# hucsmn/suffix_array

Measured on AMD Instinct MI355X. Metric: input MB/s indexed (SA build), higher is better.
Workload: dtype u8; 1 GPU; c3_english_256m: 268435456 bytes per GPU, seed base + rank, one independent text per GPU; n_bytes=268435456, sigma=57, symbols_per_key=13, refinement_rounds=9, text_rounds=0, radix_passes=25, unresolved_after_initial_sort=199000237

## Files before the change

suffix_array_amd/csrc/host/pipeline.hpp:

```cpp
#pragma once
#include "support.hpp"
#include "tuning.hpp"
#include "pool.hpp"

#include <functional>

namespace sa {

constexpr int SORT_MAX_WG = 1024;
constexpr int BK_TOP_BITS_MAX = 18;
constexpr uint32_t BK_BUCKETS_MAX = 1u << BK_TOP_BITS_MAX;
static_assert(32 - 16 <= BK_MAX_LBITS, "two 8-bit passes inside a bucket");
constexpr size_t GRAM_MAX_ENTRIES = (size_t)1 << 24;
static_assert(GROUP_CAP_MAX == GS_CAP, "Tuning clamps SA_AMD_GROUP_CAP to the kernel's cap");

#ifdef SA_AMD_DIAG
typedef void (*DownsweepFn)(const uint64_t *, const uint32_t *, uint64_t *, uint32_t *, uint32_t *,
                            const uint32_t *, int64_t, int, uint32_t, int64_t, int);
struct SortVariant { int threads, items, wg_per_cu; DownsweepFn fn; const char *name; };
static const SortVariant sort_variants[] = {
    { 1024, 8, 2, k_radix_downsweep_wcl<1024, 8, 16, 1, false, uint64_t, 4>, "carry-completed lines 1024x8 + LDS prefetch of half of the next tile's keys (default)" },
    { 1024, 8, 2, k_radix_downsweep_wcl<1024, 8>, "carry-completed lines 1024x8" },
    { 512, 16, 1, k_radix_downsweep_wcl<512, 16>, "carry-completed lines 512x16" },
    { 1024, 8, 2, k_radix_downsweep_wcl<1024, 8, 8>, "carry 1024x8, granule 8" },
#ifdef SA_AMD_DIAG
    { 1024, 8, 2, k_radix_downsweep<1024, 8, 4>, "plain tile scatter 1024x8 (first generation)" },
    { 1024, 8, 2, k_radix_downsweep<1024, 8, 4, 1>, "plain 1024x8 ABLATION sequential stores (wrong results)" },
    { 1024, 8, 2, k_radix_downsweep<1024, 8, 4, 33>, "plain 1024x8 ABLATION no ranking + sequential stores (wrong results)" },
    { 1024, 8, 2, k_radix_downsweep<1024, 8, 4, 16>, "plain 1024x8 ABLATION no stores (wrong results)" },
    { 1024, 8, 2, k_radix_downsweep<1024, 8, 4, 49>, "plain 1024x8 ABLATION no ranking, no stores (wrong results)" },
    { 1024, 8, 2, k_radix_downsweep_wcl<1024, 8, 16, 1, true>, "carry 1024x8 DIAGNOSTIC phase stamps (tools/phase_stamps.py)" },
#endif
};
constexpr int N_SORT_VARIANTS = (int)(sizeof(sort_variants) / sizeof(sort_variants[0]));

struct SortGrid { int G; int64_t tiles_per_wg; int tile; };
static SortGrid sort_grid(int64_t count, const SortVariant &sv)
{
    SortGrid g;
    g.tile = sv.threads * sv.items;
    const int64_t tiles = ceil_div(count, g.tile);
    int max_wg = 256 * sv.wg_per_cu;
    if (max_wg > SORT_MAX_WG) max_wg = SORT_MAX_WG;
    g.tiles_per_wg = ceil_div(tiles, max_wg);
    if (g.tiles_per_wg < 1) g.tiles_per_wg = 1;
    g.G = (int)ceil_div(tiles, g.tiles_per_wg);
    if (g.G < 1) g.G = 1;
    return g;
}

#else
constexpr int N_SORT_VARIANTS = 1;
#endif

struct SortScratch {
    uint32_t *spine;
    uint32_t *digit_tot;
    unsigned long long *status;
    uint32_t *err;
};

struct Workspace {
    uint64_t *keysA, *keysB, *keysC;
    uint32_t *valsA, *valsB, *isa, *U0, *U1, *G0, *G1;
    uint32_t *spine, *digit_tot, *tcnt, *thead, *tnext, *hist, *total, *chg, *has_isa;
    uint8_t *packed;
    uint8_t *gram_flags;
    uint4 *gram_table;
    uint32_t *surv_bits, *surv_cnt, *todo_bits, *ft_cnt, *ft_head;
    unsigned long long *os_status;
    uint32_t *os_err;
    uint32_t *bk_start;
    uint32_t *early_bits, *early_cnt;
    SortScratch ss;
    size_t bytes, bytes2;
};

static Workspace carve(void *base, int64_t n, size_t cap = ~(size_t)0, void *base2 = nullptr)
{
    Workspace w;
    const size_t N = (size_t)(n > 0 ? n : 1);
    size_t off = 0, off2 = 0;
    auto take = [&](size_t b) {
        if (off + b <= cap) { size_t o = off; off = align_up(off + b, 256); return (char *)base + o; }
        size_t o = off2; off2 = align_up(off2 + b, 256); return (char *)base2 + o;
    };
    const size_t rr_tiles = (size_t)ceil_div((int64_t)N, RR_TILE);
    const size_t ft_tiles = (size_t)ceil_div((int64_t)N, FT_TILE) + 1;
    const size_t gram_entries = N < GRAM_MAX_ENTRIES ? N : GRAM_MAX_ENTRIES;
    w.spine = (uint32_t *)take((size_t)RADIX * SORT_MAX_WG * 4);
    w.digit_tot = (uint32_t *)take(RADIX * 4);
    w.os_status = (unsigned long long *)take(((size_t)ceil_div((int64_t)N, OS_MIN_TILE) + 1) * RADIX * 8);
    w.os_err = (uint32_t *)take(256);
    w.hist = (uint32_t *)take(256 * 4);
    w.total = (uint32_t *)take(256);
    w.chg = (uint32_t *)take((size_t)RR_CHG_COUNTERS * 32 * 4);
    w.tcnt = (uint32_t *)take(rr_tiles * 4);
    w.thead = (uint32_t *)take(rr_tiles * 4);
    w.tnext = (uint32_t *)take(rr_tiles * 4);
    w.surv_cnt = (uint32_t *)take(rr_tiles * 4);
    w.ft_cnt = (uint32_t *)take(ft_tiles * 4);
    w.ft_head = (uint32_t *)take(ft_tiles * 4);
    w.bk_start = (uint32_t *)take(((size_t)BK_BUCKETS_MAX + 1) * 4);
    w.early_cnt = (uint32_t *)take(((N + 1 + EARLY_TILE - 1) / EARLY_TILE + 8) * 4);
    w.gram_table = (uint4 *)take((gram_entries / 64 + 1) * 16);
    w.has_isa = (uint32_t *)take((N + 31) / 32 * 4);
    w.surv_bits = (uint32_t *)take((N + 31) / 32 * 4);
    w.todo_bits = (uint32_t *)take((N + 31) / 32 * 4);
    w.early_bits = (uint32_t *)take(((N + 1 + 31) / 32 + EARLY_THREADS) * 4);
    w.gram_flags = (uint8_t *)take(gram_entries + 64);
    w.packed = (uint8_t *)take(N / 2 + 64);
    w.keysA = (uint64_t *)take((N + 64) * 8);
    w.keysB = (uint64_t *)take((N + 64) * 8);
    w.valsA = (uint32_t *)take(N * 4);
    w.valsB = (uint32_t *)take(N * 4);
    w.isa = (uint32_t *)take(N * 4);
    w.U0 = (uint32_t *)take(N * 4);
    w.G0 = (uint32_t *)take(N * 4);
    w.U1 = (uint32_t *)take(N * 4);
    w.G1 = (uint32_t *)take(N * 4);
    w.keysC = (uint64_t *)take((N + 64) * 8);
    w.ss.spine = w.spine; w.ss.digit_tot = w.digit_tot; w.ss.status = w.os_status; w.ss.err = w.os_err;
    w.bytes = off;
    w.bytes2 = off2;
    return w;
}


struct OsShape { int threads, items; bool seq; int wg_per_cu; };
static const OsShape os_shapes64[] = { { 1024, 8, false, 1 }, { 512, 16, true, 2 }, { 512, 8, false, 2 } };
static const OsShape os_shapes32[] = { { 1024, 12, false, 1 }, { 512, 16, true, 2 }, { 512, 12, false, 2 }, { 1024, 8, false, 1 } };
constexpr int N_OS_SHAPES64 = (int)(sizeof(os_shapes64) / sizeof(os_shapes64[0]));
constexpr int N_OS_SHAPES32 = (int)(sizeof(os_shapes32) / sizeof(os_shapes32[0]));
constexpr int OS_TICKETS = 64;
constexpr int OS_MAX_RADIX = 512;
constexpr int OS_ZONE = OS_TICKETS + OS_MAX_RADIX * OS_NSEG;
static_assert(OS_NSEG <= OS_TICKETS, "one ticket word per segment");
constexpr int OS_MAX_ZONES = 2 * 8 + 2;
static_assert(OS_MAX_ZONES * OS_ZONE <= RADIX * SORT_MAX_WG, "the zones live in the spine slab");

#ifdef SA_AMD_DIAG
static bool onesweep_on(const SortScratch &ss, const Tuning &tn) { return ss.status != nullptr && !tn.no_onesweep; }
#else
static bool onesweep_on(const SortScratch &ss, const Tuning &) { return ss.status != nullptr; }
#endif

struct OnesweepGeom { int tiles, nseg, tiles_per_seg; int64_t seg_elems; };
static OnesweepGeom onesweep_geom(int64_t count, int tile)
{
    OnesweepGeom g;
    g.tiles = (int)ceil_div(count, tile);
    if (g.tiles < 1) g.tiles = 1;
    int nseg = g.tiles < OS_NSEG ? g.tiles : OS_NSEG;
    g.tiles_per_seg = (int)ceil_div(g.tiles, nseg);
    g.nseg = (int)ceil_div(g.tiles, g.tiles_per_seg);
    g.seg_elems = (int64_t)g.tiles_per_seg * tile;
    return g;
}

struct FirstCounts { uint32_t *counts; int64_t chunk_elems; int G; void *zero_ptr; size_t zero_bytes; };
static FirstCounts sort_first_counts(const SortScratch &ss, const Tuning &tn, int64_t count, bool keys32);

static int cu_count()
{
    static int cus = 0;
    if (cus > 0) return cus;
    int dev = 0;
    hipDeviceProp_t prop;
    if (hipGetDevice(&dev) == hipSuccess && hipGetDeviceProperties(&prop, dev) == hipSuccess && prop.multiProcessorCount > 0) cus = prop.multiProcessorCount;
    else { (void)hipGetLastError(); cus = 256; }
    return cus;
}

static int read_words(void *dst, const void *dsrc, size_t bytes, hipStream_t st);

__global__ __launch_bounds__(RADIX) void k_os_digit_totals(const uint32_t *__restrict__ hist, int nseg, uint32_t *__restrict__ digit_tot)
{
    uint32_t s = 0;
    for (int q = 0; q < nseg; ++q) s += hist[threadIdx.x * nseg + q];
    digit_tot[threadIdx.x] = s;
}

constexpr int HA_THREADS = 256;
template <typename KeyT>
__global__ __launch_bounds__(HA_THREADS) void k_radix_hist_all(const KeyT *__restrict__ keys, int64_t count, int begin_bit, int end_bit,
                                                               uint32_t *__restrict__ zone0, int zone_words, int ticket_words)
{
    __shared__ uint32_t h[8][RADIX];
    for (int i = threadIdx.x; i < 8 * RADIX; i += HA_THREADS) (&h[0][0])[i] = 0;
    __syncthreads();
    const int np = (end_bit - begin_bit + RADIX_BITS - 1) / RADIX_BITS;
    for (int64_t i = (int64_t)blockIdx.x * HA_THREADS + threadIdx.x; i < count; i += (int64_t)gridDim.x * HA_THREADS) {
        const uint64_t k = (uint64_t)keys[i];
        for (int p = 0; p < np; ++p) {
            const int sh = begin_bit + p * RADIX_BITS, nb = end_bit - sh < RADIX_BITS ? end_bit - sh : RADIX_BITS;
            atomicAdd(&h[p][(k >> sh) & ((1u << nb) - 1u)], 1u);
        }
    }
    __syncthreads();
    for (int i = threadIdx.x; i < np * RADIX; i += HA_THREADS) {
        const uint32_t c = (&h[0][0])[i];
        if (c) atomicAdd(&zone0[(size_t)(i / RADIX) * zone_words + ticket_words + (i % RADIX)], c);
    }
}

template <typename KeyT, int THREADS, int ITEMS, bool SEQ, int RBITS = RADIX_BITS>
static int sort_pairs_onesweep(KeyT *keys_in, uint32_t *vals_in, KeyT *keys_alt, uint32_t *vals_alt, int64_t count, int begin_bit, int end_bit,
                               const SortScratch &ss, uint32_t *final_vals, hipStream_t st, KeyT **keys_res, uint32_t **vals_res, int *passes,
                               int *skipped, const Tuning &tn, bool iota, bool may_skip, bool first_counted,
                               const uint8_t *text = nullptr, int64_t text_n = 0,
                               int text_bits = 8,
                               int val_extra = 0,
                               KeyT *keys_out2 = nullptr)
{
    constexpr int TILE = THREADS * ITEMS;
    constexpr int R = 1 << RBITS;
    static_assert(R <= OS_MAX_RADIX && (RBITS == RADIX_BITS || TILE >= 2 * OS_MIN_TILE), "zones and granule slab are sized for 8-bit digits of 4 Ki-element tiles");
    static_assert(TILE >= OS_MIN_TILE, "the granule slab is sized for tiles of at least OS_MIN_TILE elements");
    constexpr bool K64 = sizeof(KeyT) == 8;
    OnesweepGeom g = onesweep_geom(count, TILE);
    auto zone = [&](int i) { return ss.spine + (size_t)i * OS_ZONE; };
    int z = 0;
    bool have_counts = first_counted;
    const int npass = (int)ceil_div(end_bit - begin_bit, RBITS);
    const bool upfront = RBITS == RADIX_BITS && !tn.no_upfront_counts && count < tn.count_next_min_n && !may_skip && !text && npass <= 8 && npass >= 2;
    if (upfront) { g.nseg = 1; g.tiles_per_seg = g.tiles; g.seg_elems = (int64_t)g.tiles * TILE; }
    HIP_TRY(hipMemsetAsync(ss.status, 0, (size_t)g.tiles * R * 8, st));
    {
        int zones = (may_skip ? 2 * npass : npass) + 1;
        if (zones > OS_MAX_ZONES) return SA_AMD_EINTERNAL;
        const int z0 = (first_counted && !upfront) ? 1 : 0;
        HIP_TRY(hipMemsetAsync(zone(z0), 0, (size_t)(zones - z0) * OS_ZONE * 4, st));
    }
    if (upfront) {
        int blocks = (int)ceil_div(count, (int64_t)HA_THREADS * 16);
        if (blocks > 512) blocks = 512;
        if (blocks < 1) blocks = 1;
        PROF(K64 ? KC_UPSWEEP : KC_UPSWEEP32, count, st, hipLaunchKernelGGL((k_radix_hist_all<KeyT>), dim3((unsigned)blocks), dim3(HA_THREADS), 0, st, (const KeyT *)keys_in, count,
                                                                        begin_bit, end_bit, zone(0), (int)OS_ZONE, (int)OS_TICKETS));
        have_counts = true;
    }
    KeyT *kin = keys_in, *kout = keys_alt;
    uint32_t *vin = vals_in, *vout = vals_alt;
    constexpr int WG_PER_CU = THREADS <= 512 ? 2 : 1;
    int grid = cu_count() * WG_PER_CU;
    if (grid > g.tiles) grid = g.tiles;
    uint32_t epoch = 0;
    for (int shift = begin_bit; shift < end_bit; shift += RBITS) {
        const int nb = (end_bit - shift) < RBITS ? (end_bit - shift) : RBITS;
        const uint32_t dmask = (1u << nb) - 1u;
        const bool last = shift + RBITS >= end_bit;
        uint32_t *vdst = (last && final_vals) ? final_vals : vout;
        if (!have_counts) {
            if (RBITS != RADIX_BITS) return SA_AMD_EINTERNAL;
            int split = 2048 / g.nseg;
            while (split > 1 && g.seg_elems / split < 8192) split /= 2;
            const int64_t sub = K64 ? ((ceil_div(g.seg_elems, split) + 1) & ~(int64_t)1) : ((ceil_div(g.seg_elems, split) + 3) & ~(int64_t)3);
            if (K64)
                PROF(KC_UPSWEEP, count, st, hipLaunchKernelGGL((k_radix_upsweep), dim3(g.nseg * split), dim3(SORT_THREADS), 0, st, (const uint64_t *)kin,
                                                               zone(z) + OS_TICKETS, count, shift, dmask, g.seg_elems, g.nseg, split, sub));
            else
                PROF(KC_UPSWEEP32, count, st, hipLaunchKernelGGL((k_radix_upsweep32), dim3(g.nseg * split), dim3(SORT_THREADS), 0, st, (const uint32_t *)kin,
                                                                 zone(z) + OS_TICKETS, count, shift, dmask, g.seg_elems, g.nseg, split, sub));
        }
        if (RBITS == RADIX_BITS && may_skip && !tn.no_run_skip && count >= tn.run_skip_min && !(iota && *passes == 0) && !(last && final_vals)) {
            hipLaunchKernelGGL(k_os_digit_totals, dim3(1), dim3(RADIX), 0, st, (const uint32_t *)(zone(z) + OS_TICKETS), g.nseg, ss.digit_tot);
            LAUNCH_CHECK(st);
            uint32_t tot[RADIX];
            { const int rcw = read_words(tot, ss.digit_tot, sizeof(tot), st); if (rcw) return rcw; }
            bool constant = false;
            for (int d = 0; d < RADIX; ++d) constant |= (int64_t)tot[d] == count;
            if (constant) { ++*skipped; have_counts = false; ++z; continue; }
        }
        OnesweepPass P;
        P.hist_cur = zone(z) + OS_TICKETS;
        const bool count_next = !upfront && !last && (RBITS != RADIX_BITS || count >= tn.count_next_min_n || count < tn.count_next_below_n);
        P.hist_next = count_next ? zone(z + 1) + OS_TICKETS : nullptr;
        P.tickets = zone(z + 1);
        P.status = ss.status;
        P.err = ss.err;
        P.n = count;
        P.shift = shift; P.dmask = dmask;
        P.shift_next = shift + RBITS;
        { const int nbn = (end_bit - P.shift_next) < RBITS ? (end_bit - P.shift_next) : RBITS; P.dmask_next = last ? 0u : (1u << nbn) - 1u; }
        P.nseg = g.nseg; P.tiles_per_seg = g.tiles_per_seg; P.tiles = g.tiles;
        P.epoch = ++epoch;
        P.flags = (uint32_t)tn.onesweep_flags;
        P.text = text; P.text_n = text_n; P.text_bits = text_bits;
        P.val_extra = (text && *passes == 0 && iota) ? val_extra : 0;
        if (!K64 && !SEQ && text && *passes == 0)
            PROF(KC_ONESWEEP32, count, st,
                 hipLaunchKernelGGL((k_onesweep<THREADS, ITEMS, KeyT, SEQ, WG_PER_CU, RBITS, !K64 && !SEQ>), dim3(grid), dim3(THREADS), 0, st, (const KeyT *)kin,
                                    (const uint32_t *)((iota && *passes == 0) ? nullptr : vin), kout, vdst, P));
        else
        PROF(K64 ? KC_ONESWEEP : KC_ONESWEEP32, count, st,
             hipLaunchKernelGGL((k_onesweep<THREADS, ITEMS, KeyT, SEQ, WG_PER_CU, RBITS>), dim3(grid), dim3(THREADS), 0, st, (const KeyT *)kin,
                                (const uint32_t *)((iota && *passes == 0) ? nullptr : vin), kout, vdst, P));
        KeyT *tk = kin; kin = kout; kout = (keys_out2 && *passes == 0) ? keys_out2 : tk;
        uint32_t *free_v = vin;
        vin = vdst;
        vout = free_v;
        ++*passes;
        ++z;
        have_counts = count_next || upfront;
    }
    *keys_res = kin; *vals_res = vin;
    return SA_AMD_OK;
}

struct SortResult { uint64_t *keys; uint32_t *vals; int passes; int skipped; };

static int sort_pairs(uint64_t *keys_in, uint32_t *vals_in, uint64_t *keys_alt, uint32_t *vals_alt, int64_t count,
                      int begin_bit, int end_bit, const SortScratch &ss, uint32_t *final_vals,
                      hipStream_t st, SortResult *res, const Tuning &tn, bool iota = false,
                      bool may_skip = false,
                      bool first_counted = false)
{
    res->keys = keys_in; res->vals = vals_in; res->passes = 0; res->skipped = 0;
    if (count <= 1 || end_bit <= begin_bit) return SA_AMD_OK;
    if (onesweep_on(ss, tn)) {
#define OS_CALL64(T, I, S) sort_pairs_onesweep<uint64_t, T, I, S>(keys_in, vals_in, keys_alt, vals_alt, count, begin_bit, end_bit, ss, final_vals, st, \
                                                                 &res->keys, &res->vals, &res->passes, &res->skipped, tn, iota, may_skip, first_counted)
        switch (tn.onesweep64_shape) {
        case 1: return OS_CALL64(512, 16, true);
        case 2: return OS_CALL64(512, 8, false);
        default: return OS_CALL64(1024, 8, false);
        }
#undef OS_CALL64
    }
#ifdef SA_AMD_DIAG
    uint32_t *spine = ss.spine, *digit_tot = ss.digit_tot;
    const SortVariant &sv = sort_variants[tn.sort_variant];
    const SortGrid g = sort_grid(count, sv);
    uint64_t *kin = keys_in, *kout = keys_alt;
    uint32_t *vin = vals_in, *vout = vals_alt;
    for (int shift = begin_bit; shift < end_bit; shift += RADIX_BITS) {
        const int nb = (end_bit - shift) < RADIX_BITS ? (end_bit - shift) : RADIX_BITS;
        const uint32_t dmask = (1u << nb) - 1u;
        const bool last = shift + RADIX_BITS >= end_bit;
        uint32_t *vdst = (last && final_vals) ? final_vals : vout;
        {
            const int64_t chunk = g.tiles_per_wg * g.tile;
            int split = 2048 / g.G;
            if (split < 1) split = 1;
            while (split > 1 && chunk / split < 4096) split /= 2;
            const int64_t sub = (ceil_div(chunk, split) + 1) & ~(int64_t)1;
            if (first_counted && shift == begin_bit) {
            } else {
            if (split > 1 && res->passes == 0) HIP_TRY(hipMemsetAsync(spine, 0, (size_t)RADIX * g.G * 4, st));
            PROF(KC_UPSWEEP, count, st, hipLaunchKernelGGL((k_radix_upsweep), dim3(g.G * split), dim3(SORT_THREADS), 0, st, kin, spine,
                                                           count, shift, dmask, chunk, g.G, split, sub));
            }
        }
        PROF(KC_SPINE, (int64_t)RADIX * g.G, st, hipLaunchKernelGGL((k_spine_rows), dim3(RADIX), dim3(SPINE_THREADS), 0, st,
                                                                    spine, digit_tot, g.G));
        if (may_skip && !tn.no_run_skip && count >= tn.run_skip_min && !(iota && res->passes == 0) && !(last && final_vals)) {
            uint32_t tot[RADIX];
            { const int rcw = read_words(tot, digit_tot, sizeof(tot), st); if (rcw) return rcw; }
            bool constant = false;
            for (int d = 0; d < RADIX; ++d) constant |= (int64_t)tot[d] == count;
            if (constant) {
                HIP_TRY(hipMemsetAsync(spine, 0, (size_t)RADIX * g.G * 4, st));
                res->skipped++;
                continue;
            }
        }
        PROF(KC_DOWNSWEEP, count, st, hipLaunchKernelGGL((sv.fn), dim3(g.G), dim3(sv.threads), 0, st,
                                                         (const uint64_t *)kin, (const uint32_t *)((iota && res->passes == 0) ? nullptr : vin), kout, vdst,
                                                         spine, (const uint32_t *)digit_tot, count, shift,
                                                         dmask, g.tiles_per_wg, g.G));
        uint64_t *tk = kin; kin = kout; kout = tk;
        uint32_t *free_v = vin;
        vin = vdst;
        vout = free_v;
        res->passes++;
    }
    res->keys = kin; res->vals = vin;
    return SA_AMD_OK;
#else
    return SA_AMD_EINTERNAL;
#endif
}

struct SortResult32 { uint32_t *keys; uint32_t *vals; int passes; };
#ifdef SA_AMD_DIAG
constexpr int SORT32_THREADS = 1024;
typedef void (*Downsweep32Fn)(const uint32_t *, const uint32_t *, uint32_t *, uint32_t *, uint32_t *, const uint32_t *, int64_t, int,
                              uint32_t, int64_t, int);
struct Sort32Variant { int items; Downsweep32Fn fn; };
static const Sort32Variant sort32_variants[] = {
    { 12, k_radix_downsweep_wcl<SORT32_THREADS, 12, 16, 1, false, uint32_t, 12> },
    { 12, k_radix_downsweep_wcl<SORT32_THREADS, 12, 16, 1, false, uint32_t> },
    { 8, k_radix_downsweep_wcl<SORT32_THREADS, 8, 16, 1, false, uint32_t> },
    { 16, k_radix_downsweep_wcl<SORT32_THREADS, 16, 16, 1, false, uint32_t> },
    { 8, k_radix_downsweep_wcl<SORT32_THREADS, 8, 16, 1, false, uint32_t, 8> },
};
constexpr int N_SORT32_VARIANTS = (int)(sizeof(sort32_variants) / sizeof(sort32_variants[0]));

struct SortGrid32 { int G; int64_t tiles_per_wg, tile; };
static SortGrid32 sort_grid32(int64_t count, const Sort32Variant &sv)
{
    SortGrid32 g;
    g.tile = (int64_t)SORT32_THREADS * sv.items;
    const int64_t tiles = ceil_div(count, g.tile);
    g.tiles_per_wg = ceil_div(tiles, 512);
    if (g.tiles_per_wg < 1) g.tiles_per_wg = 1;
    g.G = (int)ceil_div(tiles, g.tiles_per_wg);
    return g;
}

#else
constexpr int N_SORT32_VARIANTS = 1;
#endif

static int sort_pairs32(uint32_t *keys_in, uint32_t *vals_in, uint32_t *keys_alt, uint32_t *vals_alt, int64_t count, int begin_bit,
                        int end_bit, const SortScratch &ss, uint32_t *final_vals, hipStream_t st, SortResult32 *res,
                        const Tuning &tn, bool iota = false, bool first_counted = false,
                        int rbits = RADIX_BITS,
                        const uint8_t *text = nullptr, int64_t text_n = 0, int text_bits = 8,
                        int val_extra = 0,
                        uint32_t *keys_out2 = nullptr)
{
    res->keys = keys_in; res->vals = vals_in; res->passes = 0;
    if (keys_out2 && (rbits != RADIX_BITS || text)) return SA_AMD_EINTERNAL;
    if (count <= 1 || end_bit <= begin_bit) return SA_AMD_OK;
    if (rbits != RADIX_BITS && (rbits != 9 || !onesweep_on(ss, tn) || !first_counted)) return SA_AMD_EINTERNAL;
    if (text && (!onesweep_on(ss, tn) || !first_counted || tn.onesweep32_shape != 0)) return SA_AMD_EINTERNAL;
    if (onesweep_on(ss, tn)) {
        int skipped = 0;
        if (rbits == 9)
            return sort_pairs_onesweep<uint32_t, 1024, 12, false, 9>(keys_in, vals_in, keys_alt, vals_alt, count, begin_bit, end_bit, ss, final_vals, st,
                                                                     &res->keys, &res->vals, &res->passes, &skipped, tn, iota, false, first_counted, text, text_n, text_bits, val_extra);
        if (text)
            return sort_pairs_onesweep<uint32_t, 1024, 12, false, RADIX_BITS>(keys_in, vals_in, keys_alt, vals_alt, count, begin_bit, end_bit, ss, final_vals, st,
                                                                              &res->keys, &res->vals, &res->passes, &skipped, tn, iota, false, first_counted, text, text_n, text_bits, val_extra);
#define OS_CALL32(T, I, S) sort_pairs_onesweep<uint32_t, T, I, S>(keys_in, vals_in, keys_alt, vals_alt, count, begin_bit, end_bit, ss, final_vals, st, \
                                                                 &res->keys, &res->vals, &res->passes, &skipped, tn, iota, false, first_counted, \
                                                                 nullptr, 0, 8, 0, keys_out2)
        switch (tn.onesweep32_shape) {
        case 1: return OS_CALL32(512, 16, true);
        case 2: return OS_CALL32(512, 12, false);
        case 3: return OS_CALL32(1024, 8, false);
        default: return OS_CALL32(1024, 12, false);
        }
#undef OS_CALL32
    }
#ifdef SA_AMD_DIAG
    uint32_t *spine = ss.spine, *digit_tot = ss.digit_tot;
    const Sort32Variant &sv = sort32_variants[tn.sort32_variant];
    const SortGrid32 g32 = sort_grid32(count, sv);
    const int64_t SORT32_TILE = g32.tile, tiles_per_wg = g32.tiles_per_wg;
    const int G = g32.G;
    uint32_t *kin = keys_in, *kout = keys_alt, *vin = vals_in, *vout = vals_alt;
    for (int shift = begin_bit; shift < end_bit; shift += RADIX_BITS) {
        const int nb = (end_bit - shift) < RADIX_BITS ? (end_bit - shift) : RADIX_BITS;
        const uint32_t dmask = (1u << nb) - 1u;
        const bool last = shift + RADIX_BITS >= end_bit;
        uint32_t *vdst = (last && final_vals) ? final_vals : vout;
        {
            const int64_t chunk = tiles_per_wg * SORT32_TILE;
            int split = 2048 / G;
            if (split < 1) split = 1;
            while (split > 1 && chunk / split < 8192) split /= 2;
            const int64_t sub = (ceil_div(chunk, split) + 3) & ~(int64_t)3;
            if (first_counted && shift == begin_bit) {
            } else {
            if (split > 1 && res->passes == 0) HIP_TRY(hipMemsetAsync(spine, 0, (size_t)RADIX * G * 4, st));
            PROF(KC_UPSWEEP32, count, st, hipLaunchKernelGGL((k_radix_upsweep32), dim3(G * split), dim3(SORT_THREADS), 0, st,
                                                           (const uint32_t *)kin, spine, count, shift, dmask, chunk, G, split, sub));
            }
        }
        PROF(KC_SPINE, (int64_t)RADIX * G, st, hipLaunchKernelGGL((k_spine_rows), dim3(RADIX), dim3(SPINE_THREADS), 0, st, spine, digit_tot, G));
        PROF(KC_DOWNSWEEP32, count, st, hipLaunchKernelGGL((sv.fn),
                                                         dim3(G), dim3(SORT32_THREADS), 0, st, (const uint32_t *)kin,
                                                         (const uint32_t *)((iota && res->passes == 0) ? nullptr : vin), kout,
                                                         vdst, spine, (const uint32_t *)digit_tot, count, shift, dmask,
                                                         tiles_per_wg, G));
        uint32_t *tk = kin; kin = kout; kout = (keys_out2 && res->passes == 0) ? keys_out2 : tk;
        uint32_t *free_v = vin;
        vin = vdst;
        vout = free_v;
        res->passes++;
    }
    res->keys = kin; res->vals = vin;
    return SA_AMD_OK;
#else
    return SA_AMD_EINTERNAL;
#endif
}

static FirstCounts sort_first_counts(const SortScratch &ss, const Tuning &tn, int64_t count, bool keys32)
{
    FirstCounts f;
    if (onesweep_on(ss, tn)) {
        const OsShape &sh = keys32 ? os_shapes32[tn.onesweep32_shape] : os_shapes64[tn.onesweep64_shape];
        const int tile = sh.threads * sh.items;
        const OnesweepGeom g = onesweep_geom(count, tile);
        f.counts = ss.spine + OS_TICKETS; f.chunk_elems = g.seg_elems; f.G = g.nseg;
        f.zero_ptr = ss.spine; f.zero_bytes = (size_t)OS_ZONE * 4;
        return f;
    }
#ifdef SA_AMD_DIAG
    f.counts = ss.spine; f.zero_ptr = ss.spine;
    if (keys32) {
        const SortGrid32 g32 = sort_grid32(count, sort32_variants[tn.sort32_variant]);
        f.chunk_elems = g32.tiles_per_wg * g32.tile; f.G = g32.G;
    } else {
        const SortGrid g64 = sort_grid(count, sort_variants[tn.sort_variant]);
        f.chunk_elems = g64.tiles_per_wg * g64.tile; f.G = g64.G;
    }
    f.zero_bytes = (size_t)RADIX * f.G * 4;
    return f;
#else
    f.counts = ss.spine; f.zero_ptr = ss.spine; f.chunk_elems = count; f.G = 1; f.zero_bytes = (size_t)RADIX * 4;
    return f;
#endif
}

struct BkShape { int threads, items, minw; };
static const BkShape bk_shapes[] = { { 256, 10, 6 }, { 512, 10, 8 }, { 1024, 10, 8 }, { 1024, 20, 1 }, { 256, 20, 1 } };
constexpr int N_BK_SHAPES = (int)(sizeof(bk_shapes) / sizeof(bk_shapes[0]));
constexpr int N_BK_DEFAULT = 4;
static int64_t bucket_cap(int shape) { return (int64_t)bk_shapes[shape].threads * bk_shapes[shape].items; }
static int64_t bucket_cap_max() { return bucket_cap(N_BK_DEFAULT - 1); }

static int bucket_sort32(const uint32_t *keys_in, const uint32_t *vals_in, uint32_t *keys_out, uint32_t *vals_out, int64_t count, int top_bits,
                         uint32_t *start, uint32_t *words, hipStream_t st, const Tuning &tn, bool *done, uint32_t *largest,
                         const BucketFinish *fin = nullptr, const KeyParams *P = nullptr, const KeySrc *K = nullptr, bool *fused = nullptr,
                         int val_extra = 0)
{
    *done = false; *largest = 0;
    if (fused) *fused = false;
    if (top_bits < 32 - BK_MAX_LBITS || top_bits > BK_TOP_BITS_MAX) return SA_AMD_EINTERNAL;
    const int lbits = 32 - top_bits;
    if (val_extra < 0 || lbits + val_extra > BK_MAX_LBITS) return SA_AMD_EINTERNAL;
    const uint32_t nb = 1u << top_bits;
    HIP_TRY(hipMemsetAsync(words, 0, 8, st));
    PROF(KC_MISC, nb, st, hipLaunchKernelGGL((k_bucket_starts), dim3((unsigned)ceil_div((int64_t)nb + 1, BK_STARTS_THREADS)), dim3(BK_STARTS_THREADS),
                                              0, st, keys_in, count, lbits, nb, start));
    PROF(KC_MISC, nb, st, hipLaunchKernelGGL((k_bucket_max), dim3((unsigned)ceil_div((int64_t)nb, BK_STARTS_THREADS)), dim3(BK_STARTS_THREADS), 0, st,
                                              (const uint32_t *)start, nb, words));
    uint32_t maxb = 0;
    { const int rcw = read_words(&maxb, words, 4, st); if (rcw) return rcw; }
    *largest = maxb;
    int shape = -1;
    if (tn.bucket_shape >= 0 && tn.bucket_shape < N_BK_SHAPES && bucket_cap(tn.bucket_shape) >= (int64_t)maxb) shape = tn.bucket_shape;
    for (int c = 0; shape < 0 && c < N_BK_DEFAULT; ++c)
        if (bucket_cap(c) >= (int64_t)maxb) shape = c;
    if (shape < 0) return SA_AMD_OK;
    const bool fuse = fin != nullptr && (bk_shapes[shape].items <= 10 || tn.bucket_finish_always);
    const BucketFinish F0 = BucketFinish();
    const KeyParams P0 = KeyParams();
    const KeySrc K0 = KeySrc();
#define BK_LAUNCH(T, I, W)                                                                                                               \
    do {                                                                                                                                 \
        if (fuse) PROF(KC_BUCKET, count, st, hipLaunchKernelGGL((k_bucket_sort<T, I, W, true>), dim3(nb), dim3(T), 0, st, keys_in, vals_in,         \
                                                                (const uint32_t *)start, lbits, keys_out, vals_out, words + 1, *fin, *P, *K, val_extra)); \
        else PROF(KC_BUCKET, count, st, hipLaunchKernelGGL((k_bucket_sort<T, I, W, false>), dim3(nb), dim3(T), 0, st, keys_in, vals_in,             \
                                                            (const uint32_t *)start, lbits, keys_out, vals_out, words + 1, F0, P0, K0, val_extra)); \
    } while (0)
    switch (shape) {
    case 0: BK_LAUNCH(256, 10, 6); break;
    case 1: BK_LAUNCH(512, 10, 8); break;
    case 2: BK_LAUNCH(1024, 10, 8); break;
    case 3: BK_LAUNCH(1024, 20, 1); break;
    default: BK_LAUNCH(256, 20, 1); break;
    }
#undef BK_LAUNCH
    *done = true;
    if (fused) *fused = fuse;
    return SA_AMD_OK;
}

#ifdef SA_AMD_DIAG
static int64_t sample_count(int64_t n, const Tuning &tn)
{
    int lg = tn.sample_log ? tn.sample_log : (n >= ((int64_t)1 << 28) ? 22 : (n >= ((int64_t)1 << 27) ? 21 : 20));
    while (lg > 16 && ((int64_t)1 << lg) * 4 > n) --lg;
    return (int64_t)1 << lg;
}

static int sample_sort64(uint64_t *keys_a, uint64_t *keys_b, uint64_t *keys_c, uint32_t *vals_a, uint32_t *vals_b, uint32_t *u0, uint32_t *u1,
                         uint32_t *big, uint32_t *small, uint32_t *words, uint32_t *final_vals, int64_t n, int key_bits, const SortScratch &ss,
                         hipStream_t st, sa_amd_stats *local, const Tuning &tn, bool *done, bool trace)
{
    *done = false;
    const int64_t S = sample_count(n, tn);
    if (S < 65536 || n < 4 * S || n >= ((int64_t)1 << 32)) return SA_AMD_OK;
    uint64_t *samp = keys_c, *samp_alt = keys_c + S;
    PROF(KC_MISC, S, st, hipLaunchKernelGGL((k_ss_sample), dim3((unsigned)ceil_div(S, 256)), dim3(256), 0, st, (const uint64_t *)keys_a, n, S, samp));
    SortResult sr;
// ... 11 lines not shown
    PROF(KC_SS_COUNT, n, st, hipLaunchKernelGGL((k_ss_count<1>), dim3((unsigned)tiles1), dim3(SS_THREADS), 0, st, (const uint64_t *)keys_a, n, sample, S,
                                                (const uint32_t *)nullptr, (const uint32_t *)nullptr, (const uint32_t *)nullptr, counts));
    PROF(KC_RR_SCAN, tiles1, st, hipLaunchKernelGGL((k_ss_scan_tiles<SS_WAYS>), dim3((unsigned)chunks), dim3(SS_WAYS), 0, st, counts, tiles1, per,
                                                    (const uint32_t *)nullptr, tot1));
    PROF(KC_RR_SCAN, chunks, st, hipLaunchKernelGGL((k_ss_bases1), dim3(1), dim3(SS_WAYS), 0, st, (const uint32_t *)tot1, chunks, base1, seg_start, seg_first));
    PROF(KC_RR_SCAN, max_tiles2, st, hipLaunchKernelGGL((k_ss_tiles), dim3(SS_WAYS + 1), dim3(256), 0, st, (const uint32_t *)seg_start, (const uint32_t *)seg_first,
                                                        max_tiles2, tile_seg, tile_base));
    PROF(KC_SS_SCATTER, n, st, hipLaunchKernelGGL((k_ss_scatter<1>), dim3((unsigned)tiles1), dim3(SS_THREADS), 0, st, (const uint64_t *)keys_a, (const uint32_t *)nullptr, n,
                                                  sample, S, (const uint32_t *)nullptr, (const uint32_t *)nullptr, (const uint32_t *)nullptr,
                                                  (const uint32_t *)counts, (const uint32_t *)base1, per, keys_b, vals_a));
    PROF(KC_SS_COUNT, n, st, hipLaunchKernelGGL((k_ss_count<2>), dim3((unsigned)max_tiles2), dim3(SS_THREADS), 0, st, (const uint64_t *)keys_b, n, sample, S,
                                                (const uint32_t *)tile_seg, (const uint32_t *)tile_base, (const uint32_t *)seg_start, counts));
    PROF(KC_RR_SCAN, max_tiles2, st, hipLaunchKernelGGL((k_ss_scan_tiles<SS_IDS2>), dim3(SS_WAYS), dim3(SS_IDS2), 0, st, counts, max_tiles2, (int64_t)0,
                                                        (const uint32_t *)seg_first, tot2));
    PROF(KC_RR_SCAN, SS_WAYS, st, hipLaunchKernelGGL((k_ss_bases2), dim3(SS_WAYS), dim3(SS_IDS2), 0, st, (const uint32_t *)tot2, (const uint32_t *)seg_start, bstart, (uint32_t)n));
    PROF(KC_SS_SCATTER, n, st, hipLaunchKernelGGL((k_ss_scatter<2>), dim3((unsigned)max_tiles2), dim3(SS_THREADS), 0, st, (const uint64_t *)keys_b, (const uint32_t *)vals_a, n,
                                                  sample, S, (const uint32_t *)tile_seg, (const uint32_t *)tile_base, (const uint32_t *)seg_start,
                                                  (const uint32_t *)counts, (const uint32_t *)bstart, (int64_t)1, keys_a, vals_b));
    HIP_TRY(hipMemsetAsync(words, 0, 16, st));
    if (!tn.sample_merge)
    PROF(KC_SS_BUCKET, n, st, hipLaunchKernelGGL((k_ss_bucket_sort<SB_SMALL_THREADS, SB_SMALL_ITEMS, 9, 0, false>), dim3((unsigned)SS_BUCKETS), dim3(SB_SMALL_THREADS), 0, st,
                                                 (const uint64_t *)keys_a, (const uint32_t *)vals_b, (const uint32_t *)bstart, keys_b, final_vals, words, words + 4));
    else
    PROF(KC_SS_BUCKET, n, st, hipLaunchKernelGGL((k_ss_bucket_merge<SB_SMALL_THREADS, SB_SMALL_ITEMS>), dim3((unsigned)SS_BUCKETS), dim3(SB_SMALL_THREADS), 0, st,
                                                 (const uint64_t *)keys_a, (const uint32_t *)vals_b, (const uint32_t *)bstart, keys_b, final_vals, words));
    PROF(KC_SS_BUCKET, 0, st, hipLaunchKernelGGL((k_ss_bucket_sort<SB_THREADS, SB_ITEMS, 10, SB_SMALL_CAP, true>), dim3((unsigned)SS_BUCKETS), dim3(SB_THREADS), 0, st,
                                                 (const uint64_t *)keys_a, (const uint32_t *)vals_b, (const uint32_t *)bstart, keys_b, final_vals, words, words + 4));
    uint32_t res[2] = { 0, 0 };
    { const int rcw = read_words(res, words, 8, st); if (rcw) return rcw; }
    local->sort_passes += 3; local->sorted_elements += 3 * n;
    if (trace) fprintf(stderr, "suffix_array_amd: sample sort: %lld samples, largest bucket %u (a workgroup holds %d), %u oversize buckets that are no equality buckets\n",
                       (long long)S, res[1], SB_CAP, res[0]);
    *done = res[0] == 0;
    return SA_AMD_OK;
}

#endif

static int make_key_params(const uint32_t *hist, KeyParams *P, int *sigma_out, int kb_max = 64)
{
    int sigma = 0;
    for (int c = 0; c < 256; ++c) {
        if (hist[c]) P->code[c] = (uint8_t)sigma++;
        else P->code[c] = 0;
    }
    *sigma_out = sigma;
    P->packed = nullptr;
    P->gram = 0; P->gram_m = 0; P->gram_tail = 0; P->gram_top = 0; P->gram_D = 0; P->gram_table = nullptr;
    const uint64_t se = sigma > 2 ? (uint64_t)sigma : 2u;
    P->sigma = se;
    if ((se & (se - 1)) == 0) {
        const int bits = bit_length(se - 1);
        P->bits = bits;
        P->k = kb_max / bits;
        const int used = P->k * bits;
        P->mask = used >= 64 ? ~0ull : ((1ull << used) - 1ull);
        P->top = 0;
        return used;
    }
    unsigned __int128 pw = 1;
    int k = 0;
    while (pw * se <= ((unsigned __int128)1 << kb_max)) { pw *= se; ++k; }
    P->bits = 0;
    P->k = k;
    P->mask = ~0ull;
    uint64_t top = 1;
    for (int i = 0; i + 1 < k; ++i) top *= se;
    P->top = top;
    const unsigned __int128 maxkey = pw - 1;
    return bit_length((uint64_t)maxkey);
}

struct PinnedWords {
    PinBlock b;
    bool failed = false;
    ~PinnedWords() { if (b.p) pool().release_pinned(b); }
};
static thread_local PinnedWords g_pinned;
static thread_local int g_readbacks = 0;
static thread_local bool g_posted_off = false;
static std::atomic<uint32_t> g_post_seq{0};

constexpr int POST_LINE = 16;
__global__ __launch_bounds__(256) void k_post_words(const uint32_t *__restrict__ src, uint32_t *__restrict__ dst, int words, uint32_t seq)
{
    const int lines = (words + POST_LINE - 2) / (POST_LINE - 1);
    for (int i = threadIdx.x; i < lines * POST_LINE; i += 256) {
        const int q = i / POST_LINE, j = i % POST_LINE;
        if (j) { const int k = q * (POST_LINE - 1) + j - 1; dst[i] = k < words ? src[k] : 0u; }
    }
    __threadfence_system();
    __syncthreads();
    for (int q = threadIdx.x; q < lines; q += 256) __hip_atomic_store(dst + q * POST_LINE, seq, __ATOMIC_RELEASE, __HIP_MEMORY_SCOPE_SYSTEM);
}

static int read_words(void *dst, const void *dsrc, size_t bytes, hipStream_t st)
{
    ++g_readbacks;
    if (!g_pinned.b.p && !g_pinned.failed) {
        if (pool().pinned(8192, -1, -1, &g_pinned.b) == SA_AMD_OK) memset(g_pinned.b.p, 0, 8192);
        else g_pinned.failed = true;
    }
    if (!g_pinned.b.p) {
        HIP_TRY(hipMemcpyAsync(dst, dsrc, bytes, hipMemcpyDeviceToHost, st));
        HIP_TRY(hipStreamSynchronize(st));
        return SA_AMD_OK;
    }
    const int words = (int)(bytes / 4);
    const int lines = (words + POST_LINE - 2) / (POST_LINE - 1);
    if (!g_posted_off && (bytes & 3) == 0 && words > 0 && (size_t)lines * POST_LINE * 4 <= 4096) {
        uint32_t *host = (uint32_t *)g_pinned.b.p;
        uint32_t seq = g_post_seq.fetch_add(1, std::memory_order_relaxed) + 1;
        if (seq == 0) seq = g_post_seq.fetch_add(1, std::memory_order_relaxed) + 1;
        hipLaunchKernelGGL(k_post_words, dim3(1), dim3(256), 0, st, (const uint32_t *)dsrc, host, words, seq);
        if (hipGetLastError() == hipSuccess) {
            const auto t0 = std::chrono::steady_clock::now();
            bool done = false, finished = false;
            for (unsigned spin = 0; !done; ++spin) {
                done = true;
                for (int q = lines - 1; q >= 0 && done; --q)
                    done = __atomic_load_n((volatile uint32_t *)(host + q * POST_LINE), __ATOMIC_ACQUIRE) == seq;
                if (done) break;
                if ((spin & 1023u) == 1023u) {
                    const double us = std::chrono::duration<double, std::micro>(std::chrono::steady_clock::now() - t0).count();
                    if (us > 200.0) {
                        if (finished) break;
                        const hipError_t q = hipStreamQuery(st);
                        if (q == hipSuccess) finished = true;
                        else if (q != hipErrorNotReady) { (void)hipGetLastError(); break; }
                    }
                }
            }
            if (done) {
                uint32_t *out = (uint32_t *)dst;
                for (int k = 0; k < words; ++k) out[k] = host[(k / (POST_LINE - 1)) * POST_LINE + 1 + k % (POST_LINE - 1)];
                return SA_AMD_OK;
            }
        }
    }
    char *copy = (char *)g_pinned.b.p + 4096;
    HIP_TRY(hipMemcpyAsync(copy, dsrc, bytes, hipMemcpyDeviceToHost, st));
    HIP_TRY(hipStreamSynchronize(st));
    memcpy(dst, copy, bytes);
    return SA_AMD_OK;
}

static bool binned(int64_t n, int64_t count, const Tuning &tn)
{
    if (tn.no_binned_isa) return false;
    if (tn.binned_isa_always) return count > 0;
    return n >= ((int64_t)1 << 25) && (count >= n || count >= tn.binned_min);
}

static int scatter_binned(uint32_t *pk, uint32_t *pv, uint32_t *altk, uint32_t *altv, int64_t count, int64_t n,
                          const Workspace &w, hipStream_t st, sa_amd_stats *local, const Tuning &tn, bool iota = false,
                          uint32_t *altk2 = nullptr, uint32_t *altv2 = nullptr)
{
    const int nb = bit_length((uint64_t)(n > 1 ? n : 1));
    int wlog = nb - 16;
    if (wlog < 10) wlog = 10;
    if (wlog > 15) wlog = 15;
    const bool two = nb > wlog && (tn.scatter_levels == 2 || (tn.scatter_levels == 0 && count >= ((int64_t)1 << 25)));
    SortResult32 pr;
    if (two) {
        int rc;
        if (iota) {
            const int mid = wlog + RADIX_BITS < nb ? wlog + RADIX_BITS : nb;
            rc = sort_pairs32(pk, nullptr, altk, altv, count, wlog, mid, w.ss, nullptr, st, &pr, tn, true);
            if (rc) return rc;
            if (pr.passes != 1) return SA_AMD_EINTERNAL;
            local->sort_passes += 1; local->sorted_elements += count;
            if (mid < nb) {
                rc = sort_pairs32(altk, altv, altk2, altv2, count, mid, nb, w.ss, nullptr, st, &pr, tn);
                if (rc) return rc;
                local->sort_passes += pr.passes; local->sorted_elements += (int64_t)pr.passes * count;
            }
        } else {
            rc = sort_pairs32(pk, pv, altk, altv, count, wlog, nb, w.ss, nullptr, st, &pr, tn, false, false, RADIX_BITS, nullptr, 0, 8, 0, altk2);
            if (rc) return rc;
            local->sort_passes += pr.passes; local->sorted_elements += (int64_t)pr.passes * count;
        }
        const unsigned grid = (unsigned)ceil_div(count, SW_CHUNK);
        if (wlog <= 13)
            PROF(KC_SCATTER, count, st, hipLaunchKernelGGL((k_scatter_windows<13>), dim3(grid), dim3(SW_THREADS), 0, st, (const uint32_t *)pr.keys,
                                                           (const uint32_t *)pr.vals, w.isa, count, (uint32_t)n, wlog));
        else
            PROF(KC_SCATTER, count, st, hipLaunchKernelGGL((k_scatter_windows<15>), dim3(grid), dim3(SW_THREADS), 0, st, (const uint32_t *)pr.keys,
                                                           (const uint32_t *)pr.vals, w.isa, count, (uint32_t)n, wlog));
        return SA_AMD_OK;
    }
    const int shift = nb > RADIX_BITS ? nb - RADIX_BITS : 0;
    int rc = sort_pairs32(pk, pv, altk, altv, count, shift, shift + RADIX_BITS, w.ss, nullptr, st, &pr, tn, iota);
    if (rc) return rc;
    local->sort_passes += pr.passes; local->sorted_elements += (int64_t)pr.passes * count;
    PROF(KC_SCATTER, count, st, hipLaunchKernelGGL((k_scatter_pairs<uint32_t>), dim3((unsigned)ceil_div(count, 1024)), dim3(256), 0, st,
                                                   (const uint32_t *)pr.keys, (const uint32_t *)pr.vals, w.isa, count, (uint32_t)n));
    return SA_AMD_OK;
}

struct Refined { const uint64_t *keys; const uint32_t *vals; uint32_t *vnext; int64_t m_global; };

constexpr int RC_FLAGGED = 16, RC_GROUPS = 8, RC_BIG_LISTED = 12, RC_BIG_ORDERED = 13, RC_WORDS = 17;
constexpr int RC_BIG_LISTED_SAVED = 14, RC_BIG_ORDERED_SAVED = 15;
struct RoundCtl {
    bool defer = false;
    const uint32_t *resume_tot = nullptr;
    bool skip_big = false;
    bool counters_clear = false;
    bool deferred = false;
    int64_t m_flagged = -1;
    int64_t big_listed = -1;
};

static int split_giant_groups(uint64_t *rkA, uint64_t *rkB, uint32_t *Vcur, uint32_t *Valt, const uint32_t *Ucur, const uint32_t *Gcur,
                              uint32_t *scratchU, uint32_t *scratchG, int64_t m, int64_t n, uint32_t groups, int kb, int sort_bits,
                              const Workspace &w, hipStream_t st, sa_amd_stats *local, Refined *out, const Tuning &tn, bool *taken,
                              bool starts_ready)
{
    *taken = false;
    const int64_t tiles = ceil_div(m, RR_TILE);
    auto up = [](size_t b) { return (b + 255) & ~(size_t)255; };
    char *sg = (char *)scratchG;
    uint32_t *starts = (uint32_t *)sg;            sg += up(((size_t)groups + 1) * 4);
    uint32_t *mps = (uint32_t *)sg;               sg += up(((size_t)groups + 1) * 4);
    uint32_t *Lless = (uint32_t *)sg;             sg += up((size_t)groups * 4);
    uint64_t *pivot = (uint64_t *)sg;             sg += up((size_t)groups * 8);
    const size_t cap = (size_t)m / 8 + 1;
    uint32_t *mv = (uint32_t *)sg, *mv_alt = mv + ((cap + 63) & ~(size_t)63);
    uint64_t *mk = (uint64_t *)scratchU, *mk_alt = mk + ((cap + 31) & ~(size_t)31);
    const size_t need_g = (size_t)(sg - (char *)scratchG) + 2 * ((cap + 63) & ~(size_t)63) * 4;
    const size_t need_u = 2 * ((cap + 31) & ~(size_t)31) * 8;
    if (need_g > (size_t)n * 4 || need_u > (size_t)n * 4) return SA_AMD_OK;
    if (!starts_ready)
        PROF(KC_RR_COUNT, m, st, hipLaunchKernelGGL((k_group_starts), dim3((unsigned)tiles), dim3(RR_THREADS), 0, st, Ucur, Gcur, m,
                                                    (const uint32_t *)w.ft_cnt, groups, starts));
    PROF(KC_MISC, groups, st, hipLaunchKernelGGL((k_split_pivots), dim3((unsigned)ceil_div((int64_t)groups, 256)), dim3(256), 0, st,
                                             (const uint64_t *)rkA, (const uint32_t *)starts, groups, kb, pivot));
    PROF(KC_RR_COUNT, m, st, hipLaunchKernelGGL((k_split_count), dim3((unsigned)tiles), dim3(RR_THREADS), 0, st, (const uint64_t *)rkA, m, kb,
                                                (const uint64_t *)pivot, w.tcnt));
    PROF(KC_RR_SCAN, tiles, st, hipLaunchKernelGGL((k_rr_scan), dim3(1), dim3(SPINE_THREADS), 0, st, w.tcnt, w.thead, tiles, w.total));
    uint32_t minor = 0;
    { const int rcw = read_words(&minor, w.total, 4, st); if (rcw) return rcw; }
    if ((int64_t)minor * 8 > m) return SA_AMD_OK;
    *taken = true;
    out->m_global = m;
    if (minor == 0) {
        out->keys = rkA; out->vals = Vcur; out->vnext = Valt;
        return SA_AMD_OK;
    }
    PROF(KC_RR_APPLY, m, st, hipLaunchKernelGGL((k_split_pass<false>), dim3((unsigned)tiles), dim3(RR_THREADS), 0, st,
                                                (const uint64_t *)rkA, (const uint32_t *)Vcur, m, kb, (const uint64_t *)pivot,
                                                (const uint32_t *)w.tcnt, (const uint32_t *)starts, groups, mps, (const uint32_t *)w.total,
                                                mk, mv, (const uint32_t *)nullptr, (uint64_t *)nullptr, (uint32_t *)nullptr));
    SortResult s2;
    const int rc = sort_pairs(mk, mv, mk_alt, mv_alt, minor, 0, sort_bits, w.ss, nullptr, st, &s2, tn);
    if (rc) return rc;
    local->sort_passes += s2.passes; local->sorted_elements += (int64_t)s2.passes * minor;
    PROF(KC_MISC, groups, st, hipLaunchKernelGGL((k_split_less), dim3((unsigned)ceil_div((int64_t)groups, 256)), dim3(256), 0, st,
                                             (const uint64_t *)s2.keys, (const uint32_t *)mps, (const uint64_t *)pivot, groups, kb, Lless));
    PROF(KC_RR_APPLY, m, st, hipLaunchKernelGGL((k_split_pass<true>), dim3((unsigned)tiles), dim3(RR_THREADS), 0, st,
                                                (const uint64_t *)rkA, (const uint32_t *)Vcur, m, kb, (const uint64_t *)pivot,
                                                (const uint32_t *)w.tcnt, (const uint32_t *)starts, groups, mps, (const uint32_t *)w.total,
                                                (uint64_t *)nullptr, (uint32_t *)nullptr, (const uint32_t *)Lless, rkB, Valt));
    PROF(KC_SCATTER, minor, st, hipLaunchKernelGGL((k_split_place_minor), dim3((unsigned)ceil_div((int64_t)minor, 256)), dim3(256), 0, st,
                                                   (const uint64_t *)s2.keys, (const uint32_t *)s2.vals, (int64_t)minor, kb,
                                                   (const uint32_t *)starts, (const uint32_t *)mps, (const uint32_t *)Lless, rkB, Valt));
    out->keys = rkB; out->vals = Valt; out->vnext = Vcur;
    return SA_AMD_OK;
}

static int refine_list(uint64_t *rkA, uint64_t *rkB, uint32_t *Vcur, uint32_t *Valt, const uint32_t *Ucur, const uint32_t *Gcur,
                       uint32_t *scratchU, uint32_t *scratchG, int64_t m, int64_t n, const uint8_t *dT, const KeyParams &P,
                       const KeySrc &K_in, int g_bits, bool *local_ok, const Workspace &w, hipStream_t st, sa_amd_stats *local,
                       Refined *out, const Tuning &tn, bool retry_local = false, int *split_rest = nullptr,
                       RoundCtl *ctl = nullptr)
{
    KeySrc K = K_in;
    K.net_min = tn.network_min;
    const bool resume = ctl && ctl->resume_tot;
    const int64_t tiles = ceil_div(m, RR_TILE);
    const int kb = K.kb;
    SortResult sr;
    int rc;
    bool counted = false;
    uint32_t groups = 0;
    if (!*local_ok && retry_local && !tn.no_local_sort && m < tn.dense_rekey_min) *local_ok = true;
    if (!*local_ok && retry_local && !tn.no_local_sort && m >= tn.dense_rekey_min) {
        PROF(KC_RR_COUNT, m, st, hipLaunchKernelGGL((k_flag_count), dim3((unsigned)tiles), dim3(RR_THREADS), 0, st,
                                                    (const uint8_t *)nullptr, Ucur, Gcur, m, w.tcnt, w.ft_cnt));
        PROF(KC_RR_SCAN, tiles, st, hipLaunchKernelGGL((k_rr_scan), dim3(1), dim3(SPINE_THREADS), 0, st, w.ft_cnt, w.thead, tiles, w.total + 8));
        { const int rcw = read_words(&groups, w.total + 8, 4, st); if (rcw) return rcw; }
        counted = true;
        if ((int64_t)groups * 2 * tn.group_cap >= m) *local_ok = true;
    }
    const bool had_local_pass = *local_ok;
    if (*local_ok) {
        uint8_t *flags = (uint8_t *)scratchG;
        const unsigned gs_blocks = (unsigned)ceil_div(m, GS_TILE);
        const int cap = tn.group_cap;
        const bool big_local = !tn.no_big_group_sort && kb <= 32 && m > GS_CAP && !(ctl && ctl->skip_big);
        uint32_t *bheads = big_local ? scratchU : (uint32_t *)nullptr, *bcount = big_local ? w.total + RC_BIG_LISTED : (uint32_t *)nullptr;
        if (!resume) {
        if (!(ctl && ctl->counters_clear))
            HIP_TRY(hipMemsetAsync(w.total + RC_BIG_LISTED, 0, 8, st));
        if (K.mode == KS_TEXT)
            PROF(KC_LOCAL, m, st, hipLaunchKernelGGL((k_group_sort<KS_TEXT>), dim3(gs_blocks), dim3(GS_THREADS), 0, st, (const uint32_t *)Vcur,
                                                     Gcur, Ucur, dT, P, m, n, K, rkA, Vcur, flags, cap, bheads, bcount));
        else if (K.mode == KS_LOWKEY)
            PROF(KC_LOCAL, m, st, hipLaunchKernelGGL((k_group_sort<KS_LOWKEY>), dim3(gs_blocks), dim3(GS_THREADS), 0, st, (const uint32_t *)Vcur,
                                                     Gcur, Ucur, dT, P, m, n, K, rkA, Vcur, flags, cap, bheads, bcount));
        else if (K.mode == KS_RANK)
            PROF(KC_LOCAL, m, st, hipLaunchKernelGGL((k_group_sort<KS_RANK>), dim3(gs_blocks), dim3(GS_THREADS), 0, st, (const uint32_t *)Vcur,
                                                     Gcur, Ucur, dT, P, m, n, K, rkA, Vcur, flags, cap, bheads, bcount));
        else if (K.mode == KS_CHASE)
            PROF(KC_LOCAL, m, st, hipLaunchKernelGGL((k_group_sort<KS_CHASE>), dim3(gs_blocks), dim3(GS_THREADS), 0, st, (const uint32_t *)Vcur,
                                                     Gcur, Ucur, dT, P, m, n, K, rkA, Vcur, flags, cap, bheads, bcount));
        else {
            int64_t gblocks = ceil_div(m, GK_THREADS);
            if (gblocks > 8192) gblocks = 8192;
            PROF(KC_GATHER, m, st, hipLaunchKernelGGL((k_gather_textkey<KS_SPARSE>), dim3((unsigned)gblocks), dim3(GK_THREADS), 0, st,
                                                      (const uint32_t *)Vcur, Gcur, dT, P, m, n, K, rkA));
            PROF(KC_LOCAL, m, st, hipLaunchKernelGGL((k_group_sort<KS_PRE>), dim3(gs_blocks), dim3(GS_THREADS), 0, st, (const uint32_t *)Vcur,
                                                     Gcur, Ucur, dT, P, m, n, K, rkA, Vcur, flags, cap, bheads, bcount));
        }
        if (gs_blocks > 1)
            PROF(KC_LOCAL, 0, st, hipLaunchKernelGGL((k_group_sort_straddle), dim3(gs_blocks - 1), dim3(GX_THREADS), 0, st, rkA, Vcur, Gcur,
                                                     Ucur, m, flags, cap, K, n));
        if (big_local) {
            const int lo = cap > GS_CAP ? cap : GS_CAP;
            PROF(KC_LOCAL, 0, st, hipLaunchKernelGGL((k_group_sort_big<256>), dim3((unsigned)(8 * cu_count())), dim3(256), 0, st, rkA, Vcur, Gcur, m, kb, lo,
                                                     (const uint32_t *)bheads, (const uint32_t *)bcount, flags, w.total + 13));
            PROF(KC_LOCAL, 0, st, hipLaunchKernelGGL((k_group_sort_big<512>), dim3((unsigned)(4 * cu_count())), dim3(512), 0, st, rkA, Vcur, Gcur, m, kb,
                                                     lo > GB_CAP_SMALL ? lo : GB_CAP_SMALL, (const uint32_t *)bheads, (const uint32_t *)bcount, flags, w.total + 13));
        }
        PROF(KC_RR_COUNT, m, st, hipLaunchKernelGGL((k_flag_count), dim3((unsigned)tiles), dim3(RR_THREADS), 0, st,
                                                    (const uint8_t *)flags, Ucur, Gcur, m, w.tcnt, w.ft_cnt));
        PROF(KC_RR_SCAN, tiles, st, hipLaunchKernelGGL((k_rr_scan_pair), dim3(2), dim3(SPINE_THREADS), 0, st, w.tcnt, w.thead, w.total + RC_FLAGGED,
                                                       w.ft_cnt, (uint32_t *)nullptr, w.total + RC_GROUPS, tiles));
        }
        if (ctl && ctl->defer && !resume) {
            ctl->deferred = true;
            out->keys = rkA; out->vals = Vcur; out->vnext = Valt; out->m_global = 0;
            return SA_AMD_OK;
        }
        uint32_t tot9[RC_WORDS] = { 0 };
// ... 27 lines not shown
    int sort_bits = kb + g_bits;
    bool rekeyed = false;
    if (m >= tn.dense_rekey_min) {
        if (!counted || had_local_pass) {
            PROF(KC_RR_COUNT, m, st, hipLaunchKernelGGL((k_flag_count), dim3((unsigned)tiles), dim3(RR_THREADS), 0, st,
                                                        (const uint8_t *)nullptr, Ucur, Gcur, m, w.tcnt, w.ft_cnt));
            PROF(KC_RR_SCAN, tiles, st, hipLaunchKernelGGL((k_rr_scan), dim3(1), dim3(SPINE_THREADS), 0, st, w.ft_cnt, w.thead, tiles, w.total + 8));
            { const int rcw = read_words(&groups, w.total + 8, 4, st); if (rcw) return rcw; }
            }
        const int idx_bits = bit_length((uint64_t)(groups > 0 ? groups - 1 : 0));
        if (ceil_div(kb + idx_bits, RADIX_BITS) < ceil_div(kb + g_bits, RADIX_BITS)) {
            sort_bits = kb + idx_bits;
            rekeyed = true;
        }
    }
    const bool split_wanted = rekeyed && !tn.no_split && m >= tn.split_min && groups > 0 && (int64_t)groups * tn.split_group_min <= m &&
                              !(split_rest && *split_rest > 0);
    bool starts_ready = false;
    if (had_local_pass) {
        if (rekeyed)
            PROF(KC_RR_APPLY, m, st, hipLaunchKernelGGL((k_rekey_dense), dim3((unsigned)tiles), dim3(RR_THREADS), 0, st, rkA, Ucur, Gcur, m,
                                                        (const uint32_t *)w.ft_cnt, kb));
    } else if (K.mode == KS_SPARSE) {
        int64_t gblocks = ceil_div(m, GK_THREADS);
        if (gblocks > 8192) gblocks = 8192;
        PROF(KC_GATHER, m, st, hipLaunchKernelGGL((k_gather_textkey<KS_SPARSE>), dim3((unsigned)gblocks), dim3(GK_THREADS), 0, st,
                                                  (const uint32_t *)Vcur, Gcur, dT, P, m, n, K, rkA));
        if (rekeyed)
            PROF(KC_RR_APPLY, m, st, hipLaunchKernelGGL((k_rekey_dense), dim3((unsigned)tiles), dim3(RR_THREADS), 0, st, rkA, Ucur, Gcur, m,
                                                        (const uint32_t *)w.ft_cnt, kb));
    } else {
        const uint32_t *th = rekeyed ? (const uint32_t *)w.ft_cnt : (const uint32_t *)nullptr;
        uint32_t *gs = split_wanted ? scratchG : (uint32_t *)nullptr;
        starts_ready = gs != nullptr;
        if (K.mode == KS_TEXT)
            PROF(KC_GATHER, m, st, hipLaunchKernelGGL((k_gather_keyed<KS_TEXT>), dim3((unsigned)tiles), dim3(RR_THREADS), 0, st,
                                                      (const uint32_t *)Vcur, Ucur, Gcur, dT, P, m, n, K, th, rkA, gs, groups));
        else if (K.mode == KS_LOWKEY)
            PROF(KC_GATHER, m, st, hipLaunchKernelGGL((k_gather_keyed<KS_LOWKEY>), dim3((unsigned)tiles), dim3(RR_THREADS), 0, st,
                                                      (const uint32_t *)Vcur, Ucur, Gcur, dT, P, m, n, K, th, rkA, gs, groups));
        else
            PROF(KC_GATHER, m, st, hipLaunchKernelGGL((k_gather_keyed<KS_RANK>), dim3((unsigned)tiles), dim3(RR_THREADS), 0, st,
                                                      (const uint32_t *)Vcur, Ucur, Gcur, dT, P, m, n, K, th, rkA, gs, groups));
    }
    if (split_rest && *split_rest > 0) --*split_rest;
    else if (split_wanted) {
        bool taken = false;
        rc = split_giant_groups(rkA, rkB, Vcur, Valt, Ucur, Gcur, scratchU, scratchG, m, n, groups, kb, sort_bits, w, st, local, out, tn, &taken,
                                starts_ready);
        if (rc || taken) return rc;
        if (split_rest) *split_rest = 3;
    }
    rc = sort_pairs(rkA, Vcur, rkB, Valt, m, 0, sort_bits, w.ss, nullptr, st, &sr, tn, false, true);
    if (rc) return rc;
    local->sort_passes += sr.passes; local->sorted_elements += (int64_t)sr.passes * m;
    out->keys = sr.keys; out->vals = sr.vals; out->m_global = m;
    out->vnext = (sr.vals == Vcur) ? Valt : Vcur;
    return SA_AMD_OK;
}

static int choose_gram_keys(const uint8_t *dT, int64_t n, KeyParams *Pp, int *key_bits, const Workspace &w, hipStream_t st,
                            const Tuning &tn, bool trace)
{
    KeyParams &P = *Pp;
    const uint64_t se = P.sigma;
    const uint64_t cap = (uint64_t)((size_t)n < GRAM_MAX_ENTRIES ? (size_t)n : GRAM_MAX_ENTRIES);
    int g = 0;
    uint64_t S = 1;
    for (int t = 1; t <= 8; ++t) {
        if (S * se > cap) break;
        S *= se; g = t;
        if (tn.gram_g >= 2 && g == tn.gram_g) break;
    }
    if (g < 2) return SA_AMD_OK;
    uint64_t top = 1;
    for (int t = 0; t + 1 < g; ++t) top *= se;
    const int64_t gtiles = ceil_div((int64_t)S, GT_TILE);
    HIP_TRY(hipMemsetAsync(w.gram_flags, 0, (size_t)S, st));
    PROF(KC_MISC, n, st, hipLaunchKernelGGL((k_gram_mark), dim3((unsigned)ceil_div(ceil_div(n, KB_TILE), GM_TPW)), dim3(KB_THREADS), 0, st, dT, n, P, g,
                                            (uint32_t)top, w.gram_flags));
    PROF(KC_MISC, (int64_t)S, st, hipLaunchKernelGGL((k_gram_count), dim3((unsigned)gtiles), dim3(GT_THREADS), 0, st,
                                            (const uint8_t *)w.gram_flags, (int64_t)S, w.tcnt));
    PROF(KC_RR_SCAN, gtiles, st, hipLaunchKernelGGL((k_rr_scan), dim3(1), dim3(SPINE_THREADS), 0, st, w.tcnt, w.thead, gtiles, w.total));
    uint32_t D = 0;
    { const int rcw = read_words(&D, w.total, 4, st); if (rcw) return rcw; }
    int m = 0;
    unsigned __int128 pw = 1;
    while (D >= 2 && (m + 1) * g <= 64 && pw * D <= ((unsigned __int128)1 << 64)) { pw *= D; ++m; }
    int tail = 0;
    while (m > 0 && tail < tn.gram_tail_max && m * g + tail + 1 <= 64 && pw * se <= ((unsigned __int128)1 << 64)) { pw *= se; ++tail; }
    const int gram_bits = m > 0 ? bit_length((uint64_t)(pw - 1)) : 0;
    const int plain_passes = (int)ceil_div(*key_bits, RADIX_BITS), gram_passes = (int)ceil_div(gram_bits, RADIX_BITS);
    const int syms = m * g + tail;
    const bool better = m > 0 && (syms > P.k || (syms == P.k && gram_passes < plain_passes));
    if (trace) fprintf(stderr, "suffix_array_amd: gram keys: %u of %llu %d-grams occur -> %d symbols (%d grams + %d plain) in %d bits (plain: %d in %d) -> %s\n",
                       D, (unsigned long long)S, g, syms, m, tail, gram_bits, P.k, *key_bits, better ? "gram keys" : "plain keys");
    if (!better) return SA_AMD_OK;
    PROF(KC_MISC, (int64_t)S, st, hipLaunchKernelGGL((k_gram_table), dim3((unsigned)gtiles), dim3(GT_THREADS), 0, st,
                                            (const uint8_t *)w.gram_flags, (int64_t)S, (const uint32_t *)w.tcnt, w.gram_table));
    P.gram = g; P.gram_m = m; P.gram_tail = tail; P.gram_top = (uint32_t)top; P.gram_D = D; P.gram_table = w.gram_table;
    P.bits = 0; P.k = syms; P.mask = ~0ull;
    *key_bits = gram_bits;
    return SA_AMD_OK;
}

struct EarlyDownload {
    int off = 0;
    int64_t threshold = 0;
    std::function<void(hipEvent_t)> start;
    std::function<int64_t()> stop;
    bool started = false;
    int64_t m_snap = 0;
    int64_t covered = 0;
    int64_t holes = 0;
    const uint32_t *d_bits = nullptr, *d_tile_off = nullptr, *d_holes = nullptr;
    hipEvent_t ev = nullptr;
};

struct DeviceBuild {
    const uint8_t *dT;
    uint32_t *dSA, *SA;
    int64_t n;
    hipStream_t st;
    Tuning tn;
    Workspace w;
    sa_amd_stats local;
    EarlyDownload *early = nullptr;
    bool trace = false;
    double trace_t = 0;
    double lap() { const double t = now_ms(), d = t - trace_t; trace_t = t; return d; }
    bool timing_only() const
    {
#ifdef SA_AMD_DIAG
        return tn.timing_only_initial_sort;
#else
        return false;
#endif
    }
    KeyParams P, Ptext;
    int sigma = 0, key_bits = 0, g_bits = 0, top_shift = 0;
    bool force_dense = false, text_ok = false, local_ok = false, probe_dense = false;
    SortResult sr;
    const uint32_t *sorted32 = nullptr;
    int bucket_top_bits = 0;
    bool flat_text = false;
    bool bucket_finished = false;
    uint64_t *sorted0 = nullptr;
    uint32_t *Ucur = nullptr, *Unext = nullptr, *Gcur = nullptr, *Gnext = nullptr, *Vcur = nullptr;
    uint64_t *rkA = nullptr, *rkB = nullptr;
    int64_t tiles = 0, m = 0, depth = 0;
    uint32_t m32 = 0;
    bool lists_ready = false, finished32 = false, fused64 = false, sparse = false;
    bool isa_tail_ranks = false;
    int s_sym = 0, tkb = 0, key2_bits = 0;
    bool unary_done = false;
    bool prev_clean = true;
    int deferred_misses = 0;


    int early_maybe_start()
    {
        if (!early || early->started || m <= 0 || m > early->threshold || !early->start) return SA_AMD_OK;
        if (!early->ev && hipEventCreateWithFlags(&early->ev, hipEventDisableTiming) != hipSuccess) { (void)hipGetLastError(); return SA_AMD_OK; }
        hipLaunchKernelGGL(k_set_u32, dim3(1), dim3(1), 0, st, dSA, (uint32_t)n);
        LAUNCH_CHECK(st);
        HIP_TRY(hipMemsetAsync(w.early_bits, 0, (((size_t)n + 1 + 31) / 32 + EARLY_THREADS) * 4, st));
        int64_t blocks = ceil_div(m, 256 * 8);
        if (blocks > 65536) blocks = 65536;
        if ((((uintptr_t)Ucur) & 15) != 0) return SA_AMD_OK;
        PROF(KC_MISC, m, st, hipLaunchKernelGGL((k_early_mark), dim3((unsigned)blocks), dim3(256), 0, st, (const uint32_t *)Ucur, m, (uint32_t)early->off, w.early_bits));
        HIP_TRY(hipEventRecord(early->ev, st));
        early->started = true;
        early->m_snap = m;
        if (trace) fprintf(stderr, "suffix_array_amd: early download starts with %lld suffixes still tied\n", (long long)m);
        early->start(early->ev);
        return SA_AMD_OK;
    }
    int early_finish()
    {
        if (!early || !early->started) return SA_AMD_OK;
        early->covered = early->stop ? early->stop() : 0;
        if (early->covered > n + early->off) early->covered = n + early->off;
        early->holes = 0;
        if (early->covered <= 0) return SA_AMD_OK;
        const int64_t tiles_e = ceil_div(early->covered, EARLY_TILE);
        const int64_t words = ceil_div(early->covered, 32);
        PROF(KC_MISC, early->covered, st, hipLaunchKernelGGL((k_early_count), dim3((unsigned)tiles_e), dim3(EARLY_THREADS), 0, st,
                                                             (const uint32_t *)w.early_bits, words, w.early_cnt));
        PROF(KC_RR_SCAN, tiles_e, st, hipLaunchKernelGGL((k_rr_scan), dim3(1), dim3(SPINE_THREADS), 0, st, w.early_cnt, (uint32_t *)nullptr, tiles_e, w.early_cnt + tiles_e));
        uint32_t *holes = (uint32_t *)w.keysC;
        PROF(KC_MISC, early->covered, st, hipLaunchKernelGGL((k_early_gather), dim3((unsigned)tiles_e), dim3(EARLY_THREADS), 0, st,
                                                             (const uint32_t *)w.early_bits, words, (const uint32_t *)w.early_cnt,
                                                             (const uint32_t *)(dSA + 1 - early->off), holes));
        uint32_t total = 0;
        { const int rcw = read_words(&total, w.early_cnt + tiles_e, 4, st); if (rcw) return rcw; }
        early->holes = total;
        early->d_bits = w.early_bits; early->d_tile_off = w.early_cnt; early->d_holes = holes;
        return SA_AMD_OK;
    }

    int choose_bucket_bits() const
    {
        if (tn.no_bucket_sort || n < tn.bucket_min_n || n <= 1) return 0;
        const bool wide_ok = onesweep_on(w.ss, tn) && tn.onesweep32_shape == 0;
        if (tn.bucket_bits == 18 && wide_ok) return 18;
        if (tn.bucket_bits == 16) return 16;
        const bool value_bits = wide_ok && !tn.no_value_bits && !tn.no_text_keys && g_bits <= 30 &&
                                ((sigma == 256 && P.bits == 8) || (sigma == 4 && P.bits == 2 && !tn.no_packed_text));
        if (value_bits && (n >> 16) > 7500 && (n >> 18) * 10 <= bucket_cap_max() * 9) return 18;
        if ((n >> 16) * 10 <= bucket_cap(2) * 9) return 16;
        if (wide_ok && (n >> 18) * 10 <= bucket_cap_max() * 9) return 18;
        if ((n >> 16) * 10 <= bucket_cap_max() * 9) return 16;
        return 0;
    }

    bool flat_rule_applies() const { return n >= 2 && n < tn.top32_probe_min_n && n < ((int64_t)1 << 24) && !tn.no_flat_rule; }

    int geometry_and_probes()
    {
        int rc = SA_AMD_OK; (void)rc;
        HIP_TRY(hipMemsetAsync(w.hist, 0, 256 * 4, st));
        {
            int64_t blocks = ceil_div(ceil_div(n, 16), BH_THREADS);
            if (blocks > 2048) blocks = 2048;
            if (blocks < 1) blocks = 1;
            const bool counts = flat_rule_applies();
            if (counts) PROF(KC_BYTE_HIST, n, st, hipLaunchKernelGGL((k_byte_hist_counts), dim3((unsigned)(blocks > 256 ? 256 : blocks)), dim3(BH_THREADS), 0, st, dT, n, w.hist));
            else PROF(KC_BYTE_HIST, n, st, hipLaunchKernelGGL((k_byte_hist), dim3((unsigned)blocks), dim3(BH_THREADS), 0, st, dT, n, w.hist));
        }
        uint32_t hist[256];
        { const int rcw = read_words(hist, w.hist, sizeof(hist), st); if (rcw) return rcw; }
        int kb_max = tn.key_bits_max;
        if (flat_rule_applies()) {
            double h0 = 0.0; int used = 0;
            for (int c = 0; c < 256; ++c)
                if (hist[c]) { const double pc = (double)hist[c] / (double)n; h0 -= pc * std::log2(pc); ++used; }
            if (used >= 2 && h0 > std::log2((double)used) - 0.01) {
                int kb = (bit_length((uint64_t)(n - 1)) + 20 + 7) / 8 * 8;
                if (kb < 32) kb = 32;
                if (kb < kb_max) kb_max = kb;
                flat_text = true;
            }
        }
        key_bits = make_key_params(hist, &P, &sigma, kb_max);
        local.sigma = sigma; local.bits_per_symbol = P.bits; local.symbols_per_key = P.k;
        if (sigma == 1 && !tn.no_unary_shortcut) {
            int64_t blocks = ceil_div(n, 256 * 16);
            if (blocks > 16384) blocks = 16384;
            PROF(KC_MISC, n, st, hipLaunchKernelGGL((k_fill_descending), dim3((unsigned)blocks), dim3(256), 0, st, SA, n));
            unary_done = true;
            return SA_AMD_OK;
        }

        g_bits = bit_length((uint64_t)(n - 1 > 0 ? n - 1 : 1));
        bucket_top_bits = choose_bucket_bits();
        force_dense = tn.force_dense;
        text_ok = !force_dense && !tn.no_text_rounds;
        local_ok = !tn.no_local_sort;

        top_shift = 0;
        if (text_ok && local_ok && key_bits > 32 && !tn.no_top32) {
            bool use = tn.force_top32;
            if (!use && n >= tn.top32_probe_min_n) {
                int64_t S = (int64_t)1 << 20;
                while (S > 1024 && S * 8 > n) S >>= 1;
                PROF(KC_MISC, S, st, hipLaunchKernelGGL((k_sample_keys), dim3((unsigned)ceil_div(S, GK_THREADS)), dim3(GK_THREADS), 0, st, dT, P, n, S,
                                                        key_bits - 32, w.keysA));
                const uint32_t H = (uint32_t)S * 4u;
                HIP_TRY(hipMemsetAsync(w.keysB, 0xff, (size_t)H * 8, st));
                HIP_TRY(hipMemsetAsync(w.total, 0, 8, st));
                PROF(KC_MISC, S, st, hipLaunchKernelGGL((k_count_sample_dups), dim3((unsigned)(ceil_div(S, 256) < 4096 ? ceil_div(S, 256) : 4096)), dim3(256), 0, st, (const uint64_t *)w.keysA, S,
                                                        (unsigned long long *)w.keysB, H - 1u, w.total));
                const int tb = choose_bucket_bits();
                if (tb) {
                    HIP_TRY(hipMemsetAsync(w.keysC, 0, ((size_t)1 << tb) * 4, st));
                    PROF(KC_MISC, S / 4, st, hipLaunchKernelGGL((k_sample_bucket_hist), dim3((unsigned)ceil_div(S / 4, BK_STARTS_THREADS)), dim3(BK_STARTS_THREADS), 0, st,
                                                            (const uint64_t *)w.keysA, S / 4, tb, (uint32_t *)w.keysC));
                    PROF(KC_MISC, S, st, hipLaunchKernelGGL((k_u32_max), dim3((unsigned)(((size_t)1 << tb) / BK_STARTS_THREADS)), dim3(BK_STARTS_THREADS), 0, st,
                                                            (const uint32_t *)w.keysC, 1u << tb, w.total + 1));
                }
                uint32_t dups = 0;
                {
                    uint32_t two[2] = { 0, 0 };
                    const int rcw = read_words(two, w.total, 8, st); if (rcw) return rcw;
                    dups = two[0];
                    const double est = (double)two[1] * (double)n / (double)(S / 4);
                    if (tb && est > 3.0 * (double)bucket_cap_max()) {
                        bucket_top_bits = 0;
                        if (trace) fprintf(stderr, "suffix_array_amd: bucket sort of the 32-bit first stage: largest bucket estimated at %.0f suffixes -> four global passes\n", est);
                    }
                }
                const double p32 = (double)n * 2.0 * (double)dups / ((double)S * (double)S);
                use = p32 < (double)tn.top32_partners_x100 / 100.0;
                double p64 = -1.0;
                if (!use && p32 < 4.0 * (double)tn.top32_collisions_x100 / 100.0) {
                    PROF(KC_MISC, S, st, hipLaunchKernelGGL((k_sample_keys), dim3((unsigned)ceil_div(S, GK_THREADS)), dim3(GK_THREADS), 0, st, dT, P, n, S,
                                                            -1, w.keysA));
                    HIP_TRY(hipMemsetAsync(w.keysB, 0xff, (size_t)H * 8, st));
                    HIP_TRY(hipMemsetAsync(w.total, 0, 4, st));
                    PROF(KC_MISC, S, st, hipLaunchKernelGGL((k_count_sample_dups), dim3((unsigned)(ceil_div(S, 256) < 4096 ? ceil_div(S, 256) : 4096)), dim3(256), 0, st, (const uint64_t *)w.keysA, S,
                                                            (unsigned long long *)w.keysB, H - 1u, w.total));
                    uint32_t dups64 = 0;
                    { const int rcw = read_words(&dups64, w.total, 4, st); if (rcw) return rcw; }
                    const double chance = (double)S * (double)S / 8589934592.0;
                    const double d64 = (double)dups64 > chance ? (double)dups64 - chance : 0.0;
                    p64 = (double)n * 2.0 * d64 / ((double)S * (double)S);
// ... 172 lines not shown
            if (!ss_done) {
            rc = sort_pairs(w.keysA, w.valsA, w.keysB, w.valsB, n, 0, key_bits, w.ss, SA, st, &sr, tn, iota, sigma == 1, counted);
            if (rc) return rc;
            local.sort_passes += sr.passes; local.sorted_elements += (int64_t)sr.passes * n;
            }
        }
        P.packed = packed_out;
        if (sr.vals != SA) {
            PROF(KC_MISC, n, st, hipLaunchKernelGGL((k_copy_u32), dim3(1), dim3(256), 0, st, sr.vals, SA, n));
        }

        return SA_AMD_OK;
    }

    int first_round_from_sorted_keys()
    {
        int rc = SA_AMD_OK; (void)rc;
        Ucur = w.U0; Unext = w.U1; Gcur = w.G0; Gnext = w.G1;
        Vcur = w.valsA;
        tiles = ceil_div(n, RR_TILE);
        m32 = 0;
        m = 0;
        rkA = w.keysA; rkB = w.keysB;
        sorted0 = sr.keys;
        lists_ready = false;
        depth = P.k;
        Ptext = P;
        if (P.bits == 0) Ptext.bits = bit_length(P.sigma - 1);
        Ptext.gram = 0;
        s_sym = 0; tkb = 0;
        {
            const int room = 64 - g_bits;
            s_sym = room / Ptext.bits;
            if (s_sym > 64) s_sym = 64;
            tkb = s_sym * Ptext.bits;
        }
        finished32 = false; fused64 = false;
        if (top_shift && local_ok && !tn.no_fused_finish && !timing_only()) {
            const int cap = tn.group_cap;
            uint32_t *surv_bits = w.surv_bits, *surv_head = w.isa;
            if (!bucket_finished) {
            HIP_TRY(hipMemsetAsync(surv_bits, 0, ((size_t)n + 31) / 32 * 4, st));
            HIP_TRY(hipMemsetAsync(w.tcnt, 0, (size_t)tiles * 4, st));
            HIP_TRY(hipMemsetAsync(w.thead, 0, (size_t)tiles * 4, st));
            HIP_TRY(hipMemsetAsync(w.total, 0, 16, st));
            HIP_TRY(hipMemsetAsync(w.chg, 0, (size_t)RR_CHG_COUNTERS * 32 * 4, st));
            KeySrc K = KeySrc(); K.mode = KS_LOWKEY; K.kb = top_shift;
            PROF(KC_FINISH, n, st, hipLaunchKernelGGL((k_finish_sorted<uint32_t, KS_LOWKEY, false>), dim3((unsigned)ceil_div(n, FT_TILE)), dim3(FT_THREADS),
                                                     0, st, sorted32, SA, dT, P, n, K, cap, surv_bits, surv_head, w.tcnt, w.total, (uint32_t *)nullptr,
                                                     (uint32_t *)nullptr, (uint32_t *)nullptr));
            }
            if (!bucket_finished) PROF(KC_RR_SCAN, tiles, st, hipLaunchKernelGGL((k_rr_scan), dim3(1), dim3(SPINE_THREADS), 0, st, w.tcnt, w.thead, tiles, w.total));
            uint32_t cnt3[3] = { 0, 0, 0 };
            {
                uint32_t words[64 + RR_CHG_COUNTERS * 32];
                const int rcw = read_words(words, w.total, sizeof(words), st); if (rcw) return rcw;
                cnt3[0] = words[0]; cnt3[1] = words[1];
                for (int c = 0; c < RR_CHG_COUNTERS; ++c) cnt3[2] += words[64 + c * 32];
                if (bucket_finished) {
                    cnt3[0] = 0;
                    for (int c = 0; c < RR_CHG_COUNTERS; ++c) cnt3[0] += words[64 + c * 32 + 1];
                    if (cnt3[0] != 0 && cnt3[1] == 0)
                        PROF(KC_RR_SCAN, tiles, st, hipLaunchKernelGGL((k_rr_scan), dim3(1), dim3(SPINE_THREADS), 0, st, w.tcnt, w.thead, tiles, w.total));
                }
            }
            if (cnt3[1] == 0) {
                finished32 = true;
                m = cnt3[0];
                local.locally_sorted += cnt3[2];
                local.unresolved_after_initial = m;
                if (m > 0) {
                    PROF(KC_RR_APPLY, n, st, hipLaunchKernelGGL((k_surv_compact), dim3((unsigned)tiles), dim3(256), 0, st, (const uint32_t *)surv_bits,
                                                                (const uint32_t *)surv_head, (const uint32_t *)SA, n, (const uint32_t *)w.tcnt,
                                                                (const uint32_t *)w.total, Ucur, Gcur, Vcur));
                    rkA = (sr.keys == w.keysA) ? w.keysB : w.keysA;
                    rkB = w.keysC;
                    lists_ready = true;
                }
            }
        }
        if (!top_shift && text_ok && local_ok && s_sym > 0 && tn.fused64 && !tn.no_fused_finish && !tn.sparse_div_set && !timing_only()) {
            const int cap = tn.group_cap;
            const int64_t ft_tiles = ceil_div(n, FT_TILE);
            uint32_t *surv_head = w.isa;
            HIP_TRY(hipMemsetAsync(w.surv_bits, 0, ((size_t)n + 31) / 32 * 4, st));
            HIP_TRY(hipMemsetAsync(w.todo_bits, 0, ((size_t)n + 31) / 32 * 4, st));
            HIP_TRY(hipMemsetAsync(w.ft_cnt, 0, (size_t)(ft_tiles + 1) * 4, st));
            HIP_TRY(hipMemsetAsync(w.ft_head, 0, (size_t)(ft_tiles + 1) * 4, st));
            HIP_TRY(hipMemsetAsync(w.surv_cnt, 0, (size_t)tiles * 4, st));
            HIP_TRY(hipMemsetAsync(w.thead, 0, (size_t)tiles * 4, st));
            HIP_TRY(hipMemsetAsync(w.total, 0, 32, st));
            HIP_TRY(hipMemsetAsync(w.chg, 0, (size_t)RR_CHG_COUNTERS * 32 * 4, st));
            KeySrc K = KeySrc(); K.mode = KS_TEXT; K.h = depth; K.s = s_sym; K.kb = tkb;
            PROF(KC_FINISH, n, st, hipLaunchKernelGGL((k_finish_sorted<uint64_t, KS_TEXT, true>), dim3((unsigned)ft_tiles), dim3(FT_THREADS), 0, st,
                                                     (const uint64_t *)sorted0, SA, dT, Ptext, n, K, cap, w.surv_bits, surv_head, w.surv_cnt, w.total,
                                                     w.todo_bits, w.ft_cnt, w.ft_head));
            PROF(KC_RR_SCAN, ft_tiles, st, hipLaunchKernelGGL((k_rr_scan), dim3(1), dim3(SPINE_THREADS), 0, st, w.ft_cnt, w.ft_head, ft_tiles, w.total + 3));
            uint32_t cnt4[4] = { 0, 0, 0, 0 };
            {
                uint32_t words[64 + RR_CHG_COUNTERS * 32];
                const int rcw = read_words(words, w.total, sizeof(words), st); if (rcw) return rcw;
                cnt4[0] = words[0]; cnt4[1] = words[1]; cnt4[3] = words[3];
                for (int c = 0; c < RR_CHG_COUNTERS; ++c) cnt4[2] += words[64 + c * 32];
            }
            local.unresolved_after_initial = cnt4[2];
            const int64_t m_todo = cnt4[3];
            local.locally_sorted += (int64_t)cnt4[2] - m_todo;
            rkA = (sr.keys == w.keysA) ? w.keysB : w.keysA;
            rkB = w.keysC;
            if (m_todo > 0) {
                PROF(KC_RR_APPLY, n, st, hipLaunchKernelGGL((k_todo_compact<uint64_t>), dim3((unsigned)ft_tiles), dim3(FT_THREADS), 0, st,
                                                            (const uint64_t *)sorted0, (const uint32_t *)SA, n, (const uint32_t *)w.todo_bits,
                                                            (const uint32_t *)w.ft_cnt, (const uint32_t *)w.ft_head, (const uint32_t *)(w.total + 3),
                                                            Ucur, Gcur, Vcur));
                uint32_t *Valt = (Vcur == w.valsA) ? w.valsB : w.valsA;
                Refined rf;
                bool big_local = true;
                rc = refine_list(rkA, rkB, Vcur, Valt, Ucur, Gcur, Unext, Gnext, m_todo, n, dT, Ptext, K, g_bits, &big_local, w, st, &local, &rf, tn);
                if (rc) return rc;
                const int64_t tt = ceil_div(m_todo, RR_TILE);
                PROF(KC_RR_COUNT, m_todo, st, hipLaunchKernelGGL((k_rr_count<false>), dim3((unsigned)tt), dim3(RR_THREADS), 0, st, rf.keys,
                                                            (const uint32_t *)Ucur, m_todo, w.ft_cnt, w.ft_head, 0, (uint32_t *)nullptr, 0));
                PROF(KC_RR_SCAN, tt, st, hipLaunchKernelGGL((k_rr_scan), dim3(1), dim3(SPINE_THREADS), 0, st, w.ft_cnt, w.ft_head, tt, w.total + 4));
                PROF(KC_RR_APPLY, m_todo, st, hipLaunchKernelGGL((k_rr_apply<false, true, 4>), dim3((unsigned)tt), dim3(RR_THREADS), 0, st,
                                                            rf.keys, rf.vals, (const uint32_t *)Ucur, m_todo, (const uint32_t *)w.ft_cnt,
                                                            (const uint32_t *)w.ft_head, SA, surv_head, Unext, Gnext, rf.vnext, (uint32_t)n,
                                                            w.surv_bits, 0, (uint64_t *)nullptr, w.surv_cnt, (const uint32_t *)(w.total + 4), 0, (const uint32_t *)nullptr, 0, (uint32_t *)nullptr));
            }
            PROF(KC_RR_SCAN, tiles, st, hipLaunchKernelGGL((k_rr_scan), dim3(1), dim3(SPINE_THREADS), 0, st, w.surv_cnt, w.thead, tiles, w.total));
            { const int rcw = read_words(&m32, w.total, 4, st); if (rcw) return rcw; }
            m = m32;
            Ucur = w.U0; Gcur = w.G0; Vcur = w.valsA; Unext = w.U1; Gnext = w.G1;
            if (m > 0)
                PROF(KC_RR_APPLY, n, st, hipLaunchKernelGGL((k_surv_compact), dim3((unsigned)tiles), dim3(256), 0, st, (const uint32_t *)w.surv_bits,
                                                            (const uint32_t *)surv_head, (const uint32_t *)SA, n, (const uint32_t *)w.surv_cnt,
                                                            (const uint32_t *)w.total, Ucur, Gcur, Vcur));
            fused64 = true;
            lists_ready = true;
            depth += s_sym;
            local.text_rounds++;
            local.rounds++;
        }
        return SA_AMD_OK;
    }

    int group_heads()
    {
        int rc = SA_AMD_OK; (void)rc;
        if (!finished32 && !fused64) {
        if (top_shift)
            PROF(KC_RR_COUNT, n, st, hipLaunchKernelGGL((k_rr_count<true, uint32_t>), dim3((unsigned)tiles), dim3(RR_THREADS), 0, st, sorted32,
                                                        (const uint32_t *)nullptr, n, w.tcnt, w.thead, 0, (uint32_t *)nullptr, 0));
        else
            PROF(KC_RR_COUNT, n, st, hipLaunchKernelGGL((k_rr_count<true, uint64_t, true>), dim3((unsigned)tiles), dim3(RR_THREADS), 0, st, (const uint64_t *)sr.keys,
                                                        (const uint32_t *)nullptr, n, w.tcnt, w.thead, 0, w.tnext, 0));
        PROF(KC_RR_SCAN, tiles, st, hipLaunchKernelGGL((k_rr_scan), dim3(1), dim3(SPINE_THREADS), 0, st, w.tcnt, w.thead, tiles, w.total));
        { const int rcw = read_words(&m32, w.total, 4, st); if (rcw) return rcw; }
        m = m32;
        local.unresolved_after_initial = m;
        if (timing_only()) m = 0;
        }
        return SA_AMD_OK;
    }

    int finish_top32_ties()
    {
        int rc = SA_AMD_OK; (void)rc;
        if (!finished32 && top_shift && m > 0) {
            rkA = (sr.keys == w.keysA) ? w.keysB : w.keysA;
            rkB = w.keysC;
            PROF(KC_RR_APPLY, n, st, hipLaunchKernelGGL((k_rr_apply<true, false, 1, uint32_t>), dim3((unsigned)tiles), dim3(RR_THREADS), 0, st,
                                                        sorted32, (const uint32_t *)SA, (const uint32_t *)nullptr, n,
                                                        (const uint32_t *)w.tcnt, (const uint32_t *)w.thead, SA, w.isa, Ucur, Gcur, Vcur, 0u,
                                                        w.has_isa, 0, (uint64_t *)nullptr, (uint32_t *)nullptr, (const uint32_t *)w.total, 0, (const uint32_t *)nullptr, 0, (uint32_t *)nullptr));
            uint32_t *Valt = (Vcur == w.valsA) ? w.valsB : w.valsA;
            Refined rf;
            KeySrc K = KeySrc(); K.mode = KS_LOWKEY; K.kb = top_shift;
            rc = refine_list(rkA, rkB, Vcur, Valt, Ucur, Gcur, Unext, Gnext, m, n, dT, P, K, g_bits, &local_ok, w, st, &local, &rf, tn);
            if (rc) return rc;
            tiles = ceil_div(m, RR_TILE);
            PROF(KC_RR_COUNT, m, st, hipLaunchKernelGGL((k_rr_count<false>), dim3((unsigned)tiles), dim3(RR_THREADS), 0, st, rf.keys,
                                                        (const uint32_t *)Ucur, m, w.tcnt, w.thead, 0, (uint32_t *)nullptr, 0));
            PROF(KC_RR_SCAN, tiles, st, hipLaunchKernelGGL((k_rr_scan), dim3(1), dim3(SPINE_THREADS), 0, st, w.tcnt, w.thead, tiles, w.total));
            PROF(KC_RR_APPLY, m, st, hipLaunchKernelGGL((k_rr_apply<false, true, 3>), dim3((unsigned)tiles), dim3(RR_THREADS), 0, st,
                                                        rf.keys, rf.vals, (const uint32_t *)Ucur, m, (const uint32_t *)w.tcnt,
                                                        (const uint32_t *)w.thead, SA, w.isa, Unext, Gnext, rf.vnext, (uint32_t)n,
                                                        (uint32_t *)nullptr, 0, (uint64_t *)nullptr, (uint32_t *)nullptr,
                                                        (const uint32_t *)w.total, 0, (const uint32_t *)nullptr, 0, (uint32_t *)nullptr));
            { const int rcw = read_words(&m32, w.total, 4, st); if (rcw) return rcw; }
            m = m32;
            uint32_t *t;
            t = Ucur; Ucur = Unext; Unext = t;
            t = Gcur; Gcur = Gnext; Gnext = t;
            Vcur = rf.vnext;
            lists_ready = true;
            local.unresolved_after_initial = m;
        }
        return SA_AMD_OK;
    }

    int rank_setup_and_text_rounds()
    {
        int rc = SA_AMD_OK; (void)rc;
        key2_bits = bit_length((uint64_t)(2 * n));
        const int64_t sparse_div = tn.sparse_div;
        const int64_t sparse_limit = n / sparse_div;
        sparse = false;
        const bool dense_first = m > 0 && !lists_ready && (force_dense || (!text_ok && m > sparse_limit) || (probe_dense && m > sparse_limit));
        if (m > 0 && dense_first) {
            isa_tail_ranks = !tn.no_first_tail;
            if (isa_tail_ranks)
                PROF(KC_RR_SCAN, tiles, st, hipLaunchKernelGGL((k_rr_scan_next), dim3(1), dim3(SPINE_THREADS), 0, st, w.tnext, tiles, (uint32_t *)nullptr));
            if (binned(n, n, tn)) {
                uint64_t *pk = (sr.keys == w.keysA) ? w.keysB : w.keysA;
                const bool from_sa = !tn.setup_key_copy && (((uintptr_t)dSA) & 15) == 0;
                const size_t H = ((size_t)n + 1 + 3) & ~(size_t)3;
                uint32_t *pk32 = (uint32_t *)pk, *sk32 = (uint32_t *)sr.keys;
                uint64_t *pk_out = from_sa ? (uint64_t *)nullptr : pk;
                uint32_t *pv_out = from_sa ? pk32 + H + 1 : w.U1;
                if (isa_tail_ranks)
                    PROF(KC_RR_APPLY, n, st, hipLaunchKernelGGL((k_rr_apply<true, false, 2, uint64_t, true>), dim3((unsigned)tiles), dim3(RR_THREADS), 0, st,
                                                                sr.keys, (const uint32_t *)SA, (const uint32_t *)nullptr, n, w.tcnt, w.thead,
                                                                SA, w.isa, Ucur, Gcur, Vcur, (uint32_t)n, (uint32_t *)nullptr, 0, pk_out, pv_out, (const uint32_t *)w.total, 0, (const uint32_t *)w.tnext, 0, (uint32_t *)nullptr));
                else
                PROF(KC_RR_APPLY, n, st, hipLaunchKernelGGL((k_rr_apply<true, false, 2>), dim3((unsigned)tiles), dim3(RR_THREADS), 0, st,
                                                            sr.keys, (const uint32_t *)SA, (const uint32_t *)nullptr, n, w.tcnt, w.thead,
                                                            SA, w.isa, Ucur, Gcur, Vcur, (uint32_t)n, (uint32_t *)nullptr, 0, pk_out, pv_out, (const uint32_t *)w.total, 0, (const uint32_t *)nullptr, 0, (uint32_t *)nullptr));
                if (from_sa) {
                    hipLaunchKernelGGL(k_set_u32, dim3(1), dim3(1), 0, st, dSA, (uint32_t)n);
                    LAUNCH_CHECK(st);
                    rc = scatter_binned(dSA, pk32 + H, sk32, sk32 + H, n + 1, n, w, st, &local, tn, false, pk32);
                } else
                    rc = scatter_binned((uint32_t *)pk, w.U1, (uint32_t *)sr.keys, w.G1, n, n, w, st, &local, tn);
                if (rc) return rc;
            } else if (isa_tail_ranks) {
                PROF(KC_RR_APPLY, n, st, hipLaunchKernelGGL((k_rr_apply<true, false, 0, uint64_t, true>), dim3((unsigned)tiles), dim3(RR_THREADS), 0, st,
                                                            sr.keys, (const uint32_t *)SA, (const uint32_t *)nullptr, n, w.tcnt, w.thead,
                                                            SA, w.isa, Ucur, Gcur, Vcur, (uint32_t)n, (uint32_t *)nullptr, 0,
                                                            (uint64_t *)nullptr, (uint32_t *)nullptr, (const uint32_t *)w.total, 0, (const uint32_t *)w.tnext, 0, (uint32_t *)nullptr));
            } else {
                PROF(KC_RR_APPLY, n, st, hipLaunchKernelGGL((k_rr_apply<true, false, 0>), dim3((unsigned)tiles), dim3(RR_THREADS), 0, st,
                                                            sr.keys, (const uint32_t *)SA, (const uint32_t *)nullptr, n, w.tcnt, w.thead,
                                                            SA, w.isa, Ucur, Gcur, Vcur, (uint32_t)n, (uint32_t *)nullptr, 0,
                                                            (uint64_t *)nullptr, (uint32_t *)nullptr, (const uint32_t *)w.total, 0, (const uint32_t *)nullptr, 0, (uint32_t *)nullptr));
            }
        } else if (m > 0) {
            HIP_TRY(hipMemsetAsync(w.has_isa, 0, ((size_t)n + 31) / 32 * 4, st));
            if (!lists_ready) {
                rkA = (sr.keys == w.keysA) ? w.keysB : w.keysA;
                rkB = w.keysC;
                PROF(KC_RR_APPLY, n, st, hipLaunchKernelGGL((k_rr_apply<true, false, 1>), dim3((unsigned)tiles), dim3(RR_THREADS), 0, st,
                                                            (const uint64_t *)sorted0, (const uint32_t *)SA, (const uint32_t *)nullptr, n,
                                                            (const uint32_t *)w.tcnt, (const uint32_t *)w.thead, SA, w.isa, Ucur, Gcur, Vcur, 0u,
                                                            w.has_isa, 0, (uint64_t *)nullptr, (uint32_t *)nullptr, (const uint32_t *)w.total, 0, (const uint32_t *)nullptr, 0, (uint32_t *)nullptr));
            }
            bool progressing = true;

            bool counters_clear = false;
            while (text_ok && s_sym > 0 && m > sparse_limit && local.text_rounds < tn.max_text_rounds && progressing) {
                if ((rc = early_maybe_start())) return rc;
                const int64_t m_before = m;
                uint32_t *Valt = (Vcur == w.valsA) ? w.valsB : w.valsA;
                Refined rf;
                KeySrc K = KeySrc(); K.mode = KS_TEXT; K.h = depth; K.s = s_sym; K.kb = tkb;
                RoundCtl ctl;
                ctl.defer = prev_clean && local_ok && !tn.no_defer;
                ctl.counters_clear = counters_clear;
                rc = refine_list(rkA, rkB, Vcur, Valt, Ucur, Gcur, Unext, Gnext, m, n, dT, Ptext, K, g_bits, &local_ok, w, st, &local, &rf, tn, false, nullptr, &ctl);
                if (rc) return rc;
                uint32_t words[RC_WORDS];
                for (int attempt = 0; ; ++attempt) {
                    const uint32_t *gate = ctl.deferred ? (const uint32_t *)(w.total + RC_FLAGGED) : (const uint32_t *)nullptr;
                    tiles = ceil_div(m, RR_TILE);
                    PROF(KC_RR_COUNT, m, st, hipLaunchKernelGGL((k_rr_count<false>), dim3((unsigned)tiles), dim3(RR_THREADS), 0, st, rf.keys,
                                                                (const uint32_t *)Ucur, m, w.tcnt, w.thead, 0, (uint32_t *)nullptr, 0, gate));
                    PROF(KC_RR_SCAN, tiles, st, hipLaunchKernelGGL((k_rr_scan_round), dim3(2), dim3(SPINE_THREADS), 0, st, w.tcnt, w.thead, tiles, w.total,
                                                                   (uint32_t *)nullptr, (uint32_t *)nullptr, w.total + RC_BIG_LISTED, gate));
                    PROF(KC_RR_APPLY, m, st, hipLaunchKernelGGL((k_rr_apply<false, true, 3>), dim3((unsigned)tiles), dim3(RR_THREADS), 0, st,
                                                                rf.keys, rf.vals, (const uint32_t *)Ucur, m, (const uint32_t *)w.tcnt,
                                                                (const uint32_t *)w.thead, SA, w.isa, Unext, Gnext, rf.vnext,
                                                                (uint32_t)n, (uint32_t *)nullptr, 0, (uint64_t *)nullptr, (uint32_t *)nullptr,
                                                                (const uint32_t *)w.total, 0, (const uint32_t *)nullptr, 0, (uint32_t *)nullptr, gate));
                    { const int rcw = read_words(words, w.total, sizeof(words), st); if (rcw) return rcw; }
                    if (!ctl.deferred) break;
                    if (words[RC_FLAGGED] == 0) { ctl.m_flagged = 0; local.locally_sorted += m; break; }
                    if (attempt > 0) return SA_AMD_EINTERNAL;
                    uint32_t tot[RC_WORDS];
                    memcpy(tot, words, sizeof(tot));
                    ctl.resume_tot = tot; ctl.defer = false; ctl.deferred = false;
                    rc = refine_list(rkA, rkB, Vcur, Valt, Ucur, Gcur, Unext, Gnext, m, n, dT, Ptext, K, g_bits, &local_ok, w, st, &local, &rf, tn, false, nullptr, &ctl);
                    if (rc) return rc;
                    ctl.resume_tot = nullptr;
                }
                prev_clean = ctl.m_flagged == 0;
                counters_clear = true;
                uint32_t *Vnext = rf.vnext;
                m32 = words[0];
                m = m32;
                uint32_t *t;
                t = Ucur; Ucur = Unext; Unext = t;
                t = Gcur; Gcur = Gnext; Gnext = t;
                Vcur = Vnext;
                depth += s_sym;
                local.text_rounds++;
                local.rounds++;
                progressing = m * 4 <= m_before * 3;
                if (trace) fprintf(stderr, "suffix_array_amd: text round %d depth %lld: tied %lld -> %lld  (%.2f ms)\n", local.text_rounds, (long long)depth, (long long)m_before, (long long)m, lap());
            }
            if (m > sparse_limit) {
                int64_t blocks = ceil_div(n, 256);
                if (blocks > 16384) blocks = 16384;
                if (binned(n, n, tn) && (((uintptr_t)dSA) & 15) == 0) {
                    hipLaunchKernelGGL(k_set_u32, dim3(1), dim3(1), 0, st, dSA, (uint32_t)n);
                    LAUNCH_CHECK(st);
                    const size_t H = ((size_t)n + 1 + 3) & ~(size_t)3;
                    rc = scatter_binned(dSA, nullptr, (uint32_t *)rkB, (uint32_t *)rkB + H, n + 1, n, w, st, &local, tn, true,
                                        (uint32_t *)rkA, (uint32_t *)rkA + H);
                    if (rc) return rc;
                } else
                    PROF(KC_SCATTER, n, st, hipLaunchKernelGGL((k_isa_from_sa), dim3((unsigned)blocks), dim3(256), 0, st, (const uint32_t *)SA, w.isa, n));
                blocks = ceil_div(m, 256);
                if (blocks > 16384) blocks = 16384;
                PROF(KC_SCATTER, m, st, hipLaunchKernelGGL((k_isa_tied), dim3((unsigned)blocks), dim3(256), 0, st, (const uint32_t *)Vcur,
                                                           (const uint32_t *)Gcur, w.isa, m, n));
            } else {
                sparse = m > 0;
            }
        }
        local.sparse_mode = sparse ? 1 : 0;
        if (trace) fprintf(stderr, "suffix_array_amd: initial sort + text rounds + rank set-up done, %lld tied (%.2f ms since the last line)\n", (long long)m, lap());

        return SA_AMD_OK;
    }

    int doubling_rounds()
    {
        int rc = SA_AMD_OK; (void)rc;
        const int64_t depth_text = depth;
        int64_t h = depth;
        bool chase_ok = false;
        int split_rest = 0;
        bool parent_tail = isa_tail_ranks;
        int64_t changed_prev = isa_tail_ranks ? m : 0;
        int64_t m_local_off = m;
        int rounds_local_off = 0;
        bool all_small = false;
        bool counters_clear = false;
        const int sa_final = (!sparse && !tn.sa_every_round) ? 1 : 0;
        while (m > 0) {
            if (local.rounds >= 48) return SA_AMD_EINTERNAL;
            if ((rc = early_maybe_start())) return rc;
            uint32_t *Valt = (Vcur == w.valsA) ? w.valsB : w.valsA;
            KeySrc K = KeySrc();
            K.mode = sparse ? KS_SPARSE : KS_RANK; K.h = h; K.kb = key2_bits; K.isa = w.isa;
            if (!local_ok && !tn.no_local_sort && m * 2 < m_local_off) local_ok = true;
            const bool retry_local = !local_ok && ++rounds_local_off >= 3;
            K.iters = (!sparse && local_ok && chase_ok) ? (m >= tn.chase_big_min ? tn.chase_big : tn.chase) : 1;
            if (K.iters > 1) K.mode = KS_CHASE;
            K.has_isa = w.has_isa; K.sorted_keys = sorted0; K.sorted_top32 = sorted32; K.sa = SA; K.depth = depth_text; K.top_shift = top_shift;
            Refined rf;
            if (local_ok) { m_local_off = m; rounds_local_off = 0; }
            const int64_t expect = (!parent_tail || m < changed_prev) ? m : changed_prev;
            const bool bin = !sparse && binned(n, expect, tn);
            RoundCtl ctl;
            ctl.defer = prev_clean && !bin && local_ok && !tn.no_defer;
            ctl.skip_big = all_small;
            ctl.counters_clear = counters_clear;
            rc = refine_list(rkA, rkB, Vcur, Valt, Ucur, Gcur, Unext, Gnext, m, n, dT, P, K, g_bits, &local_ok, w, st, &local, &rf, tn, retry_local, &split_rest, &ctl);
            if (rc) return rc;
            uint32_t words[64 + RR_CHG_COUNTERS * 32];
            for (int attempt = 0; ; ++attempt) {
                if (retry_local && rf.m_global < m) { m_local_off = m; rounds_local_off = 0; }
                const uint64_t *keysS = rf.keys; const uint32_t *valsS = rf.vals; uint32_t *Vnext = rf.vnext;
                const uint32_t *gate = ctl.deferred ? (const uint32_t *)(w.total + RC_FLAGGED) : (const uint32_t *)nullptr;
                tiles = ceil_div(m, RR_TILE);
                if (sparse)
                    PROF(KC_RR_COUNT, m, st, hipLaunchKernelGGL((k_rr_count<false>), dim3((unsigned)tiles), dim3(RR_THREADS), 0, st, keysS, Ucur, m, w.tcnt,
                                       w.thead, 0, (uint32_t *)nullptr, 0, gate));
                else
                    PROF(KC_RR_COUNT, m, st, hipLaunchKernelGGL((k_rr_count<false, uint64_t, true>), dim3((unsigned)tiles), dim3(RR_THREADS), 0, st, keysS, Ucur, m,
                                       w.tcnt, w.thead, 0, w.tnext, key2_bits, gate));
                PROF(KC_RR_SCAN, tiles, st, hipLaunchKernelGGL((k_rr_scan_round), dim3(2), dim3(SPINE_THREADS), 0, st, w.tcnt, w.thead, tiles, w.total,
                                                               sparse ? (uint32_t *)nullptr : w.tnext, sparse ? (uint32_t *)nullptr : w.chg, w.total + RC_BIG_LISTED, gate));
                if (sparse) {
// ... 137 lines not shown
```

suffix_array_amd/csrc/host/tuning.hpp:

```cpp
#pragma once
#include <cstdlib>
#include <cstdint>
#include <atomic>

namespace sa {

constexpr int64_t SPARSE_DIV_DEFAULT = 64;
constexpr int GROUP_CAP_MAX = 1024;

inline bool env_flag(const char *name)
{
    const char *e = getenv(name);
    return e && *e && !(e[0] == '0' && e[1] == 0);
}

inline int64_t env_int(const char *name, int64_t def, int64_t lo, int64_t hi)
{
    const char *e = getenv(name);
    if (!e || !*e) return def;
    char *end = nullptr;
    const long long v = strtoll(e, &end, 10);
    if (end == e) return def;
    return v < lo ? lo : (v > hi ? hi : (int64_t)v);
}

inline int env_small_max() { return (int)env_int("SA_AMD_SMALL_MAX", 8192, 0, 8192); }

#ifdef SA_AMD_DIAG
inline std::atomic<int> g_rerank_routes{0};
#endif

struct Tuning {
    int sort_variant = 0;
    int sort32_variant = 0;
    int key_bits_max = 64;
    int group_cap = GROUP_CAP_MAX;
    int64_t sparse_div = SPARSE_DIV_DEFAULT;
    bool sparse_div_set = false;
    bool force_dense = false;
    bool no_text_rounds = false;
    bool no_local_sort = false;
    bool no_top32 = false;
    bool force_top32 = false;
    bool no_fused_finish = false;
    bool fused64 = false;
    bool no_packed_text = false;
    bool no_binned_isa = false;
    bool binned_isa_always = false;
    bool no_run_skip = false;
    int64_t run_skip_min = (int64_t)1 << 25;
    int64_t dense_rekey_min = (int64_t)1 << 22;
    bool no_first_tail = false;
    bool sa_every_round = false;
    bool setup_key_copy = false;
    bool no_repeat_probe = false;
    int64_t binned_min = (int64_t)1 << 26;
    int chase = 7;
    int chase_big = 3;
    int64_t chase_big_min = (int64_t)1 << 23;
    int scatter_levels = 0;
    int max_text_rounds = 4;
    bool no_split = false;
    int64_t split_min = (int64_t)1 << 22;
    int64_t split_group_min = (int64_t)1 << 15;
    bool no_gram_keys = false;
    int64_t gram_min_n = (int64_t)1 << 22;
    int gram_g = 0;
    int gram_tail_max = 8;
    int top32_partners_x100 = 50;
    int top32_collisions_x100 = 400;
    int64_t top32_probe_min_n = (int64_t)1 << 21;
    int small_max = 8192;
    bool no_onesweep = false;
    int onesweep_flags = 0;
    int onesweep64_shape = 0;
    int onesweep32_shape = 0;
    bool no_unary_shortcut = false;
    int64_t count_next_min_n = 20000000;
    int64_t count_next_below_n = 393216;
    int network_min = 256;
    bool no_upfront_counts = false;
    bool no_flat_rule = false;
    bool no_posted_readback = false;
    bool no_defer = false;
    bool no_big_group_sort = false;
    bool no_text_keys = false;
    bool no_value_bits = false;
    bool no_bucket_sort = false;
    int64_t bucket_min_n = (int64_t)1 << 25;
    bool no_bucket_finish = false;
    bool bucket_finish_always = false;
    int bucket_bits = 0;
    int bucket_shape = -1;
#ifdef SA_AMD_DIAG
    bool sample_sort = false;
    int64_t sample_sort_min_n = (int64_t)1 << 26;
    bool sample_merge = false;
    int sample_log = 0;
    bool timing_only_initial_sort = false;
#endif

    static Tuning from_env(int n_sort_variants, int n_sort32_variants, int n_os64 = 1, int n_os32 = 1)
    {
        Tuning t;
        t.sort_variant = (int)env_int("SA_AMD_SORT_VARIANT", 0, 0, 1 << 20);
        if (t.sort_variant >= n_sort_variants) t.sort_variant = 0;
        t.sort32_variant = (int)env_int("SA_AMD_SORT32_VARIANT", 0, 0, 1 << 20);
        if (t.sort32_variant >= n_sort32_variants) t.sort32_variant = 0;
        t.key_bits_max = (int)env_int("SA_AMD_KEY_BITS", 64, 16, 64);
        t.group_cap = (int)env_int("SA_AMD_GROUP_CAP", GROUP_CAP_MAX, 2, GROUP_CAP_MAX);
        t.sparse_div_set = getenv("SA_AMD_SPARSE_DIV") != nullptr;
        t.sparse_div = env_int("SA_AMD_SPARSE_DIV", SPARSE_DIV_DEFAULT, 1, (int64_t)1 << 40);
        t.force_dense = env_flag("SA_AMD_FORCE_DENSE");
        t.no_text_rounds = env_flag("SA_AMD_NO_TEXT_ROUNDS");
        t.no_local_sort = env_flag("SA_AMD_NO_LOCAL_SORT");
        t.no_top32 = env_flag("SA_AMD_NO_TOP32");
        t.force_top32 = env_flag("SA_AMD_FORCE_TOP32");
        t.no_fused_finish = env_flag("SA_AMD_NO_FUSED_FINISH");
        t.fused64 = env_flag("SA_AMD_FUSED64");
        t.no_packed_text = env_flag("SA_AMD_NO_PACKED_TEXT");
        t.no_binned_isa = env_flag("SA_AMD_NO_BINNED_ISA");
        t.binned_isa_always = env_flag("SA_AMD_BINNED_ISA_ALWAYS");
        t.no_run_skip = env_flag("SA_AMD_NO_RUN_SKIP");
        t.run_skip_min = env_int("SA_AMD_RUN_SKIP_MIN", (int64_t)1 << 25, 1, (int64_t)1 << 40);
        t.no_first_tail = env_flag("SA_AMD_NO_FIRST_TAIL");
        t.no_repeat_probe = env_flag("SA_AMD_NO_REPEAT_PROBE");
        t.dense_rekey_min = env_int("SA_AMD_DENSE_REKEY_MIN", (int64_t)1 << 22, 1, (int64_t)1 << 40);
        t.max_text_rounds = (int)env_int("SA_AMD_MAX_TEXT_ROUNDS", 4, 0, 8);
        t.chase = (int)env_int("SA_AMD_CHASE", 7, 1, 15);
        t.chase_big = (int)env_int("SA_AMD_CHASE_BIG", 3, 1, 15);
        t.chase_big_min = env_int("SA_AMD_CHASE_BIG_MIN", (int64_t)1 << 23, 1, (int64_t)1 << 40);
        t.scatter_levels = (int)env_int("SA_AMD_SCATTER_LEVELS", 0, 0, 2);
        t.binned_min = env_int("SA_AMD_BINNED_MIN", (int64_t)1 << 26, 1, (int64_t)1 << 40);
        t.no_split = env_flag("SA_AMD_NO_SPLIT");
        t.split_min = env_int("SA_AMD_SPLIT_MIN", (int64_t)1 << 22, 1, (int64_t)1 << 40);
        t.split_group_min = env_int("SA_AMD_SPLIT_GROUP_MIN", (int64_t)1 << 15, 1, (int64_t)1 << 40);
        t.no_gram_keys = env_flag("SA_AMD_NO_GRAM_KEYS");
        t.gram_min_n = env_int("SA_AMD_GRAM_MIN_N", (int64_t)1 << 22, 1, (int64_t)1 << 40);
        t.gram_g = (int)env_int("SA_AMD_GRAM_G", 0, 0, 8);
        t.gram_tail_max = (int)env_int("SA_AMD_GRAM_TAIL", 8, 0, 8);
        t.top32_partners_x100 = (int)env_int("SA_AMD_TOP32_PARTNERS_X100", 50, 0, 1000000);
        t.top32_collisions_x100 = (int)env_int("SA_AMD_TOP32_COLLISIONS_X100", 400, 0, 1000000);
        t.top32_probe_min_n = env_int("SA_AMD_TOP32_PROBE_MIN_N", (int64_t)1 << 21, 8192, (int64_t)1 << 40);
        t.small_max = env_small_max();
        t.no_onesweep = env_flag("SA_AMD_NO_ONESWEEP");
        t.onesweep_flags = (int)env_int("SA_AMD_ONESWEEP_FLAGS", 0, 0, 255);
        t.onesweep64_shape = (int)env_int("SA_AMD_ONESWEEP64_SHAPE", 0, 0, 1 << 20);
        if (t.onesweep64_shape >= n_os64) t.onesweep64_shape = 0;
        t.onesweep32_shape = (int)env_int("SA_AMD_ONESWEEP32_SHAPE", 0, 0, 1 << 20);
        if (t.onesweep32_shape >= n_os32) t.onesweep32_shape = 0;
        t.no_big_group_sort = env_flag("SA_AMD_NO_BIG_GROUP_SORT");
        t.no_defer = env_flag("SA_AMD_NO_DEFER");
        t.no_posted_readback = env_flag("SA_AMD_NO_POSTED_READBACK");
        t.no_flat_rule = env_flag("SA_AMD_NO_FLAT_RULE");
        t.no_upfront_counts = env_flag("SA_AMD_NO_UPFRONT_COUNTS");
        t.network_min = (int)env_int("SA_AMD_NETWORK_MIN", 256, 0, 1 << 20);
        t.count_next_min_n = env_int("SA_AMD_COUNT_NEXT_MIN_N", 20000000, 0, (int64_t)1 << 40);
        t.count_next_below_n = env_int("SA_AMD_COUNT_NEXT_BELOW_N", 393216, 0, (int64_t)1 << 40);
        t.no_unary_shortcut = env_flag("SA_AMD_NO_UNARY_SHORTCUT");

        t.no_text_keys = env_flag("SA_AMD_NO_TEXT_KEYS");
        t.no_value_bits = env_flag("SA_AMD_NO_VALUE_BITS");
        t.no_bucket_sort = env_flag("SA_AMD_NO_BUCKET_SORT");
        t.bucket_min_n = env_int("SA_AMD_BUCKET_MIN_N", (int64_t)1 << 25, 1, (int64_t)1 << 40);
        t.no_bucket_finish = env_flag("SA_AMD_NO_BUCKET_FINISH");
        t.bucket_finish_always = env_flag("SA_AMD_BUCKET_FINISH_ALWAYS");
        t.bucket_bits = (int)env_int("SA_AMD_BUCKET_BITS", 0, 0, 18);
        if (t.bucket_bits != 16 && t.bucket_bits != 18) t.bucket_bits = 0;
        t.bucket_shape = (int)env_int("SA_AMD_BUCKET_SHAPE", -1, -1, 64);
#ifdef SA_AMD_DIAG
        t.sample_sort = env_flag("SA_AMD_SAMPLE_SORT");
        t.sample_merge = env_flag("SA_AMD_SAMPLE_MERGE");
        t.sample_sort_min_n = env_int("SA_AMD_SAMPLE_SORT_MIN_N", (int64_t)1 << 26, (int64_t)1 << 17, (int64_t)1 << 40);
        t.sample_log = (int)env_int("SA_AMD_SAMPLE_LOG", 0, 0, 24);
        if (t.sample_log != 0 && t.sample_log < 16) t.sample_log = 16;
        t.timing_only_initial_sort = env_flag("SA_AMD_TIMING_ONLY_INITIAL_SORT");
        {
            const int r = g_rerank_routes.load(std::memory_order_relaxed);
            t.sa_every_round = (r & 1) != 0;
            t.setup_key_copy = (r & 2) != 0;
        }
#endif
        return t;
    }
};

constexpr size_t STAGE_BYTES = (size_t)16 << 20;

struct HostTuning {
    int small_max;
    int copy_threads;
    size_t staged_min;
    bool prefault;
    int prefault_keep;
    bool prefault_wait;
    int64_t early_div;
    size_t early_min;
    size_t early_chunk;
    int64_t early_wait;
    bool reduced;
    bool lanes;
    int64_t lanes_min_n;
    bool kernel_d2h;
    bool kernel_d2h_always;
    int verbose;

    static HostTuning from_env()
    {
        HostTuning h;
        h.small_max = env_small_max();
        h.copy_threads = (int)env_int("SA_AMD_COPY_THREADS", 12, 0, 32);
        h.staged_min = (size_t)env_int("SA_AMD_STAGED_MIN_BYTES", (int64_t)64 << 20, 0, (int64_t)1 << 40);
        h.prefault = env_int("SA_AMD_NO_PREFAULT", 0, 0, 1) == 0;
        h.prefault_keep = (int)env_int("SA_AMD_PREFAULT_KEEP", 3, 0, 32);
        h.prefault_wait = env_int("SA_AMD_PREFAULT_WAIT", 0, 0, 1) != 0;
        h.early_div = env_int("SA_AMD_EARLY_DIV", 4, 0, 1 << 20);
        h.early_min = (size_t)env_int("SA_AMD_EARLY_MIN_BYTES", (int64_t)128 << 20, 0, (int64_t)1 << 40);
        h.early_chunk = (size_t)env_int("SA_AMD_EARLY_CHUNK_BYTES", (int64_t)STAGE_BYTES, 65536, (int64_t)STAGE_BYTES) & ~(size_t)4095;
        h.early_wait = env_int("SA_AMD_EARLY_WAIT_CHUNKS", 0, 0, 1 << 20);
        h.reduced = env_int("SA_AMD_NO_REDUCED", 0, 0, 1) == 0;
        h.lanes = env_int("SA_AMD_NO_LANES", 0, 0, 1) == 0;
        h.lanes_min_n = env_int("SA_AMD_LANES_MIN_N", (int64_t)32 << 20, 0, (int64_t)1 << 40);
        h.kernel_d2h = env_int("SA_AMD_NO_KERNEL_D2H", 0, 0, 1) == 0;
        h.kernel_d2h_always = env_int("SA_AMD_KERNEL_D2H_ALWAYS", 0, 0, 1) != 0;
        h.verbose = (int)env_int("SA_AMD_VERBOSE", 0, 0, 9);
        return h;
    }
};

}
```

suffix_array_amd/csrc/kernels/onesweep.hpp:

```cpp
#pragma once
#include "common.hpp"
#include "radix_sort.hpp"

namespace sa {

constexpr int OS_NSEG = 8;
constexpr int OS_LB = 3;
struct __attribute__((packed, aligned(4))) Words4 { uint32_t x, y, z, w; };
constexpr int OS_MIN_TILE = 4096;

__device__ __forceinline__ unsigned os_xcc_id()
{
    return (unsigned)__builtin_amdgcn_s_getreg((3 << 11) | 20) & 7u;
}

typedef __attribute__((address_space(1))) unsigned long long os_gu64;

__device__ __forceinline__ uint32_t text_key32(const uint8_t *__restrict__ T, int64_t n, int64_t i)
{
    if (i + 8 <= n) {
        const uintptr_t a = (uintptr_t)(T + i);
        const uint32_t *W = (const uint32_t *)(a & ~(uintptr_t)3);
        const uint32_t lo = W[0], hi = W[1];
        const uint32_t le = __builtin_amdgcn_alignbyte(hi, lo, (uint32_t)(a & 3u));
        return __builtin_bswap32(le);
    }
    uint32_t k = 0;
#pragma unroll
    for (int b = 0; b < 4; ++b) k = (k << 8) | (i + b < n ? (uint32_t)T[i + b] : 0u);
    return k;
}

__global__ __launch_bounds__(SORT_THREADS) void k_text_upsweep32(const uint8_t *__restrict__ T, int64_t n, uint32_t *__restrict__ counts,
                                                                 int shift, uint32_t dmask, int64_t chunk_elems, int G, int split, int64_t sub_elems)
{
    __shared__ uint32_t h[SORT_WAVES][512];
    for (int i = threadIdx.x; i < SORT_WAVES * 512; i += SORT_THREADS) (&h[0][0])[i] = 0;
    __syncthreads();
    uint32_t *mine = h[wave_id()];
    const int g = (int)(blockIdx.x / split), part = (int)(blockIdx.x % split);
    const int64_t cbegin = (int64_t)g * chunk_elems;
    int64_t cend = cbegin + chunk_elems;
    if (cend > n) cend = n;
    int64_t begin = cbegin + (int64_t)part * sub_elems;
    int64_t end = begin + sub_elems;
    if (begin > cend) begin = cend;
    if (end > cend || part == split - 1) end = cend;
    int64_t i = begin + (int64_t)threadIdx.x * 16;
    for (; i + 16 <= end && i + 32 <= n; i += (int64_t)SORT_THREADS * 16) {
        const uintptr_t a = (uintptr_t)(T + i);
        const uint32_t *W = (const uint32_t *)(a & ~(uintptr_t)3);
        const uint32_t sh = (uint32_t)(a & 3u);
        const Words4 q = *(const Words4 *)W;
        const uint32_t w4 = W[4], w5 = W[5];
        const uint32_t v[6] = { __builtin_amdgcn_alignbyte(q.y, q.x, sh), __builtin_amdgcn_alignbyte(q.z, q.y, sh), __builtin_amdgcn_alignbyte(q.w, q.z, sh),
                                __builtin_amdgcn_alignbyte(w4, q.w, sh), __builtin_amdgcn_alignbyte(w5, w4, sh), 0u };
#pragma unroll
        for (int j = 0; j < 16; ++j) {
            const uint32_t key = __builtin_bswap32(__builtin_amdgcn_alignbyte(v[(j >> 2) + 1], v[j >> 2], (uint32_t)(j & 3)));
            atomicAdd(&mine[(key >> shift) & dmask], 1u);
        }
    }
    for (; i < end; i += (int64_t)SORT_THREADS * 16)
        for (int64_t p = i; p < i + 16 && p < end; ++p) atomicAdd(&mine[(text_key32(T, n, p) >> shift) & dmask], 1u);
    __syncthreads();
    for (int d = threadIdx.x; d <= (int)dmask; d += SORT_THREADS) {
        uint32_t sum = 0;
#pragma unroll
        for (int w = 0; w < SORT_WAVES; ++w) sum += h[w][d];
        if (sum) atomicAdd(&counts[(int64_t)d * G + g], sum);
    }
}

__global__ __launch_bounds__(256) void k_pack_text2(const uint8_t *__restrict__ T, int64_t n, KeyParams P, uint8_t *__restrict__ packed)
{
    __shared__ uint8_t lcode[256];
    lcode[threadIdx.x] = P.code[threadIdx.x];
    __syncthreads();
    const int64_t words = (n + 15) / 16;
    for (int64_t wi = (int64_t)blockIdx.x * 256 + threadIdx.x; wi < words; wi += (int64_t)gridDim.x * 256) {
        const int64_t p = wi * 16;
        uint32_t v = 0;
        if (p + 16 <= n && (((uintptr_t)(T + p)) & 15) == 0) {
            const uint4 q = *(const uint4 *)(T + p);
            const uint32_t w4[4] = { q.x, q.y, q.z, q.w };
#pragma unroll
            for (int j = 0; j < 16; ++j) v = (v << 2) | (uint32_t)lcode[(w4[j >> 2] >> (8 * (j & 3))) & 255u];
        } else {
#pragma unroll
            for (int j = 0; j < 16; ++j) v = (v << 2) | (p + j < n ? (uint32_t)lcode[T[p + j]] : 0u);
        }
        ((uint32_t *)packed)[wi] = __builtin_bswap32(v);
    }
}

__device__ __forceinline__ uint64_t packed_window64(const uint8_t *B)
{
    const uintptr_t a = (uintptr_t)B;
    const uint32_t *W = (const uint32_t *)(a & ~(uintptr_t)3);
    const uint32_t sh = (uint32_t)(a & 3u);
    const uint32_t w0 = W[0], w1 = W[1], w2 = W[2];
    const uint32_t v0 = __builtin_amdgcn_alignbyte(w1, w0, sh), v1 = __builtin_amdgcn_alignbyte(w2, w1, sh);
    return ((uint64_t)__builtin_bswap32(v0) << 32) | (uint64_t)__builtin_bswap32(v1);
}

__global__ __launch_bounds__(SORT_THREADS) void k_packed2_upsweep32(const uint8_t *__restrict__ packed, int64_t n, uint32_t *__restrict__ counts,
                                                                    int shift, uint32_t dmask, int64_t chunk_elems, int G, int split, int64_t sub_elems)
{
    __shared__ uint32_t h[SORT_WAVES][512];
    for (int i = threadIdx.x; i < SORT_WAVES * 512; i += SORT_THREADS) (&h[0][0])[i] = 0;
    __syncthreads();
    uint32_t *mine = h[wave_id()];
    const int g = (int)(blockIdx.x / split), part = (int)(blockIdx.x % split);
    const int64_t cbegin = (int64_t)g * chunk_elems;
    int64_t cend = cbegin + chunk_elems;
    if (cend > n) cend = n;
    int64_t begin = cbegin + (int64_t)part * sub_elems;
    int64_t end = begin + sub_elems;
    if (begin > cend) begin = cend;
    if (end > cend || part == split - 1) end = cend;
    for (int64_t i = begin + (int64_t)threadIdx.x * 16; i < end; i += (int64_t)SORT_THREADS * 16) {
        const uint64_t win = packed_window64(packed + (i >> 2));
#pragma unroll
        for (int j = 0; j < 16; ++j)
            if (i + j < end) atomicAdd(&mine[((uint32_t)(win >> (32 - 2 * j)) >> shift) & dmask], 1u);
    }
    __syncthreads();
    for (int d = threadIdx.x; d <= (int)dmask; d += SORT_THREADS) {
        uint32_t sum = 0;
#pragma unroll
        for (int w = 0; w < SORT_WAVES; ++w) sum += h[w][d];
        if (sum) atomicAdd(&counts[(int64_t)d * G + g], sum);
    }
}

struct OnesweepPass {
    const uint32_t *hist_cur;
    uint32_t *hist_next;
    uint32_t *tickets;
    unsigned long long *status;
    uint32_t *err;
    int64_t n;
    int shift, shift_next;
    uint32_t dmask, dmask_next;
    int nseg, tiles_per_seg, tiles;
    uint32_t epoch;
    const uint8_t *text;
    int64_t text_n;
    int text_bits;
    int val_extra;
    uint32_t flags;
};

template <int THREADS, int ITEMS, typename KeyT, bool SEQ, int WG_PER_CU, int RBITS = RADIX_BITS, bool TEXT_KEYS = false>
__global__ __launch_bounds__(THREADS, WG_PER_CU * THREADS / 256) void k_onesweep(
    const KeyT *__restrict__ keys_in, const uint32_t *__restrict__ vals_in, KeyT *__restrict__ keys_out, uint32_t *__restrict__ vals_out,
    OnesweepPass P)
{
    constexpr int RADIX = 1 << RBITS;
    constexpr int RADIX_BITS = RBITS;
    static_assert(RBITS == 8 || !SEQ, "the digits of the sequential shapes travel as bytes");
    static_assert(!TEXT_KEYS || sizeof(KeyT) == 4, "text keys are the top 32 key bits");
    constexpr int TILE = THREADS * ITEMS;
    constexpr int NWAVES = THREADS / WAVE;
    constexpr int WAVE_ELEMS = WAVE * ITEMS;
    static_assert(THREADS >= RADIX, "thread d owns digit d");
    static_assert(TILE < 65536, "16-bit tile-local counters");
    static_assert(ITEMS % 4 == 0, "digits are packed four to a register, tile positions two");
    __shared__ __attribute__((aligned(16))) KeyT lds_k[TILE];
    __shared__ __attribute__((aligned(16))) uint32_t lds_v_sep[SEQ ? 1 : TILE];
    __shared__ uint16_t wave_hist[NWAVES][RADIX];
    __shared__ uint32_t digit_base[RADIX];
    __shared__ uint32_t goff[RADIX];
    __shared__ uint32_t bnd[RADIX];
    __shared__ uint8_t seg0[RADIX];
    __shared__ uint32_t hist2[RADIX * OS_NSEG];
    __shared__ uint32_t scan_lds[NWAVES + 1];
    __shared__ int s_tile, s_seg;
    uint32_t *lds_v = SEQ ? (uint32_t *)lds_k : lds_v_sep;

    const int tid = threadIdx.x, l = lane_id(), w = wave_id();
    const unsigned xcc = os_xcc_id();
    const int nseg = P.nseg;
    const bool count_next = P.hist_next != nullptr;
    for (int i = tid; i < RADIX * OS_NSEG; i += THREADS) hist2[i] = 0;
    int cand = 0;
    int cur_seg = -1;
    uint32_t my_segbase = 0;
    uint16_t *my_hist = wave_hist[w];
    const int e0 = w * WAVE_ELEMS + l;
    const uint32_t seg_elems = (uint32_t)P.tiles_per_seg * (uint32_t)TILE;
    const unsigned long long tagA = ((unsigned long long)(P.epoch * 4u + 1u)) << 32, tagI = ((unsigned long long)(P.epoch * 4u + 2u)) << 32;
    os_gu64 *status = (os_gu64 *)P.status;
#ifdef SA_AMD_DIAG
    const bool stamping = (P.flags & 128u) != 0 && tid == 0;
    unsigned long long t_prev = stamping ? __builtin_amdgcn_s_memtime() : 0ull;
    auto stamp = [&](int phase) {
        if (stamping) {
            const unsigned long long now = __builtin_amdgcn_s_memtime();
            atomicAdd(&g_phase_cycles[phase], now - t_prev);
            t_prev = now;
        }
    };
#else
    auto stamp = [](int) {};
#endif

    const int own = ((int)xcc < nseg) ? (nseg - 1 - (int)xcc) / 8 + 1 : 0;
    auto cand_seg = [&](int c) { return c < own ? (int)xcc + 8 * c : c - own; };
    auto seg_tiles = [&](int s) { int cnt = P.tiles - s * P.tiles_per_seg; return cnt > P.tiles_per_seg ? P.tiles_per_seg : cnt; };
    auto take_ticket = [&](int *sg) -> int {
        while (cand < own + nseg) {
            const int s = cand_seg(cand), cnt = seg_tiles(s);
            if (cnt > 0) {
                const int k = (int)atomicAdd(&P.tickets[s], 1u);
                if (k < cnt) { *sg = s; return s * P.tiles_per_seg + k; }
            }
            ++cand;
        }
        *sg = -1;
        return -1;
    };
    int next_t = -1, next_seg = -1, pend_s = -1, pend_k = 0x7fffffff;
    if (tid == 0) next_t = take_ticket(&next_seg);
    for (;;) {
        if (tid == 0) { s_tile = next_t; s_seg = next_seg; }
        __syncthreads();
        const int t = s_tile, seg = s_seg;
        if (t < 0) break;
        if (tid == 0) {
            pend_s = cand < own + nseg ? cand_seg(cand) : -1;
            pend_k = (pend_s >= 0 && seg_tiles(pend_s) > 0) ? (int)atomicAdd(&P.tickets[pend_s], 1u) : 0x7fffffff;
        }
        const int seg_first = seg * P.tiles_per_seg;
        int e0v = e0, tidv = tid;
        asm volatile("" : "+v"(e0v), "+v"(tidv));
        int ebv = w * WAVE_ELEMS + l * ITEMS;
        asm volatile("" : "+v"(ebv));
#define OS_ELEM(j) (TEXT_KEYS ? ebv + (j) : e0v + (j) * WAVE)
        const int64_t base = (int64_t)t * TILE;
        const int valid = (P.n - base) >= TILE ? TILE : (int)(P.n - base);
        const bool full = valid == TILE;
        KeyT key[ITEMS];
        uint32_t val[ITEMS], pp[ITEMS / 2];
        uint32_t xpack = 0;
#define OS_POS(j) ((pp[(j) >> 1] >> (16 * ((j) & 1))) & 0xffffu)
        if (TEXT_KEYS && P.text_bits == 2) {
            const uint64_t win = packed_window64(P.text + ((base + ebv) >> 2));
#pragma unroll
            for (int j = 0; j < ITEMS; ++j) key[j] = (full || ebv + j < valid) ? (KeyT)(uint32_t)(win >> (32 - 2 * j)) : (KeyT)~(KeyT)0;
            if (P.val_extra) {
#pragma unroll
                for (int j = 0; j < ITEMS; ++j) xpack |= (((uint32_t)win >> (30 - 2 * j)) & 3u) << (2 * j);
            }
        } else if (TEXT_KEYS && base + TILE + 24 <= P.text_n) {
            static_assert(!TEXT_KEYS || (ITEMS <= 13 && ITEMS % 4 == 0), "ITEMS + 3 bytes out of five aligned words (2 ITEMS + 30 bits out of 64 for the packed text); a lane's first position is word-aligned relative to the tile");
            const uintptr_t a = (uintptr_t)(P.text + base + ebv);
            const uint32_t *W = (const uint32_t *)(a & ~(uintptr_t)3);
            const uint32_t sh = (uint32_t)(a & 3u);
            const Words4 q = *(const Words4 *)W;
            const uint32_t w4 = W[4];
            const uint32_t v0 = __builtin_amdgcn_alignbyte(q.y, q.x, sh), v1 = __builtin_amdgcn_alignbyte(q.z, q.y, sh),
                           v2 = __builtin_amdgcn_alignbyte(q.w, q.z, sh), v3 = __builtin_amdgcn_alignbyte(w4, q.w, sh);
            const uint32_t v[5] = { v0, v1, v2, v3, 0u };
#pragma unroll
            for (int j = 0; j < ITEMS; ++j)
                key[j] = (KeyT)__builtin_bswap32(__builtin_amdgcn_alignbyte(v[(j >> 2) + 1], v[j >> 2], (uint32_t)(j & 3)));
            if (P.val_extra) {
#pragma unroll
                for (int j = 0; j < ITEMS; ++j) xpack |= ((v[(j + 4) >> 2] >> (8 * ((j + 4) & 3) + 6)) & 3u) << (2 * j);
            }
        } else {
#pragma unroll
        for (int j = 0; j < ITEMS; ++j) {
            const int e = OS_ELEM(j);
            if (TEXT_KEYS) {
                key[j] = (full || e < valid) ? (KeyT)text_key32(P.text, P.text_n, base + e) : (KeyT)~(KeyT)0;
                if (P.val_extra && base + e + 4 < P.text_n) xpack |= ((uint32_t)P.text[base + e + 4] >> 6) << (2 * j);
            } else key[j] = (full || e < valid) ? keys_in[base + e] : (KeyT)~(KeyT)0;
        }
        }
        if (seg != cur_seg) {
            uint32_t tot = 0, below = 0;
            if (tid < RADIX) {
                for (int s = 0; s < nseg; ++s) {
                    const uint32_t c = P.hist_cur[tid * nseg + s];
                    if (s < seg) below += c;
                    tot += c;
                }
            }
            uint32_t all;
            const uint32_t dstart = block_excl_sum<THREADS>(tot, scan_lds, &all);
            my_segbase = dstart + below;
            cur_seg = seg;
        }
        for (int i = tid; i < NWAVES * RADIX / 2; i += THREADS) ((uint32_t *)&wave_hist[0][0])[i] = 0;
        __syncthreads();
        stamp(0);
#pragma unroll
        for (int j = 0; j < ITEMS; ++j) {
            const bool ok = full || OS_ELEM(j) < valid;
            const uint32_t d = digit_of(key[j], P.shift, P.dmask);
            const uint64_t okm = __ballot(ok);
            uint32_t xlo = ~(uint32_t)okm, xhi = ~(uint32_t)(okm >> 32);
#pragma unroll
            for (int b = 0; b < RADIX_BITS; ++b) {
                const uint32_t sel = (uint32_t)((int32_t)(d << (31 - b)) >> 31);
                const uint64_t bal = __ballot(sel != 0);
                xlo |= (uint32_t)bal ^ sel;
                xhi |= (uint32_t)(bal >> 32) ^ sel;
            }
            const uint32_t mlo = ~xlo, mhi = ~xhi;
            const uint32_t below = __builtin_amdgcn_mbcnt_hi(mhi, __builtin_amdgcn_mbcnt_lo(mlo, 0u));
            const uint32_t prior = my_hist[d];
            if (ok && below == 0) my_hist[d] = (uint16_t)(prior + (uint32_t)(__popc(mlo) + __popc(mhi)));
            if ((j & 1) == 0) pp[j >> 1] = prior + below; else pp[j >> 1] |= (prior + below) << 16;
            __builtin_amdgcn_sched_barrier(0);
        }
        stamp(1);
        auto load_vals = [&]() {
        if (vals_in) {
#pragma unroll
            for (int j = 0; j < ITEMS; ++j) {
                const int e = OS_ELEM(j);
                val[j] = (full || e < valid) ? vals_in[base + e] : 0u;
            }
        } else {
#pragma unroll
            for (int j = 0; j < ITEMS; ++j) val[j] = (uint32_t)(base + OS_ELEM(j));
            if (TEXT_KEYS && P.val_extra) {
                const int e = P.val_extra;
#pragma unroll
                for (int j = 0; j < ITEMS; ++j) val[j] |= (((xpack >> (2 * j)) & 3u) >> (2 - e)) << (32 - e);
            }
        }
        };
        if (!SEQ) load_vals();
        lds_barrier();
        stamp(2);
        uint32_t tot = 0;
        if (tid < RADIX) {
#pragma unroll
            for (int ww = 0; ww < NWAVES; ++ww) {
                const uint32_t cnt = wave_hist[ww][tid];
                wave_hist[ww][tid] = (uint16_t)tot;
                tot += cnt;
            }
        }
        unsigned long long lb[OS_LB];
        const bool walk = tid < RADIX && t > seg_first;
        const bool late_look = (P.flags & 1u) == 0;
        if (walk) {
            __hip_atomic_store(status + (int64_t)t * RADIX + tid, tagA | (unsigned long long)tot, __ATOMIC_RELAXED, __HIP_MEMORY_SCOPE_AGENT);
            if (!late_look) {
#pragma unroll
                for (int q = 0; q < OS_LB; ++q) {
                    const int k = t - 1 - q;
                    lb[q] = k >= seg_first ? __hip_atomic_load(status + (int64_t)k * RADIX + tid, __ATOMIC_RELAXED, __HIP_MEMORY_SCOPE_AGENT) : 0ull;
                }
            }
        }
        uint32_t tile_total;
        const uint32_t dbase = block_excl_sum_b<THREADS, true>(tot, scan_lds, &tile_total);
        if (tid < RADIX) digit_base[tid] = dbase;
        lds_barrier();
        stamp(3);
        uint32_t dpack[SEQ ? ITEMS / 4 : 1];
#pragma unroll
        for (int j = 0; j < ITEMS; ++j) {
            const uint32_t d = digit_of(key[j], P.shift, P.dmask);
            const uint32_t ps = OS_POS(j) + digit_base[d] + my_hist[d];
            if ((j & 1) == 0) pp[j >> 1] = (pp[j >> 1] & 0xffff0000u) | ps; else pp[j >> 1] = (pp[j >> 1] & 0xffffu) | (ps << 16);
            if (full || OS_ELEM(j) < valid) lds_k[ps] = key[j];
        }
        if (!SEQ) {
#pragma unroll
            for (int j = 0; j < ITEMS; ++j)
                if (full || OS_ELEM(j) < valid) lds_v[OS_POS(j)] = val[j];
        } else load_vals();
        if (walk && late_look) {
#pragma unroll
            for (int q = 0; q < OS_LB; ++q) {
                const int k = t - 1 - q;
                lb[q] = k >= seg_first ? __hip_atomic_load(status + (int64_t)k * RADIX + tid, __ATOMIC_RELAXED, __HIP_MEMORY_SCOPE_AGENT) : 0ull;
            }
        }
        stamp(4);
        if (tid < RADIX) {
            uint32_t g = my_segbase;
            if (walk) {
                uint32_t acc = 0;
                int k = t - 1;
                bool done = false;
                unsigned spins = 0;
                while (!done) {
#pragma unroll
                    for (int q = 0; q < OS_LB; ++q) {
                        if (done || k - q < seg_first) break;
                        unsigned long long x = lb[q];
                        for (;;) {
                            const unsigned long long tg = x & 0xffffffff00000000ull;
                            if (tg == tagI) { acc += (uint32_t)x; done = true; break; }
                            if (tg == tagA) { acc += (uint32_t)x; break; }
                            if (++spins > (1u << 22)) { atomicAdd(P.err, 1u); done = true; break; }
                            __builtin_amdgcn_s_sleep(2);
                            x = __hip_atomic_load(status + (int64_t)(k - q) * RADIX + tid, __ATOMIC_RELAXED, __HIP_MEMORY_SCOPE_AGENT);
                        }
                    }
                    k -= OS_LB;
                    if (!done) {
                        if (k < seg_first) { atomicAdd(P.err, 1u); break; }
#pragma unroll
                        for (int q = 0; q < OS_LB; ++q)
                            lb[q] = k - q >= seg_first ? __hip_atomic_load(status + (int64_t)(k - q) * RADIX + tid, __ATOMIC_RELAXED, __HIP_MEMORY_SCOPE_AGENT) : 0ull;
                    }
                }
                g = acc;
#ifdef SA_AMD_DIAG
                if ((P.flags & 128u) != 0 && tid == 7) {
                    atomicAdd(&g_phase_cycles[8], 1ull);
                    atomicAdd(&g_phase_cycles[9], (unsigned long long)(t - 1 - k));
                    atomicAdd(&g_phase_cycles[10], (unsigned long long)spins);
                }
#endif
            }
            __hip_atomic_store(status + (int64_t)t * RADIX + tid, tagI | (unsigned long long)(g + tot), __ATOMIC_RELAXED, __HIP_MEMORY_SCOPE_AGENT);
            goff[tid] = g - dbase;
            if (count_next) {
                const uint32_t s0 = g / seg_elems;
                seg0[tid] = (uint8_t)s0;
                bnd[tid] = (s0 + 1u) * seg_elems;
            }
        }
        __syncthreads();
        stamp(5);
#pragma unroll
        for (int j = 0; j < ITEMS; ++j) {
            const int idx = tidv + j * THREADS;
            const bool ok = full || idx < valid;
            KeyT kx = 0;
            uint32_t d = 0, gp = 0;
            if (SEQ && (j & 3) == 0) dpack[j >> 2] = 0;
            if (ok) {
                kx = lds_k[idx];
                d = digit_of(kx, P.shift, P.dmask);
                gp = goff[d] + (uint32_t)idx;
                keys_out[gp] = kx;
                if (!SEQ) vals_out[gp] = lds_v[idx];
                else dpack[j >> 2] |= d << (8 * (j & 3));
            }
            if (count_next) {
                const uint32_t slot = ok ? ((uint32_t)seg0[d] + (gp >= bnd[d] ? 1u : 0u)) * RADIX + digit_of(kx, P.shift_next, P.dmask_next) : 0u;
                const uint64_t act = __ballot(ok);
                const uint32_t f = (uint32_t)__builtin_amdgcn_readfirstlane((int)slot);
                if (__all(!ok || slot == f)) {
                    if (act && l == 0) atomicAdd(&hist2[f], (uint32_t)__popcll(act));
                } else if (ok) atomicAdd(&hist2[slot], 1u);
            }
        }
        stamp(6);
        if (SEQ) {
            lds_barrier();
#pragma unroll
            for (int j = 0; j < ITEMS; ++j)
                if (full || OS_ELEM(j) < valid) lds_v[OS_POS(j)] = val[j];
            lds_barrier();
#pragma unroll
            for (int j = 0; j < ITEMS; ++j) {
                const int idx = tidv + j * THREADS;
                if (full || idx < valid) {
                    const uint32_t d = (dpack[j >> 2] >> (8 * (j & 3))) & 255u;
                    vals_out[goff[d] + (uint32_t)idx] = lds_v[idx];
                }
            }
        }
        stamp(7);
#undef OS_POS
#undef OS_ELEM
        if (tid == 0) {
            if (pend_s >= 0 && pend_k < seg_tiles(pend_s)) { next_t = pend_s * P.tiles_per_seg + pend_k; next_seg = pend_s; }
            else { if (pend_s >= 0) ++cand; next_t = take_ticket(&next_seg); }
        }
    }
    if (count_next) {
        __syncthreads();
        for (int i = tid; i < RADIX * OS_NSEG; i += THREADS) {
            const uint32_t c = hist2[i];
            const int s = i / RADIX, d = i % RADIX;
            if (c && s < nseg) atomicAdd(&P.hist_next[d * nseg + s], c);
        }
    }
}

}
```

suffix_array_amd/csrc/kernels/rerank.hpp:

```cpp
#pragma once
#include "common.hpp"

namespace sa {

constexpr int RR_THREADS = 1024;
constexpr int RR_ITEMS = 8;
constexpr int RR_TILE = RR_THREADS * RR_ITEMS;

constexpr int RR_WAVE_ELEMS = WAVE * RR_ITEMS;

struct WaveGroups { uint64_t head[RR_ITEMS], tied[RR_ITEMS], valid[RR_ITEMS], phead[RR_ITEMS]; };

__device__ __forceinline__ uint64_t shfl64(uint64_t v, int src)
{
    return ((uint64_t)(uint32_t)__shfl((int)(uint32_t)(v >> 32), src, WAVE) << 32) | (uint32_t)__shfl((int)(uint32_t)v, src, WAVE);
}

template <typename KeyT, bool PARENTS = false>
__device__ __forceinline__ WaveGroups rr_wave_classify(const KeyT *__restrict__ keys, int64_t m, int64_t wbase, int key_shift, int g_shift = 0,
                                                       uint64_t *kout = nullptr)
{
    const int l = lane_id();
    uint64_t k[RR_ITEMS];
    WaveGroups g;
#pragma unroll
    for (int r = 0; r < RR_ITEMS; ++r) {
        const int64_t i = wbase + 64 * r + l;
        k[r] = i < m ? ((uint64_t)keys[i] >> key_shift) : 0ull;
        g.valid[r] = __ballot(i < m);
    }
    const uint64_t before = (wbase > 0 && wbase - 1 < m) ? ((uint64_t)keys[wbase - 1] >> key_shift) : 0ull;
    const uint64_t after = (wbase + RR_WAVE_ELEMS < m) ? ((uint64_t)keys[wbase + RR_WAVE_ELEMS] >> key_shift) : 0ull;
#pragma unroll
    for (int r = 0; r < RR_ITEMS; ++r) {
        uint64_t up = shfl64(k[r], l ? l - 1 : 0);
        const uint64_t prev_last = r ? shfl64(k[r ? r - 1 : 0], 63) : before;
        if (l == 0) up = prev_last;
        const int64_t i = wbase + 64 * r + l;
        g.head[r] = __ballot(i < m && (i == 0 || k[r] != up));
        g.phead[r] = PARENTS ? __ballot(i < m && (i == 0 || ((k[r] ^ up) >> g_shift) != 0ull)) : 0ull;
    }
    if (kout) {
#pragma unroll
        for (int r = 0; r < RR_ITEMS; ++r) kout[r] = k[r];
        kout[RR_ITEMS] = before;
    }
    const uint64_t last_key = shfl64(k[RR_ITEMS - 1], 63);
    const bool boundary_after = (wbase + RR_WAVE_ELEMS >= m) || after != last_key;
#pragma unroll
    for (int r = 0; r < RR_ITEMS; ++r) {
        const uint64_t bnd = g.head[r] | ~g.valid[r];
        const uint64_t bnd_next0 = (r + 1 < RR_ITEMS) ? ((g.head[(r + 1) % RR_ITEMS] | ~g.valid[(r + 1) % RR_ITEMS]) & 1ull)
                                                      : (boundary_after ? 1ull : 0ull);
        const uint64_t next = (bnd >> 1) | (bnd_next0 << 63);
        g.tied[r] = g.valid[r] & ~(g.head[r] & next);
    }
    return g;
}

constexpr uint32_t RR_NO_HEAD = 0xffffffffu;
constexpr int RR_CHG_COUNTERS = 16;
__device__ __forceinline__ uint32_t rr_first_head_code(const WaveGroups &g, int64_t wbase, int r_from)
{
    uint32_t code = RR_NO_HEAD;
#pragma unroll
    for (int r = RR_ITEMS - 1; r >= 0; --r) {
        if (r >= r_from && g.head[r]) {
            const int b = __builtin_ctzll(g.head[r]);
            code = ((uint32_t)(wbase + 64 * r + b) << 1) | (uint32_t)((g.phead[r] >> b) & 1ull);
        }
    }
    return code;
}

template <bool FIRST, typename KeyT = uint64_t, bool PARENTS = false>
__global__ __launch_bounds__(RR_THREADS) void k_rr_count(const KeyT *__restrict__ keys,
                                                          const uint32_t *__restrict__ U, int64_t m,
                                                          uint32_t *__restrict__ tile_cnt,
                                                          uint32_t *__restrict__ tile_head, int key_shift,
                                                          uint32_t *__restrict__ tile_first, int g_shift,
                                                          const uint32_t *__restrict__ gate = nullptr)
{
    __shared__ uint32_t wcnt[RR_THREADS / WAVE], whead[RR_THREADS / WAVE], wfirst[RR_THREADS / WAVE];
    if (gate && *gate) return;
    const int64_t wbase = (int64_t)blockIdx.x * RR_TILE + (int64_t)wave_id() * RR_WAVE_ELEMS;
    uint64_t kk[RR_ITEMS + 1];
    const WaveGroups g = rr_wave_classify<KeyT, false>(keys, m, wbase, key_shift, 0, PARENTS ? kk : nullptr);
    uint32_t cnt = 0, lasthead = 0;
#pragma unroll
    for (int r = 0; r < RR_ITEMS; ++r) {
        cnt += (uint32_t)__popcll(g.tied[r]);
        if (g.head[r]) {
            const int64_t i = wbase + 64 * r + (63 - __builtin_clzll(g.head[r]));
            lasthead = (FIRST ? (uint32_t)i : U[i]) + 1u;
        }
    }
    uint32_t first_code = RR_NO_HEAD;
    if (PARENTS) {
        bool found = false;
#pragma unroll
        for (int r = 0; r < RR_ITEMS; ++r) {
            if (!found && g.head[r]) {
                found = true;
                const int b = __builtin_ctzll(g.head[r]);
                const uint64_t mine = shfl64(kk[r], b);
                const uint64_t left = b ? shfl64(kk[r], b - 1) : (r ? shfl64(kk[r ? r - 1 : 0], 63) : kk[RR_ITEMS]);
                const int64_t i = wbase + 64 * r + b;
                const uint32_t ph = (i == 0 || ((mine ^ left) >> g_shift) != 0ull) ? 1u : 0u;
                first_code = ((uint32_t)i << 1) | ph;
            }
        }
    }
    if (lane_id() == 0) { wcnt[wave_id()] = cnt; whead[wave_id()] = lasthead; wfirst[wave_id()] = first_code; }
    __syncthreads();
    if (threadIdx.x == 0) {
        uint32_t tot = 0, mx = 0, fc = RR_NO_HEAD;
        for (int w = 0; w < RR_THREADS / WAVE; ++w) { tot += wcnt[w]; mx = mx > whead[w] ? mx : whead[w]; fc = fc < wfirst[w] ? fc : wfirst[w]; }
        tile_cnt[blockIdx.x] = tot;
        tile_head[blockIdx.x] = mx;
        if (PARENTS) tile_first[blockIdx.x] = fc;
    }
}

__device__ __forceinline__ void rr_scan_next_body(uint32_t *__restrict__ tile_first, int64_t tiles, uint32_t *__restrict__ changed_cnt)
{
    __shared__ uint32_t s_min[SPINE_THREADS];
    const int t = threadIdx.x;
    const int64_t per = (tiles + SPINE_THREADS - 1) / SPINE_THREADS;
    int64_t b = (int64_t)t * per, e = b + per;
    if (b > tiles) b = tiles;
    if (e > tiles) e = tiles;
    uint32_t mn = RR_NO_HEAD;
    for (int64_t i = b; i < e; ++i) { const uint32_t c = tile_first[i]; mn = mn < c ? mn : c; }
    s_min[t] = mn;
    __syncthreads();
    for (int o = 1; o < SPINE_THREADS; o <<= 1) {
        const uint32_t other = t + o < SPINE_THREADS ? s_min[t + o] : RR_NO_HEAD;
        __syncthreads();
        if (other < s_min[t]) s_min[t] = other;
        __syncthreads();
    }
    uint32_t run = t + 1 < SPINE_THREADS ? s_min[t + 1] : RR_NO_HEAD;
    for (int64_t i = e - 1; i >= b; --i) {
        const uint32_t c = tile_first[i];
        tile_first[i] = run;
        run = run < c ? run : c;
    }
    if (t < RR_CHG_COUNTERS && changed_cnt) changed_cnt[t * 32] = 0u;
}

__global__ __launch_bounds__(SPINE_THREADS) void k_rr_scan_next(uint32_t *__restrict__ tile_first, int64_t tiles, uint32_t *__restrict__ changed_cnt)
{
    rr_scan_next_body(tile_first, tiles, changed_cnt);
}

__device__ __forceinline__ void rr_scan_body(uint32_t *__restrict__ tile_cnt, uint32_t *__restrict__ tile_head, int64_t tiles,
                                             uint32_t *__restrict__ out_total)
{
    __shared__ uint32_t lds[SPINE_THREADS / WAVE + 1];
    const int64_t per = ((tiles + SPINE_THREADS - 1) / SPINE_THREADS + 3) & ~(int64_t)3;
    int64_t b = (int64_t)threadIdx.x * per, e = b + per;
    if (b > tiles) b = tiles;
    if (e > tiles) e = tiles;
    const int64_t ev = b + ((e - b) & ~(int64_t)3);
    const bool heads = tile_head != nullptr;
    uint32_t s = 0, mx = 0;
    for (int64_t i = b; i < ev; i += 4) {
        const uint4 c = *(const uint4 *)(tile_cnt + i);
        s += c.x + c.y + c.z + c.w;
        if (heads) { const uint4 h = *(const uint4 *)(tile_head + i); mx = max(max(mx, max(h.x, h.y)), max(h.z, h.w)); }
    }
    for (int64_t i = ev; i < e; ++i) { s += tile_cnt[i]; if (heads) mx = max(mx, tile_head[i]); }
    uint32_t tot, mtot;
    uint32_t off = block_excl_sum<SPINE_THREADS>(s, lds, &tot);
    uint32_t incm = block_incl_max<SPINE_THREADS>(mx, lds, &mtot);
    uint32_t prevm = __shfl_up(incm, 1, WAVE);
    __shared__ uint32_t wlast[SPINE_THREADS / WAVE];
    if (lane_id() == WAVE - 1) wlast[wave_id()] = incm;
    __syncthreads();
    if (lane_id() == 0) prevm = wave_id() ? wlast[wave_id() - 1] : 0u;
    uint32_t run = prevm;
    for (int64_t i = b; i < ev; i += 4) {
        const uint4 c = *(const uint4 *)(tile_cnt + i);
        uint4 oc;
        oc.x = off; off += c.x; oc.y = off; off += c.y; oc.z = off; off += c.z; oc.w = off; off += c.w;
        *(uint4 *)(tile_cnt + i) = oc;
        if (heads) {
            const uint4 h = *(const uint4 *)(tile_head + i);
            uint4 oh;
            oh.x = run; run = max(run, h.x); oh.y = run; run = max(run, h.y); oh.z = run; run = max(run, h.z); oh.w = run; run = max(run, h.w);
            *(uint4 *)(tile_head + i) = oh;
        }
    }
    for (int64_t i = ev; i < e; ++i) {
        const uint32_t c = tile_cnt[i];
        tile_cnt[i] = off; off += c;
        if (heads) { const uint32_t h = tile_head[i]; tile_head[i] = run; run = run > h ? run : h; }
    }
    if (threadIdx.x == 0) *out_total = tot;
}

__global__ __launch_bounds__(SPINE_THREADS) void k_rr_scan(uint32_t *__restrict__ tile_cnt,
                                                            uint32_t *__restrict__ tile_head, int64_t tiles,
                                                            uint32_t *__restrict__ out_total)
{
    rr_scan_body(tile_cnt, tile_head, tiles, out_total);
}

__global__ __launch_bounds__(SPINE_THREADS) void k_rr_scan_pair(uint32_t *__restrict__ cntA, uint32_t *__restrict__ headA, uint32_t *__restrict__ outA,
                                                                 uint32_t *__restrict__ cntB, uint32_t *__restrict__ headB, uint32_t *__restrict__ outB,
                                                                 int64_t tiles)
{
    if (blockIdx.x == 0) rr_scan_body(cntA, headA, tiles, outA);
    else rr_scan_body(cntB, headB, tiles, outB);
}

__global__ __launch_bounds__(SPINE_THREADS) void k_rr_scan_round(uint32_t *__restrict__ tile_cnt, uint32_t *__restrict__ tile_head, int64_t tiles,
                                                                  uint32_t *__restrict__ out_total, uint32_t *__restrict__ tile_first,
                                                                  uint32_t *__restrict__ changed_cnt, uint32_t *__restrict__ clear2,
                                                                  const uint32_t *__restrict__ gate)
{
    if (gate && *gate) return;
    if (blockIdx.x == 0) { rr_scan_body(tile_cnt, tile_head, tiles, out_total); return; }
    if (tile_first) rr_scan_next_body(tile_first, tiles, changed_cnt);
    if (threadIdx.x == 0 && clear2) { clear2[2] = clear2[0]; clear2[3] = clear2[1]; clear2[0] = 0u; clear2[1] = 0u; }
}

template <bool FIRST, bool WRITE_SA, int ISA_MODE, typename KeyT = uint64_t, bool FTAIL = false>
__global__ __launch_bounds__(RR_THREADS) void k_rr_apply(
    const KeyT *__restrict__ keys, const uint32_t *__restrict__ V, const uint32_t *__restrict__ U, int64_t m,
    const uint32_t *__restrict__ tile_cnt, const uint32_t *__restrict__ tile_head, uint32_t *__restrict__ SA,
    uint32_t *__restrict__ ISA, uint32_t *__restrict__ Uo, uint32_t *__restrict__ Go, uint32_t *__restrict__ Vo,
    uint32_t n_text, uint32_t *__restrict__ has_isa, int g_shift, uint64_t *__restrict__ pair_k,
    uint32_t *__restrict__ pair_v, const uint32_t *__restrict__ tile_total, int key_shift,
    const uint32_t *__restrict__ tile_next, int parent_tail, uint32_t *__restrict__ changed_cnt,
    const uint32_t *__restrict__ gate = nullptr,
    int sa_final = 0)
{
    constexpr bool SPARSE = ISA_MODE == 1;
    if (gate && *gate) return;
    constexpr bool TAIL = (FIRST ? FTAIL : true) && (ISA_MODE == 0 || ISA_MODE == 2);
    constexpr bool COUNT_CHANGED = TAIL && !FIRST;
    constexpr int NW = RR_THREADS / WAVE;
    __shared__ uint32_t wcnt[NW], whead[NW], wfirst[NW];
    __shared__ uint32_t s_chg;
    if (COUNT_CHANGED && threadIdx.x == 0) s_chg = 0;
    if (FIRST && !WRITE_SA && SPARSE) {
        const uint32_t here = tile_cnt[blockIdx.x];
        const uint32_t next = (blockIdx.x + 1 < gridDim.x) ? tile_cnt[blockIdx.x + 1] : *tile_total;
        if (next == here) return;
    }
    const int l = lane_id(), w = wave_id();
    const int64_t wbase = (int64_t)blockIdx.x * RR_TILE + (int64_t)w * RR_WAVE_ELEMS;
    const WaveGroups g = rr_wave_classify<KeyT, TAIL>(keys, m, wbase, key_shift, g_shift);
    uint32_t slot[RR_ITEMS], v[RR_ITEMS];
#pragma unroll
    for (int r = 0; r < RR_ITEMS; ++r) {
        const int64_t i = wbase + 64 * r + l;
        const bool in = i < m;
        slot[r] = FIRST ? (uint32_t)i : (in ? U[i] : 0u);
        v[r] = in ? V[i] : 0u;
    }
    {
        uint32_t cnt = 0, lasthead = 0;
#pragma unroll
        for (int r = 0; r < RR_ITEMS; ++r) {
            cnt += (uint32_t)__popcll(g.tied[r]);
            if (g.head[r]) lasthead = (uint32_t)__shfl((int)slot[r], 63 - __builtin_clzll(g.head[r]), WAVE) + 1u;
        }
        if (l == 0) { wcnt[w] = cnt; whead[w] = lasthead; wfirst[w] = TAIL ? rr_first_head_code(g, wbase, 0) : RR_NO_HEAD; }
    }
    __syncthreads();
    uint32_t run_cnt = tile_cnt[blockIdx.x], run_head = tile_head[blockIdx.x];
    for (int ww = 0; ww < w; ++ww) { run_cnt += wcnt[ww]; run_head = run_head > whead[ww] ? run_head : whead[ww]; }
    uint32_t next_code[RR_ITEMS];
    uint32_t n_changed = 0;
    if (TAIL) {
        uint32_t behind = tile_next[blockIdx.x];
        for (int ww = NW - 1; ww > w; --ww) behind = wfirst[ww] != RR_NO_HEAD ? wfirst[ww] : behind;
        if (behind == RR_NO_HEAD) behind = ((uint32_t)m << 1) | 1u;
#pragma unroll
        for (int r = RR_ITEMS - 1; r >= 0; --r) {
            next_code[r] = behind;
            if (g.head[r]) {
                const int b = __builtin_ctzll(g.head[r]);
                behind = ((uint32_t)(wbase + 64 * r + b) << 1) | (uint32_t)((g.phead[r] >> b) & 1ull);
            }
        }
    }
    const uint64_t le_mask = (l == 63) ? ~0ull : ((2ull << l) - 1ull);
    const uint64_t lt_mask = le_mask >> 1;
    auto code_behind = [&](int r) -> uint32_t {
        const uint64_t hgt = (l == 63) ? 0ull : (g.head[r] & (~0ull << (l + 1)));
        if (!hgt) return next_code[r];
        const int b = __builtin_ctzll(hgt);
        return ((uint32_t)(wbase + 64 * r + b) << 1) | (uint32_t)((g.phead[r] >> b) & 1ull);
    };
    constexpr bool PAIRS = COUNT_CHANGED && ISA_MODE == 2;
    uint64_t cmask[PAIRS ? RR_ITEMS : 1];
    uint32_t pair_off = 0;
    if (PAIRS) {
        __shared__ uint32_t wpairs[NW];
        __shared__ uint32_t s_base;
        uint32_t mine = 0;
#pragma unroll
        for (int r = 0; r < RR_ITEMS; ++r) {
            const int64_t i = wbase + 64 * r + l;
            cmask[r] = __ballot(i < m && !(parent_tail && (code_behind(r) & 1u)));
            mine += (uint32_t)__popcll(cmask[r]);
        }
        if (l == 0) wpairs[w] = mine;
        __syncthreads();
        if (threadIdx.x == 0) {
            uint32_t tot = 0;
            for (int ww = 0; ww < NW; ++ww) tot += wpairs[ww];
            s_base = tot ? atomicAdd(&changed_cnt[0], tot) : 0u;
        }
        __syncthreads();
        pair_off = s_base;
        for (int ww = 0; ww < w; ++ww) pair_off += wpairs[ww];
    }
#pragma unroll
    for (int r = 0; r < RR_ITEMS; ++r) {
        const int64_t i = wbase + 64 * r + l;
        const uint64_t hle = g.head[r] & le_mask;
        const int src = hle ? 63 - __builtin_clzll(hle) : 0;
        const uint32_t hslot = (uint32_t)__shfl((int)slot[r], src, WAVE);
        const uint32_t run = hle ? hslot + 1u : run_head;
        const uint32_t off = run_cnt + (uint32_t)__popcll(g.tied[r] & lt_mask);
        uint32_t rank = run;
        bool changed = true;
        if (TAIL) {
            const uint32_t code = code_behind(r);
            rank = slot[r] + ((code >> 1) - 1u - (uint32_t)i) + 1u;
            changed = !(parent_tail && (code & 1u));
            if (COUNT_CHANGED && !PAIRS) n_changed += (uint32_t)__popcll(__ballot(i < m && changed));
        }
        if (i < m) {
            if (WRITE_SA && slot[r] < n_text && !(sa_final && ((g.tied[r] >> l) & 1ull))) SA[slot[r]] = v[r];
            if (PAIRS) {
                if (changed) {
                    const uint32_t o = pair_off + (uint32_t)__popcll(cmask[r] & lt_mask);
                    ((uint32_t *)pair_k)[o] = v[r];
                    pair_v[o] = rank;
                }
            } else if (ISA_MODE == 2) {
                if (pair_k) ((uint32_t *)pair_k)[i] = v[r];
                pair_v[i] = rank;
            } else if (ISA_MODE != 3 && ISA_MODE != 4 && v[r] < n_text) {
                if (changed) {
                    ISA[v[r]] = rank;
                    if (SPARSE) atomicOr(&has_isa[v[r] >> 5], 1u << (v[r] & 31u));
                }
            }
            if ((g.tied[r] >> l) & 1ull) {
                if (ISA_MODE == 4) {
                    ISA[slot[r]] = run - 1u;
                    atomicOr(&has_isa[slot[r] >> 5], 1u << (slot[r] & 31u));
                    atomicAdd(&pair_v[slot[r] / RR_TILE], 1u);
                } else {
                    Uo[off] = slot[r]; Go[off] = run - 1u; Vo[off] = v[r];
                }
            }
        }
        run_cnt += (uint32_t)__popcll(g.tied[r]);
        if (g.head[r]) run_head = (uint32_t)__shfl((int)slot[r], 63 - __builtin_clzll(g.head[r]), WAVE) + 1u;
        if (PAIRS) pair_off += (uint32_t)__popcll(cmask[r]);
    }
    if (COUNT_CHANGED && !PAIRS) {
        if (l == 0 && n_changed) atomicAdd(&s_chg, n_changed);
        __syncthreads();
        if (threadIdx.x == 0 && s_chg) atomicAdd(&changed_cnt[(blockIdx.x % RR_CHG_COUNTERS) * 32], s_chg);
    }
}

}
```

suffix_array_amd/csrc/sa_diag.h:

```cpp
#ifndef SUFFIX_ARRAY_AMD_DIAG_H
#define SUFFIX_ARRAY_AMD_DIAG_H
#include "../../include/suffix_array_amd.h"
#ifdef __cplusplus
extern "C" {
#endif
int32_t sa_amd_debug_phase_cycles(uint64_t *out, int32_t count);
int32_t sa_amd_debug_group_sort_stamps(int32_t on);
int32_t sa_amd_debug_rerank_routes(int32_t flags);
int32_t sa_amd_debug_sort_variant_count(void);
const char *sa_amd_debug_sort_variant_name(int32_t index);
int32_t sa_amd_test_sort_pairs(uint64_t *keys, uint32_t *vals, int64_t count, int32_t begin_bit, int32_t end_bit);
int32_t sa_amd_test_sample_sort64(uint64_t *keys, uint32_t *vals, int64_t count, int32_t key_bits, int32_t *done);
int32_t sa_amd_test_sort_pairs32(uint32_t *keys, uint32_t *vals, int64_t count, int32_t begin_bit, int32_t end_bit);
int32_t sa_amd_test_bucket_sort32(uint32_t *keys, uint32_t *vals, int64_t count, int32_t top_bits, uint32_t *largest);
int32_t sa_amd_test_build_keys(const uint8_t *T, int32_t n, uint64_t *keys, int32_t *bits, int32_t *k);
int32_t sa_amd_proto_induce_l(const uint8_t *T, const uint8_t *typeL, uint32_t *SA, int32_t n, const uint32_t *head,
                              double *ms, uint64_t *counters);
#ifdef __cplusplus
}
#endif
#endif
```

suffix_array_amd/csrc/sa_diag.inc:

```

SA_EXPORT int32_t sa_amd_debug_phase_cycles(uint64_t *out, int32_t count)
{
    unsigned long long h[16] = { 0 };
    if (hipMemcpyFromSymbol(h, HIP_SYMBOL(sa::g_phase_cycles), sizeof(h)) != hipSuccess) return SA_AMD_EHIP;
    for (int i = 0; i < count && i < 16; ++i) out[i] = h[i];
    unsigned long long z[16] = { 0 };
    (void)hipMemcpyToSymbol(HIP_SYMBOL(sa::g_phase_cycles), z, sizeof(z));
    return 16;
}

SA_EXPORT int32_t sa_amd_debug_group_sort_stamps(int32_t on)
{
    const int v = on ? 1 : 0;
    return hipMemcpyToSymbol(HIP_SYMBOL(sa::g_gs_stamp_on), &v, sizeof(v)) == hipSuccess ? SA_AMD_OK : SA_AMD_EHIP;
}

SA_EXPORT int32_t sa_amd_debug_rerank_routes(int32_t flags)
{
    return sa::g_rerank_routes.exchange(flags & 3);
}

SA_EXPORT int32_t sa_amd_debug_sort_variant_count(void) { return sa::N_SORT_VARIANTS; }
SA_EXPORT const char *sa_amd_debug_sort_variant_name(int32_t i)
{
    return (i >= 0 && i < sa::N_SORT_VARIANTS) ? sa::sort_variants[i].name : "";
}

SA_EXPORT int32_t sa_amd_test_sort_pairs(uint64_t *keys, uint32_t *vals, int64_t count, int32_t begin_bit, int32_t end_bit)
{
    using namespace sa;
    if (count < 0 || (count > 0 && (!keys || !vals)) || begin_bit < 0 || end_bit > 64) return SA_AMD_EINVAL;
    if (sa_amd_device_count() <= 0) return SA_AMD_ENODEVICE;
    if (count == 0) return SA_AMD_OK;
    const Tuning tn = Tuning::from_env(N_SORT_VARIANTS, N_SORT32_VARIANTS, N_OS_SHAPES64, N_OS_SHAPES32);
    const size_t N = (size_t)count;
    DevBuf dk, dv, dsp;
    int32_t rc;
    if ((rc = dk.alloc(N * 8 * 2))) return rc;
    if ((rc = dv.alloc(N * 4 * 2))) return rc;
    if ((rc = dsp.alloc(((size_t)RADIX * SORT_MAX_WG + RADIX) * 4))) return rc;
    uint64_t *k = dk.as<uint64_t>(); uint32_t *v = dv.as<uint32_t>(), *spine = dsp.as<uint32_t>();
    HIP_TRY(hipMemcpy(k, keys, N * 8, hipMemcpyHostToDevice));
    HIP_TRY(hipMemcpy(v, vals, N * 4, hipMemcpyHostToDevice));
    SortResult sr;
    DevBuf dst;
    if ((rc = dst.alloc(((size_t)ceil_div(count, OS_MIN_TILE) + 1) * RADIX * 8 + 256))) return rc;
    HIP_TRY(hipMemset(dst.p, 0, 256));
    SortScratch ss; ss.spine = spine; ss.digit_tot = spine + (size_t)RADIX * SORT_MAX_WG;
    ss.err = dst.as<uint32_t>(); ss.status = (unsigned long long *)(dst.as<char>() + 256);
    rc = sort_pairs(k, v, k + N, v + N, count, begin_bit, end_bit, ss, nullptr, nullptr, &sr, tn);
    if (rc != SA_AMD_OK) return rc;
    HIP_TRY(hipDeviceSynchronize());
    HIP_TRY(hipMemcpy(keys, sr.keys, N * 8, hipMemcpyDeviceToHost));
    HIP_TRY(hipMemcpy(vals, sr.vals, N * 4, hipMemcpyDeviceToHost));
    { uint32_t e = 0; HIP_TRY(hipMemcpy(&e, ss.err, 4, hipMemcpyDeviceToHost)); if (e) return SA_AMD_EINTERNAL; }
    return SA_AMD_OK;
}

SA_EXPORT int32_t sa_amd_test_sample_sort64(uint64_t *keys, uint32_t *vals, int64_t count, int32_t key_bits, int32_t *done)
{
    using namespace sa;
    if (count <= 0 || !keys || !vals || !done || key_bits < 1 || key_bits > 64) return SA_AMD_EINVAL;
    if (sa_amd_device_count() <= 0) return SA_AMD_ENODEVICE;
    const Tuning tn = Tuning::from_env(N_SORT_VARIANTS, N_SORT32_VARIANTS, N_OS_SHAPES64, N_OS_SHAPES32);
    const size_t N = (size_t)count;
    DevBuf dk, dv, dsp, dst, dbig, dsmall;
    int32_t rc;
    if ((rc = dk.alloc((N + 64) * 8 * 3))) return rc;
    if ((rc = dv.alloc(N * 4 * 5))) return rc;
    if ((rc = dsp.alloc(((size_t)RADIX * SORT_MAX_WG + RADIX) * 4))) return rc;
    if ((rc = dst.alloc(((size_t)ceil_div(count, OS_MIN_TILE) + 1) * RADIX * 8 + 256))) return rc;
    if ((rc = dbig.alloc(((size_t)ceil_div(count, SS_TILE) + SS_WAYS) * SS_IDS2 * 4))) return rc;
    if ((rc = dsmall.alloc((size_t)8 << 20))) return rc;
    HIP_TRY(hipMemset(dst.p, 0, 256));
    uint64_t *k = dk.as<uint64_t>();
    uint32_t *v = dv.as<uint32_t>(), *spine = dsp.as<uint32_t>();
    HIP_TRY(hipMemcpy(k, keys, N * 8, hipMemcpyHostToDevice));
    SortScratch ss; ss.spine = spine; ss.digit_tot = spine + (size_t)RADIX * SORT_MAX_WG;
    ss.err = dst.as<uint32_t>(); ss.status = (unsigned long long *)(dst.as<char>() + 256);
    sa_amd_stats local;
    memset(&local, 0, sizeof(local));
    bool ok = false;
    uint32_t *words = dsmall.as<uint32_t>() + ((size_t)6 << 18);
    rc = sample_sort64(k, k + (N + 64), k + 2 * (N + 64), v, v + N, v + 2 * N, v + 3 * N, dbig.as<uint32_t>(), dsmall.as<uint32_t>(), words,
                       v + 4 * N, count, key_bits, ss, nullptr, &local, tn, &ok, false);
    if (rc != SA_AMD_OK) return rc;
    HIP_TRY(hipDeviceSynchronize());
    *done = ok ? 1 : 0;
    if (ok) {
        HIP_TRY(hipMemcpy(keys, k + (N + 64), N * 8, hipMemcpyDeviceToHost));
        HIP_TRY(hipMemcpy(vals, v + 4 * N, N * 4, hipMemcpyDeviceToHost));
    }
    { uint32_t e = 0; HIP_TRY(hipMemcpy(&e, ss.err, 4, hipMemcpyDeviceToHost)); if (e) return SA_AMD_EINTERNAL; }
    return SA_AMD_OK;
}

SA_EXPORT int32_t sa_amd_test_sort_pairs32(uint32_t *keys, uint32_t *vals, int64_t count, int32_t begin_bit, int32_t end_bit)
{
    using namespace sa;
    if (count < 0 || (count > 0 && (!keys || !vals)) || begin_bit < 0 || end_bit > 32) return SA_AMD_EINVAL;
    if (sa_amd_device_count() <= 0) return SA_AMD_ENODEVICE;
    if (count == 0) return SA_AMD_OK;
    const Tuning tn = Tuning::from_env(N_SORT_VARIANTS, N_SORT32_VARIANTS, N_OS_SHAPES64, N_OS_SHAPES32);
    const size_t N = ((size_t)count + 3) & ~(size_t)3;
    DevBuf dk, dv, dsp;
    int32_t rc;
    if ((rc = dk.alloc(N * 4 * 2))) return rc;
    if ((rc = dv.alloc(N * 4 * 2))) return rc;
    if ((rc = dsp.alloc(((size_t)RADIX * SORT_MAX_WG + RADIX) * 4))) return rc;
    uint32_t *k = dk.as<uint32_t>(), *v = dv.as<uint32_t>(), *spine = dsp.as<uint32_t>();
    HIP_TRY(hipMemcpy(k, keys, (size_t)count * 4, hipMemcpyHostToDevice));
    HIP_TRY(hipMemcpy(v, vals, (size_t)count * 4, hipMemcpyHostToDevice));
    SortResult32 sr;
    DevBuf dst;
    if ((rc = dst.alloc(((size_t)ceil_div(count, OS_MIN_TILE) + 1) * RADIX * 8 + 256))) return rc;
    HIP_TRY(hipMemset(dst.p, 0, 256));
    SortScratch ss; ss.spine = spine; ss.digit_tot = spine + (size_t)RADIX * SORT_MAX_WG;
    ss.err = dst.as<uint32_t>(); ss.status = (unsigned long long *)(dst.as<char>() + 256);
    rc = sort_pairs32(k, v, k + N, v + N, count, begin_bit, end_bit, ss, nullptr, nullptr, &sr, tn);
    if (rc != SA_AMD_OK) return rc;
    HIP_TRY(hipDeviceSynchronize());
    HIP_TRY(hipMemcpy(keys, sr.keys, (size_t)count * 4, hipMemcpyDeviceToHost));
    HIP_TRY(hipMemcpy(vals, sr.vals, (size_t)count * 4, hipMemcpyDeviceToHost));
    { uint32_t e = 0; HIP_TRY(hipMemcpy(&e, ss.err, 4, hipMemcpyDeviceToHost)); if (e) return SA_AMD_EINTERNAL; }
    return SA_AMD_OK;
}

__global__ void k_test_count_digit(const uint32_t *keys, int64_t n, int shift, uint32_t dmask, uint32_t *counts, int64_t chunk_elems, int G)
{
    for (int64_t i = (int64_t)blockIdx.x * blockDim.x + threadIdx.x; i < n; i += (int64_t)gridDim.x * blockDim.x)
        atomicAdd(&counts[(int64_t)((keys[i] >> shift) & dmask) * G + i / chunk_elems], 1u);
}

SA_EXPORT int32_t sa_amd_test_bucket_sort32(uint32_t *keys, uint32_t *vals, int64_t count, int32_t top_bits, uint32_t *largest)
{
    using namespace sa;
    if (count < 0 || (count > 0 && (!keys || !vals)) || !largest || (top_bits != 16 && top_bits != 18)) return SA_AMD_EINVAL;
    if (sa_amd_device_count() <= 0) return SA_AMD_ENODEVICE;
    *largest = 0;
    if (count == 0) return SA_AMD_OK;
    const Tuning tn = Tuning::from_env(N_SORT_VARIANTS, N_SORT32_VARIANTS, N_OS_SHAPES64, N_OS_SHAPES32);
    const size_t N = ((size_t)count + 3) & ~(size_t)3;
    DevBuf dk, dv, dsp, dst, dbs;
    int32_t rc;
    if ((rc = dk.alloc(N * 4 * 2))) return rc;
    if ((rc = dv.alloc(N * 4 * 3))) return rc;
    if ((rc = dsp.alloc(((size_t)RADIX * SORT_MAX_WG + RADIX) * 4))) return rc;
    if ((rc = dst.alloc(((size_t)ceil_div(count, OS_MIN_TILE) + 1) * RADIX * 8 + 256))) return rc;
    if ((rc = dbs.alloc(((size_t)BK_BUCKETS_MAX + 1) * 4))) return rc;
    uint32_t *k = dk.as<uint32_t>(), *v = dv.as<uint32_t>(), *spine = dsp.as<uint32_t>();
    HIP_TRY(hipMemcpy(k, keys, (size_t)count * 4, hipMemcpyHostToDevice));
    HIP_TRY(hipMemcpy(v, vals, (size_t)count * 4, hipMemcpyHostToDevice));
    HIP_TRY(hipMemset(dst.p, 0, 256));
    SortScratch ss; ss.spine = spine; ss.digit_tot = spine + (size_t)RADIX * SORT_MAX_WG;
    ss.err = dst.as<uint32_t>(); ss.status = (unsigned long long *)(dst.as<char>() + 256);
    SortResult32 sr;
    const int rbits = top_bits == 18 ? 9 : RADIX_BITS;
    bool counted = false;
    if (rbits == 9) {
        const FirstCounts fc = sort_first_counts(ss, tn, count, true);
        HIP_TRY(hipMemset(fc.zero_ptr, 0, fc.zero_bytes));
        hipLaunchKernelGGL(k_test_count_digit, dim3(256), dim3(256), 0, nullptr, (const uint32_t *)k, count, 32 - top_bits, 511u, fc.counts, fc.chunk_elems, fc.G);
        HIP_TRY(hipGetLastError());
        counted = true;
    }
    rc = sort_pairs32(k, v, k + N, v + N, count, 32 - top_bits, 32, ss, nullptr, nullptr, &sr, tn, false, counted, rbits);
    if (rc != SA_AMD_OK) return rc;
    uint32_t *kout = sr.keys == k ? k + N : k, *vout = v + 2 * N;
    bool done = false;
    rc = bucket_sort32(sr.keys, sr.vals, kout, vout, count, top_bits, dbs.as<uint32_t>(), ss.err + 2, nullptr, tn, &done, largest);
    if (rc != SA_AMD_OK) return rc;
    HIP_TRY(hipDeviceSynchronize());
    { uint32_t e[4] = { 0, 0, 0, 0 }; HIP_TRY(hipMemcpy(e, ss.err, 16, hipMemcpyDeviceToHost)); if (e[0] || e[3]) return SA_AMD_EINTERNAL; }
// ... 74 lines not shown
```

Baseline: 5576 MB/s.

## Build re-rank setup from group-head bitmap and fuse first-pass counts

The first re-rank count kernel now also writes a bitmap of group heads into the has_isa buffer, which is widened to 64-bit words. A new apply kernel reconstructs tied groups and ranks from that bitmap instead of re-reading and comparing 64-bit sorted keys. When possible it also builds the first radix-pass digit histogram, so the scatter sort can skip its counting pass. An optional path, off by default, derives pair values inside the first onesweep pass. This saves key traffic and a counting pass in exchange for more complex kernels and a reuse of the has_isa buffer.

```diff
diff --git a/suffix_array_amd/csrc/host/pipeline.hpp b/suffix_array_amd/csrc/host/pipeline.hpp
--- a/suffix_array_amd/csrc/host/pipeline.hpp
+++ b/suffix_array_amd/csrc/host/pipeline.hpp
@@ -104,7 +104,7 @@
     w.bk_start = (uint32_t *)take(((size_t)BK_BUCKETS_MAX + 1) * 4);
     w.early_cnt = (uint32_t *)take(((N + 1 + EARLY_TILE - 1) / EARLY_TILE + 8) * 4);
     w.gram_table = (uint4 *)take((gram_entries / 64 + 1) * 16);
-    w.has_isa = (uint32_t *)take((N + 31) / 32 * 4);
+    w.has_isa = (uint32_t *)take((N + 63) / 64 * 8);
     w.surv_bits = (uint32_t *)take((N + 31) / 32 * 4);
     w.todo_bits = (uint32_t *)take((N + 31) / 32 * 4);
     w.early_bits = (uint32_t *)take(((N + 1 + 31) / 32 + EARLY_THREADS) * 4);
@@ -158,6 +158,8 @@
     return g;
 }
 
+struct HeadVals { const uint64_t *bits; const uint32_t *next; int64_t n; int tiles; };
+static_assert(OS_HEAD_SPAN == RR_TILE, "head_next is the per-tile table of the re-rank kernels");
 struct FirstCounts { uint32_t *counts; int64_t chunk_elems; int G; void *zero_ptr; size_t zero_bytes; };
 static FirstCounts sort_first_counts(const SortScratch &ss, const Tuning &tn, int64_t count, bool keys32);
 
@@ -211,13 +213,16 @@
                                const uint8_t *text = nullptr, int64_t text_n = 0,
                                int text_bits = 8,
                                int val_extra = 0,
-                               KeyT *keys_out2 = nullptr)
+                               KeyT *keys_out2 = nullptr,
+                               const HeadVals *hv = nullptr)
 {
     constexpr int TILE = THREADS * ITEMS;
     constexpr int R = 1 << RBITS;
     static_assert(R <= OS_MAX_RADIX && (RBITS == RADIX_BITS || TILE >= 2 * OS_MIN_TILE), "zones and granule slab are sized for 8-bit digits of 4 Ki-element tiles");
     static_assert(TILE >= OS_MIN_TILE, "the granule slab is sized for tiles of at least OS_MIN_TILE elements");
     constexpr bool K64 = sizeof(KeyT) == 8;
+    constexpr bool HV_OK = !K64 && !SEQ && RBITS == RADIX_BITS && THREADS == 1024 && ITEMS == 12;
+    if (hv && (!HV_OK || text || iota)) return SA_AMD_EINTERNAL;
     OnesweepGeom g = onesweep_geom(count, TILE);
     auto zone = [&](int i) { return ss.spine + (size_t)i * OS_ZONE; };
     int z = 0;
@@ -287,8 +292,14 @@
         P.epoch = ++epoch;
         P.flags = (uint32_t)tn.onesweep_flags;
         P.text = text; P.text_n = text_n; P.text_bits = text_bits;
+        P.head_bits = (const unsigned long long *)(hv ? hv->bits : nullptr); P.head_next = hv ? hv->next : nullptr;
+        P.head_n = hv ? hv->n : 0; P.head_tiles = hv ? hv->tiles : 0;
         P.val_extra = (text && *passes == 0 && iota) ? val_extra : 0;
-        if (!K64 && !SEQ && text && *passes == 0)
+        if (HV_OK && hv && *passes == 0)
+            PROF(KC_ONESWEEP32, count, st,
+                 hipLaunchKernelGGL((k_onesweep<THREADS, ITEMS, KeyT, SEQ, WG_PER_CU, RBITS, false, HV_OK>), dim3(grid), dim3(THREADS), 0, st, (const KeyT *)kin,
+                                    (const uint32_t *)nullptr, kout, vdst, P));
+        else if (!K64 && !SEQ && text && *passes == 0)
             PROF(KC_ONESWEEP32, count, st,
                  hipLaunchKernelGGL((k_onesweep<THREADS, ITEMS, KeyT, SEQ, WG_PER_CU, RBITS, !K64 && !SEQ>), dim3(grid), dim3(THREADS), 0, st, (const KeyT *)kin,
                                     (const uint32_t *)((iota && *passes == 0) ? nullptr : vin), kout, vdst, P));
@@ -419,10 +430,12 @@
                         int rbits = RADIX_BITS,
                         const uint8_t *text = nullptr, int64_t text_n = 0, int text_bits = 8,
                         int val_extra = 0,
-                        uint32_t *keys_out2 = nullptr)
+                        uint32_t *keys_out2 = nullptr,
+                        const HeadVals *hv = nullptr)
 {
     res->keys = keys_in; res->vals = vals_in; res->passes = 0;
     if (keys_out2 && (rbits != RADIX_BITS || text)) return SA_AMD_EINTERNAL;
+    if (hv && (count <= 1 || end_bit <= begin_bit || rbits != RADIX_BITS || text || !onesweep_on(ss, tn) || tn.onesweep32_shape != 0)) return SA_AMD_EINTERNAL;
     if (count <= 1 || end_bit <= begin_bit) return SA_AMD_OK;
     if (rbits != RADIX_BITS && (rbits != 9 || !onesweep_on(ss, tn) || !first_counted)) return SA_AMD_EINTERNAL;
     if (text && (!onesweep_on(ss, tn) || !first_counted || tn.onesweep32_shape != 0)) return SA_AMD_EINTERNAL;
@@ -436,7 +449,7 @@
                                                                               &res->keys, &res->vals, &res->passes, &skipped, tn, iota, false, first_counted, text, text_n, text_bits, val_extra);
 #define OS_CALL32(T, I, S) sort_pairs_onesweep<uint32_t, T, I, S>(keys_in, vals_in, keys_alt, vals_alt, count, begin_bit, end_bit, ss, final_vals, st, \
                                                                  &res->keys, &res->vals, &res->passes, &skipped, tn, iota, false, first_counted, \
-                                                                 nullptr, 0, 8, 0, keys_out2)
+                                                                 nullptr, 0, 8, 0, keys_out2, hv)
         switch (tn.onesweep32_shape) {
         case 1: return OS_CALL32(512, 16, true);
         case 2: return OS_CALL32(512, 12, false);
@@ -754,15 +767,36 @@
     return n >= ((int64_t)1 << 25) && (count >= n || count >= tn.binned_min);
 }
 
+struct BinPlan { int nb, wlog; bool two; int shift; uint32_t dmask; bool recounts; };
+static BinPlan scatter_plan(int64_t count, int64_t n, const Tuning &tn)
+{
+    BinPlan bp;
+    bp.nb = bit_length((uint64_t)(n > 1 ? n : 1));
+    bp.wlog = bp.nb - 16;
+    if (bp.wlog < 10) bp.wlog = 10;
+    if (bp.wlog > 15) bp.wlog = 15;
+    bp.two = bp.nb > bp.wlog && (tn.scatter_levels == 2 || (tn.scatter_levels == 0 && count >= ((int64_t)1 << 25)));
+    if (bp.two) {
+        const int bits = bp.nb - bp.wlog < RADIX_BITS ? bp.nb - bp.wlog : RADIX_BITS;
+        bp.shift = bp.wlog; bp.dmask = (1u << bits) - 1u;
+    } else {
+        bp.shift = bp.nb > RADIX_BITS ? bp.nb - RADIX_BITS : 0; bp.dmask = (uint32_t)RADIX - 1u;
+    }
+    const int npass = bp.two ? (int)ceil_div(bp.nb - bp.wlog, RADIX_BITS) : 1;
+    bp.recounts = !tn.no_upfront_counts && count < tn.count_next_min_n && npass >= 2;
+    return bp;
+}
+
 static int scatter_binned(uint32_t *pk, uint32_t *pv, uint32_t *altk, uint32_t *altv, int64_t count, int64_t n,
                           const Workspace &w, hipStream_t st, sa_amd_stats *local, const Tuning &tn, bool iota = false,
-                          uint32_t *altk2 = nullptr, uint32_t *altv2 = nullptr)
-{
-    const int nb = bit_length((uint64_t)(n > 1 ? n : 1));
-    int wlog = nb - 16;
-    if (wlog < 10) wlog = 10;
-    if (wlog > 15) wlog = 15;
-    const bool two = nb > wlog && (tn.scatter_levels == 2 || (tn.scatter_levels == 0 && count >= ((int64_t)1 << 25)));
+                          uint32_t *altk2 = nullptr, uint32_t *altv2 = nullptr,
+                          bool first_counted = false,
+                          const HeadVals *hv = nullptr)
+{
+    const BinPlan bp = scatter_plan(count, n, tn);
+    const int nb = bp.nb, wlog = bp.wlog;
+    const bool two = bp.two;
+    if ((first_counted || hv) && iota) return SA_AMD_EINTERNAL;
     SortResult32 pr;
     if (two) {
         int rc;
@@ -778,7 +812,7 @@
                 local->sort_passes += pr.passes; local->sorted_elements += (int64_t)pr.passes * count;
             }
         } else {
-            rc = sort_pairs32(pk, pv, altk, altv, count, wlog, nb, w.ss, nullptr, st, &pr, tn, false, false, RADIX_BITS, nullptr, 0, 8, 0, altk2);
+            rc = sort_pairs32(pk, pv, altk, altv, count, wlog, nb, w.ss, nullptr, st, &pr, tn, false, first_counted, RADIX_BITS, nullptr, 0, 8, 0, altk2, hv);
             if (rc) return rc;
             local->sort_passes += pr.passes; local->sorted_elements += (int64_t)pr.passes * count;
         }
@@ -791,8 +825,8 @@
                                                            (const uint32_t *)pr.vals, w.isa, count, (uint32_t)n, wlog));
         return SA_AMD_OK;
     }
-    const int shift = nb > RADIX_BITS ? nb - RADIX_BITS : 0;
-    int rc = sort_pairs32(pk, pv, altk, altv, count, shift, shift + RADIX_BITS, w.ss, nullptr, st, &pr, tn, iota);
+    const int shift = bp.shift;
+    int rc = sort_pairs32(pk, pv, altk, altv, count, shift, shift + RADIX_BITS, w.ss, nullptr, st, &pr, tn, iota, first_counted, RADIX_BITS, nullptr, 0, 8, 0, nullptr, hv);
     if (rc) return rc;
     local->sort_passes += pr.passes; local->sorted_elements += (int64_t)pr.passes * count;
     PROF(KC_SCATTER, count, st, hipLaunchKernelGGL((k_scatter_pairs<uint32_t>), dim3((unsigned)ceil_div(count, 1024)), dim3(256), 0, st,
@@ -1126,6 +1160,7 @@
     uint32_t m32 = 0;
     bool lists_ready = false, finished32 = false, fused64 = false, sparse = false;
     bool isa_tail_ranks = false;
+    bool head_bits_ready = false;
     int s_sym = 0, tkb = 0, key2_bits = 0;
     bool unary_done = false;
     bool prev_clean = true;
@@ -1604,8 +1639,10 @@
             PROF(KC_RR_COUNT, n, st, hipLaunchKernelGGL((k_rr_count<true, uint32_t>), dim3((unsigned)tiles), dim3(RR_THREADS), 0, st, sorted32,
                                                         (const uint32_t *)nullptr, n, w.tcnt, w.thead, 0, (uint32_t *)nullptr, 0));
         else
-            PROF(KC_RR_COUNT, n, st, hipLaunchKernelGGL((k_rr_count<true, uint64_t, true>), dim3((unsigned)tiles), dim3(RR_THREADS), 0, st, (const uint64_t *)sr.keys,
-                                                        (const uint32_t *)nullptr, n, w.tcnt, w.thead, 0, w.tnext, 0));
+            PROF(KC_RR_COUNT, n, st, hipLaunchKernelGGL((k_rr_count<true, uint64_t, true, true>), dim3((unsigned)tiles), dim3(RR_THREADS), 0, st, (const uint64_t *)sr.keys,
+                                                        (const uint32_t *)nullptr, n, w.tcnt, w.thead, 0, w.tnext, 0, (const uint32_t *)nullptr,
+                                                        (uint64_t *)w.has_isa));
+        head_bits_ready = !top_shift;
         PROF(KC_RR_SCAN, tiles, st, hipLaunchKernelGGL((k_rr_scan), dim3(1), dim3(SPINE_THREADS), 0, st, w.tcnt, w.thead, tiles, w.total));
         { const int rcw = read_words(&m32, w.total, 4, st); if (rcw) return rcw; }
         m = m32;
@@ -1670,7 +1707,19 @@
                 uint32_t *pk32 = (uint32_t *)pk, *sk32 = (uint32_t *)sr.keys;
                 uint64_t *pk_out = from_sa ? (uint64_t *)nullptr : pk;
                 uint32_t *pv_out = from_sa ? pk32 + H + 1 : w.U1;
-                if (isa_tail_ranks)
+                const FirstCounts fc = sort_first_counts(w.ss, tn, n + 1, true);
+                const bool from_bits = isa_tail_ranks && from_sa && head_bits_ready && !tn.setup_from_keys && fc.chunk_elems >= RR_TILE;
+                bool setup_counted = false;
+                const bool ranks_in_pass = from_bits && onesweep_on(w.ss, tn) && tn.onesweep32_shape == 0 && tn.setup_ranks_in_pass;
+                const HeadVals hvals = { (const uint64_t *)w.has_isa, (const uint32_t *)w.tnext, n, (int)tiles };
+                if (from_bits) {
+                    const BinPlan bp = scatter_plan(n + 1, n, tn);
+                    setup_counted = !bp.recounts;
+                    if (setup_counted) HIP_TRY(hipMemsetAsync(fc.zero_ptr, 0, fc.zero_bytes, st));
+                    PROF(KC_RR_APPLY, n, st, hipLaunchKernelGGL((k_rr_apply_bits), dim3((unsigned)ceil_div(tiles, RB_TPW)), dim3(RR_THREADS), 0, st,
+                                                                (const uint64_t *)w.has_isa, (const uint32_t *)SA, n, (const uint32_t *)w.tcnt, (const uint32_t *)w.thead,
+                                                                (const uint32_t *)w.tnext, Ucur, Gcur, Vcur, ranks_in_pass ? (uint32_t *)nullptr : pv_out, setup_counted ? fc.counts : (uint32_t *)nullptr, fc.chunk_elems, fc.G, bp.shift, bp.dmask, (uint32_t)n));
+                } else if (isa_tail_ranks)
                     PROF(KC_RR_APPLY, n, st, hipLaunchKernelGGL((k_rr_apply<true, false, 2, uint64_t, true>), dim3((unsigned)tiles), dim3(RR_THREADS), 0, st,
                                                                 sr.keys, (const uint32_t *)SA, (const uint32_t *)nullptr, n, w.tcnt, w.thead,
                                                                 SA, w.isa, Ucur, Gcur, Vcur, (uint32_t)n, (uint32_t *)nullptr, 0, pk_out, pv_out, (const uint32_t *)w.total, 0, (const uint32_t *)w.tnext, 0, (uint32_t *)nullptr));
@@ -1678,10 +1727,13 @@
                 PROF(KC_RR_APPLY, n, st, hipLaunchKernelGGL((k_rr_apply<true, false, 2>), dim3((unsigned)tiles), dim3(RR_THREADS), 0, st,
                                                             sr.keys, (const uint32_t *)SA, (const uint32_t *)nullptr, n, w.tcnt, w.thead,
                                                             SA, w.isa, Ucur, Gcur, Vcur, (uint32_t)n, (uint32_t *)nullptr, 0, pk_out, pv_out, (const uint32_t *)w.total, 0, (const uint32_t *)nullptr, 0, (uint32_t *)nullptr));
+#ifdef SA_AMD_DIAG
+                g_setup_route.store(from_bits ? (setup_counted ? 2 : 1) + (ranks_in_pass ? 4 : 0) : 0, std::memory_order_relaxed);
+#endif
                 if (from_sa) {
                     hipLaunchKernelGGL(k_set_u32, dim3(1), dim3(1), 0, st, dSA, (uint32_t)n);
                     LAUNCH_CHECK(st);
-                    rc = scatter_binned(dSA, pk32 + H, sk32, sk32 + H, n + 1, n, w, st, &local, tn, false, pk32);
+                    rc = scatter_binned(dSA, pk32 + H, sk32, sk32 + H, n + 1, n, w, st, &local, tn, false, pk32, nullptr, setup_counted, ranks_in_pass ? &hvals : (const HeadVals *)nullptr);
                 } else
                     rc = scatter_binned((uint32_t *)pk, w.U1, (uint32_t *)sr.keys, w.G1, n, n, w, st, &local, tn);
                 if (rc) return rc;
diff --git a/suffix_array_amd/csrc/host/tuning.hpp b/suffix_array_amd/csrc/host/tuning.hpp
--- a/suffix_array_amd/csrc/host/tuning.hpp
+++ b/suffix_array_amd/csrc/host/tuning.hpp
@@ -28,6 +28,7 @@
 
 #ifdef SA_AMD_DIAG
 inline std::atomic<int> g_rerank_routes{0};
+inline std::atomic<int> g_setup_route{-1};
 #endif
 
 struct Tuning {
@@ -53,6 +54,8 @@
     bool no_first_tail = false;
     bool sa_every_round = false;
     bool setup_key_copy = false;
+    bool setup_from_keys = false;
+    bool setup_ranks_in_pass = false;
     bool no_repeat_probe = false;
     int64_t binned_min = (int64_t)1 << 26;
     int chase = 7;
@@ -179,6 +182,8 @@
             const int r = g_rerank_routes.load(std::memory_order_relaxed);
             t.sa_every_round = (r & 1) != 0;
             t.setup_key_copy = (r & 2) != 0;
+            t.setup_from_keys = (r & 4) != 0;
+            t.setup_ranks_in_pass = (r & 8) != 0;
         }
 #endif
         return t;
diff --git a/suffix_array_amd/csrc/kernels/onesweep.hpp b/suffix_array_amd/csrc/kernels/onesweep.hpp
--- a/suffix_array_amd/csrc/kernels/onesweep.hpp
+++ b/suffix_array_amd/csrc/kernels/onesweep.hpp
@@ -7,6 +7,7 @@
 constexpr int OS_NSEG = 8;
 constexpr int OS_LB = 3;
 struct __attribute__((packed, aligned(4))) Words4 { uint32_t x, y, z, w; };
+constexpr int OS_HEAD_SPAN = 8192;
 constexpr int OS_MIN_TILE = 4096;
 
 __device__ __forceinline__ unsigned os_xcc_id()
@@ -149,10 +150,14 @@
     int64_t text_n;
     int text_bits;
     int val_extra;
+    const unsigned long long *head_bits;
+    const uint32_t *head_next;
+    int64_t head_n;
+    int head_tiles;
     uint32_t flags;
 };
 
-template <int THREADS, int ITEMS, typename KeyT, bool SEQ, int WG_PER_CU, int RBITS = RADIX_BITS, bool TEXT_KEYS = false>
+template <int THREADS, int ITEMS, typename KeyT, bool SEQ, int WG_PER_CU, int RBITS = RADIX_BITS, bool TEXT_KEYS = false, bool HEAD_VALS = false>
 __global__ __launch_bounds__(THREADS, WG_PER_CU * THREADS / 256) void k_onesweep(
     const KeyT *__restrict__ keys_in, const uint32_t *__restrict__ vals_in, KeyT *__restrict__ keys_out, uint32_t *__restrict__ vals_out,
     OnesweepPass P)
@@ -177,6 +182,11 @@
     __shared__ uint32_t hist2[RADIX * OS_NSEG];
     __shared__ uint32_t scan_lds[NWAVES + 1];
     __shared__ int s_tile, s_seg;
+    constexpr int HB_TILE_WORDS = TILE / 64, HB_WORDS = HB_TILE_WORDS + OS_HEAD_SPAN / 64;
+    static_assert(!HEAD_VALS || (!SEQ && !TEXT_KEYS && TILE % 64 == 0 && HB_WORDS % WAVE == 0 && HB_WORDS < THREADS), "bitmap slice: whole words, a whole number per lane of one wave");
+    __shared__ unsigned long long hb_w[HEAD_VALS ? HB_WORDS : 1];
+    __shared__ uint32_t hb_next[HEAD_VALS ? HB_WORDS + 1 : 1];
+    __shared__ uint32_t hb_tail;
     uint32_t *lds_v = SEQ ? (uint32_t *)lds_k : lds_v_sep;
 
     const int tid = threadIdx.x, l = lane_id(), w = wave_id();
@@ -241,6 +251,17 @@
         const int64_t base = (int64_t)t * TILE;
         const int valid = (P.n - base) >= TILE ? TILE : (int)(P.n - base);
         const bool full = valid == TILE;
+        if (HEAD_VALS) {
+            const int64_t q = base + TILE;
+            const int64_t span_t = q / OS_HEAD_SPAN;
+            if (tid < HB_WORDS) {
+                const int64_t wi = (base >> 6) + tid;
+                hb_w[tid] = (wi < ((P.head_n + 63) >> 6) && wi < (span_t + 1) * (OS_HEAD_SPAN / 64)) ? P.head_bits[wi] : 0ull;
+            } else if (tid == HB_WORDS) {
+                const uint32_t code = span_t < P.head_tiles ? P.head_next[span_t] : 0xffffffffu;
+                hb_tail = code == 0xffffffffu ? (uint32_t)P.head_n : code >> 1;
+            }
+        }
         KeyT key[ITEMS];
         uint32_t val[ITEMS], pp[ITEMS / 2];
         uint32_t xpack = 0;
@@ -296,6 +317,33 @@
         }
         for (int i = tid; i < NWAVES * RADIX / 2; i += THREADS) ((uint32_t *)&wave_hist[0][0])[i] = 0;
         __syncthreads();
+        if (HEAD_VALS && w == NWAVES - 1) {
+            constexpr int PER = HB_WORDS / WAVE;
+            const uint32_t b32 = (uint32_t)base;
+            uint32_t mine = 0xffffffffu;
+#pragma unroll
+            for (int k = PER - 1; k >= 0; --k) {
+                const unsigned long long wv = hb_w[l * PER + k];
+                if (wv) mine = b32 + (uint32_t)((l * PER + k) * 64 + __builtin_ctzll(wv));
+            }
+            uint32_t sfx = mine;
+#pragma unroll
+            for (int o = 1; o < WAVE; o <<= 1) {
+                const uint32_t other = (uint32_t)__shfl_down((int)sfx, o, WAVE);
+                if (l + o < WAVE && other < sfx) sfx = other;
+            }
+            uint32_t run = (uint32_t)__shfl_down((int)sfx, 1, WAVE);
+            if (l == WAVE - 1) run = 0xffffffffu;
+            const uint32_t tail = hb_tail;
+            run = run < tail ? run : tail;
+#pragma unroll
+            for (int k = PER - 1; k >= 0; --k) {
+                const int wd = l * PER + k;
+                hb_next[wd + 1] = run;
+                const unsigned long long wv = hb_w[wd];
+                if (wv) run = b32 + (uint32_t)(wd * 64 + __builtin_ctzll(wv));
+            }
+        }
         stamp(0);
 #pragma unroll
         for (int j = 0; j < ITEMS; ++j) {
@@ -319,7 +367,14 @@
         }
         stamp(1);
         auto load_vals = [&]() {
-        if (vals_in) {
+        if (HEAD_VALS) {
+#pragma unroll
+            for (int j = 0; j < ITEMS; ++j) {
+                const int e = OS_ELEM(j);
+                const unsigned long long rest = hb_w[e >> 6] >> (e & 63);
+                val[j] = rest ? (uint32_t)base + (uint32_t)(e + __builtin_ctzll(rest)) : hb_next[(e >> 6) + 1];
+            }
+        } else if (vals_in) {
 #pragma unroll
             for (int j = 0; j < ITEMS; ++j) {
                 const int e = OS_ELEM(j);
@@ -335,7 +390,7 @@
             }
         }
         };
-        if (!SEQ) load_vals();
+        if (!SEQ && !HEAD_VALS) load_vals();
         lds_barrier();
         stamp(2);
         uint32_t tot = 0;
@@ -374,6 +429,7 @@
             if (full || OS_ELEM(j) < valid) lds_k[ps] = key[j];
         }
         if (!SEQ) {
+            if (HEAD_VALS) load_vals();
 #pragma unroll
             for (int j = 0; j < ITEMS; ++j)
                 if (full || OS_ELEM(j) < valid) lds_v[OS_POS(j)] = val[j];
diff --git a/suffix_array_amd/csrc/kernels/rerank.hpp b/suffix_array_amd/csrc/kernels/rerank.hpp
--- a/suffix_array_amd/csrc/kernels/rerank.hpp
+++ b/suffix_array_amd/csrc/kernels/rerank.hpp
@@ -73,19 +73,27 @@
     return code;
 }
 
-template <bool FIRST, typename KeyT = uint64_t, bool PARENTS = false>
+template <bool FIRST, typename KeyT = uint64_t, bool PARENTS = false, bool HEAD_BITS = false>
 __global__ __launch_bounds__(RR_THREADS) void k_rr_count(const KeyT *__restrict__ keys,
                                                           const uint32_t *__restrict__ U, int64_t m,
                                                           uint32_t *__restrict__ tile_cnt,
                                                           uint32_t *__restrict__ tile_head, int key_shift,
                                                           uint32_t *__restrict__ tile_first, int g_shift,
-                                                          const uint32_t *__restrict__ gate = nullptr)
+                                                          const uint32_t *__restrict__ gate = nullptr,
+                                                          uint64_t *__restrict__ head_bits = nullptr)
 {
     __shared__ uint32_t wcnt[RR_THREADS / WAVE], whead[RR_THREADS / WAVE], wfirst[RR_THREADS / WAVE];
     if (gate && *gate) return;
     const int64_t wbase = (int64_t)blockIdx.x * RR_TILE + (int64_t)wave_id() * RR_WAVE_ELEMS;
     uint64_t kk[RR_ITEMS + 1];
     const WaveGroups g = rr_wave_classify<KeyT, false>(keys, m, wbase, key_shift, 0, PARENTS ? kk : nullptr);
+    if (HEAD_BITS) {
+        uint64_t mine = 0;
+#pragma unroll
+        for (int r = 0; r < RR_ITEMS; ++r) mine = lane_id() == r ? g.head[r] : mine;
+        const int64_t word = (wbase >> 6) + lane_id();
+        if (lane_id() < RR_ITEMS && word < ((m + 63) >> 6)) head_bits[word] = mine;
+    }
     uint32_t cnt = 0, lasthead = 0;
 #pragma unroll
     for (int r = 0; r < RR_ITEMS; ++r) {
@@ -374,4 +382,105 @@
     }
 }
 
-}
+constexpr int RB_TPW = 4;
+__global__ __launch_bounds__(RR_THREADS) void k_rr_apply_bits(
+    const uint64_t *__restrict__ head_bits, const uint32_t *__restrict__ V, int64_t m,
+    const uint32_t *__restrict__ tile_cnt, const uint32_t *__restrict__ tile_head, const uint32_t *__restrict__ tile_next,
+    uint32_t *__restrict__ Uo, uint32_t *__restrict__ Go, uint32_t *__restrict__ Vo, uint32_t *__restrict__ pair_v,
+    uint32_t *__restrict__ counts, int64_t chunk_elems, int G, int dshift, uint32_t dmask, uint32_t front_key)
+{
+    constexpr int NW = RR_THREADS / WAVE;
+    __shared__ uint32_t wcnt[NW], whead[NW], wfirst[NW];
+    __shared__ uint32_t dhist[2 * RADIX];
+    const int l = lane_id(), w = wave_id();
+    for (int d = threadIdx.x; d < 2 * RADIX; d += RR_THREADS) dhist[d] = 0;
+    if (counts && blockIdx.x == 0 && threadIdx.x == 0) atomicAdd(&counts[(int64_t)((front_key >> dshift) & dmask) * G], 1u);
+    const int64_t tiles = (m + RR_TILE - 1) / RR_TILE, nwords = (m + 63) >> 6;
+    const int64_t tile0 = (int64_t)blockIdx.x * RB_TPW;
+    const int64_t tile1 = tile0 + RB_TPW < tiles ? tile0 + RB_TPW : tiles;
+    const uint64_t le_mask = (l == 63) ? ~0ull : ((2ull << l) - 1ull);
+    const uint64_t lt_mask = le_mask >> 1;
+    __syncthreads();
+    for (int64_t tile = tile0; tile < tile1; ++tile) {
+        const int64_t tbase = tile * RR_TILE;
+        const int64_t wbase = tbase + (int64_t)w * RR_WAVE_ELEMS;
+        const int64_t word = (wbase >> 6) + l;
+        const uint64_t mine = (l <= RR_ITEMS && word < nwords) ? head_bits[word] : 0ull;
+        uint64_t head[RR_ITEMS], tied[RR_ITEMS], valid[RR_ITEMS];
+        uint32_t v[RR_ITEMS];
+#pragma unroll
+        for (int r = 0; r < RR_ITEMS; ++r) {
+            const int64_t i = wbase + 64 * r + l;
+            head[r] = shfl64(mine, r);
+            valid[r] = __ballot(i < m);
+            v[r] = i < m ? V[i] : 0u;
+        }
+        const bool boundary_after = (wbase + RR_WAVE_ELEMS >= m) || (shfl64(mine, RR_ITEMS) & 1ull) != 0ull;
+        uint32_t cnt = 0, lasthead = 0, firsthead = RR_NO_HEAD;
+#pragma unroll
+        for (int r = RR_ITEMS - 1; r >= 0; --r) {
+            const uint64_t bnd = head[r] | ~valid[r];
+            const uint64_t bnd_next0 = (r + 1 < RR_ITEMS) ? ((head[(r + 1) % RR_ITEMS] | ~valid[(r + 1) % RR_ITEMS]) & 1ull)
+                                                          : (boundary_after ? 1ull : 0ull);
+            tied[r] = valid[r] & ~(head[r] & ((bnd >> 1) | (bnd_next0 << 63)));
+            cnt += (uint32_t)__popcll(tied[r]);
+            if (head[r]) {
+                if (!lasthead) lasthead = (uint32_t)(wbase + 64 * r + (63 - __builtin_clzll(head[r]))) + 1u;
+                firsthead = (uint32_t)(wbase + 64 * r + __builtin_ctzll(head[r]));
+            }
+        }
+        if (l == 0) { wcnt[w] = cnt; whead[w] = lasthead; wfirst[w] = firsthead; }
+        const int64_t seg = (tbase + 1) / chunk_elems;
+        const int64_t seg_end = (seg + 1) * chunk_elems;
+#pragma unroll
+        for (int r = 0; counts && r < RR_ITEMS; ++r) {
+            const int64_t i = wbase + 64 * r + l;
+            const bool in = i < m;
+            const uint32_t d = (((v[r] >> dshift) & dmask) & (uint32_t)(RADIX - 1)) + (i + 1 >= seg_end ? (uint32_t)RADIX : 0u);
+            const uint64_t act = __ballot(in);
+            const uint32_t f = (uint32_t)__builtin_amdgcn_readfirstlane((int)d);
+            if (__all(!in || d == f)) {
+                if (act && l == 0) atomicAdd(&dhist[f], (uint32_t)__popcll(act));
+            } else if (in) atomicAdd(&dhist[d], 1u);
+        }
+        __syncthreads();
+        uint32_t run_cnt = tile_cnt[tile], run_head = tile_head[tile];
+        for (int ww = 0; ww < w; ++ww) { run_cnt += wcnt[ww]; run_head = run_head > whead[ww] ? run_head : whead[ww]; }
+        uint32_t next_head[RR_ITEMS];
+        {
+            const uint32_t code = tile_next[tile];
+            uint32_t behind = code == RR_NO_HEAD ? (uint32_t)m : code >> 1;
+            for (int ww = NW - 1; ww > w; --ww) behind = wfirst[ww] != RR_NO_HEAD ? wfirst[ww] : behind;
+#pragma unroll
+            for (int r = RR_ITEMS - 1; r >= 0; --r) {
+                next_head[r] = behind;
+                if (head[r]) behind = (uint32_t)(wbase + 64 * r + __builtin_ctzll(head[r]));
+            }
+        }
+#pragma unroll
+        for (int r = 0; r < RR_ITEMS; ++r) {
+            const int64_t i = wbase + 64 * r + l;
+            const uint64_t hle = head[r] & le_mask;
+            const uint32_t run = hle ? (uint32_t)(wbase + 64 * r + (63 - __builtin_clzll(hle))) + 1u : run_head;
+            const uint64_t hgt = (l == 63) ? 0ull : (head[r] & (~0ull << (l + 1)));
+            if (i < m) {
+                if (pair_v) pair_v[i] = hgt ? (uint32_t)(wbase + 64 * r + __builtin_ctzll(hgt)) : next_head[r];
+                if ((tied[r] >> l) & 1ull) {
+                    const uint32_t off = run_cnt + (uint32_t)__popcll(tied[r] & lt_mask);
+                    Uo[off] = (uint32_t)i; Go[off] = run - 1u; Vo[off] = v[r];
+                }
+            }
+            run_cnt += (uint32_t)__popcll(tied[r]);
+            if (head[r]) run_head = (uint32_t)(wbase + 64 * r + (63 - __builtin_clzll(head[r]))) + 1u;
+        }
+        if (counts && (tile + 1 == tile1 || tbase + RR_TILE + 1 >= seg_end)) {
+            for (int d = threadIdx.x; d < 2 * RADIX; d += RR_THREADS) {
+                const uint32_t c = dhist[d];
+                if (c) { atomicAdd(&counts[(int64_t)(d & (RADIX - 1)) * G + seg + (d >> RADIX_BITS)], c); dhist[d] = 0; }
+            }
+        }
+        __syncthreads();
+    }
+}
+
+}
diff --git a/suffix_array_amd/csrc/sa_diag.h b/suffix_array_amd/csrc/sa_diag.h
--- a/suffix_array_amd/csrc/sa_diag.h
+++ b/suffix_array_amd/csrc/sa_diag.h
@@ -7,6 +7,7 @@
 int32_t sa_amd_debug_phase_cycles(uint64_t *out, int32_t count);
 int32_t sa_amd_debug_group_sort_stamps(int32_t on);
 int32_t sa_amd_debug_rerank_routes(int32_t flags);
+int32_t sa_amd_debug_last_setup_route(void);
 int32_t sa_amd_debug_sort_variant_count(void);
 const char *sa_amd_debug_sort_variant_name(int32_t index);
 int32_t sa_amd_test_sort_pairs(uint64_t *keys, uint32_t *vals, int64_t count, int32_t begin_bit, int32_t end_bit);
diff --git a/suffix_array_amd/csrc/sa_diag.inc b/suffix_array_amd/csrc/sa_diag.inc
--- a/suffix_array_amd/csrc/sa_diag.inc
+++ b/suffix_array_amd/csrc/sa_diag.inc
@@ -17,8 +17,10 @@
 
 SA_EXPORT int32_t sa_amd_debug_rerank_routes(int32_t flags)
 {
-    return sa::g_rerank_routes.exchange(flags & 3);
-}
+    return sa::g_rerank_routes.exchange(flags & 15);
+}
+
+SA_EXPORT int32_t sa_amd_debug_last_setup_route(void) { return sa::g_setup_route.exchange(-1); }
 
 SA_EXPORT int32_t sa_amd_debug_sort_variant_count(void) { return sa::N_SORT_VARIANTS; }
 SA_EXPORT const char *sa_amd_debug_sort_variant_name(int32_t i)
```

Result: faster. 5657 MB/s, median of 6 (+1.5%).
